# CookiePPP/cookietts

Measured on AMD Instinct MI355X. Metric: audio samples/sec (22.05kHz) WaveGlow infer, 80×900 mel, 1/2/4/8 GPU; real-time factor, higher is better.
Workload: dtype f32; 1 GPU; WaveGlow full (12 flows, 512 WN ch, 8 groups, 8 layers) fp32 infer, batch 8 x (80x900) mel per GPU, sigma 0.6, random-init weights; batch_per_gpu=8, frames=900, parallelism=utterance-batch shard x1

## Files before the change

cookietts_amd/_lib.py:

```python
from __future__ import annotations

import ctypes as C
import os
import threading

import torch

from . import build as _build

_LOCK = threading.Lock()
_LIB = None


class WaveGlowConfig(C.Structure):
    _fields_ = [(n, C.c_int32) for n in (
        "n_mel_channels", "n_group", "n_flows", "n_early_every", "n_early_size",
        "win_length", "hop_length", "n_layers", "n_channels", "kernel_size", "cond_hidden", "speaker_embed_dim",
        "f32_gemm_mode")]


class StftConfig(C.Structure):
    _fields_ = [("filter_length", C.c_int32), ("hop_length", C.c_int32), ("win_length", C.c_int32),
                ("n_mel_channels", C.c_int32), ("clamp_val", C.c_float)]

# ... 205 lines not shown
    "ctts_torchmoji_lengths": (C.c_int, [_FP, _FP, C.c_int32, C.c_int32, _FP]),
    "ctts_torchmoji_features_f32": (C.c_int, [C.POINTER(TorchMojiConfig), _FP, _FP, _FP, _FP, _FP, C.c_int32, C.c_int32, _FP,
                                              C.c_size_t, _FP]),
    "ctts_attention_pool_f32": (C.c_int, [_FP, _FP, _FP, _FP, _FP, C.c_int32, C.c_int32, C.c_int32, _FP]),
    "ctts_taco_embed_f32": (C.c_int, [_FP, _FP, _FP, _FP, _FP, C.c_int32, C.c_int32, C.c_int32, C.c_int32, C.c_int32,
                                      C.c_int32, _FP]),
    "ctts_taco_memory_f32": (C.c_int, [C.POINTER(TacoMemoryWeights), _FP, _FP, _FP, _FP, _FP, C.c_int32, C.c_int32,
                                       C.c_int32, C.c_int32, C.c_int32, C.c_int32, C.c_int32, _FP]),
    "ctts_taco_memory_sylps_f32": (C.c_int, [C.POINTER(TacoMemoryWeights), _FP, _FP, _FP, _FP, _FP, _FP, C.c_int32, C.c_int32,
                                             C.c_int32, C.c_int32, C.c_int32, C.c_int32, C.c_int32, _FP]),
    "ctts_pad_rows_f32": (C.c_int, [_FP, C.c_int64, C.c_int32, _FP, C.c_int32, C.c_int32, C.c_int32, C.c_int32,
                                    C.c_int32, _FP]),
    "ctts_unpad_rows_f32": (C.c_int, [_FP, _FP, C.c_int64, C.c_int32, C.c_int32, C.c_int32, C.c_int32, C.c_int32,
                                      C.c_int32, _FP]),
    "ctts_stft_packed_bytes": (C.c_size_t, [C.POINTER(StftConfig)]),
    "ctts_stft_pack": (C.c_int, [C.POINTER(StftConfig), _FP, _FP, _FP, _FP]),
    "ctts_stft_workspace_bytes": (C.c_size_t, [C.POINTER(StftConfig), C.c_int32, C.c_int32]),
    "ctts_stft_mel_f32": (C.c_int, [C.POINTER(StftConfig), _FP, _FP, _FP, _FP, C.c_int32, C.c_int32, _FP,
                                    C.c_size_t, _FP]),
    "ctts_stft_pack_inverse": (C.c_int, [C.POINTER(StftConfig), _FP, _FP, _FP, _FP]),
    "ctts_stft_transform_f32": (C.c_int, [C.POINTER(StftConfig), _FP, _FP, _FP, _FP, C.c_int32, C.c_int32, _FP,
                                          C.c_size_t, _FP]),
    "ctts_stft_inverse_f32": (C.c_int, [C.POINTER(StftConfig), _FP, _FP, _FP, _FP, C.c_float, _FP, C.c_int32,
                                        C.c_int32, _FP, C.c_size_t, _FP]),
    "ctts_stft_inverse_bias_f32": (C.c_int, [C.POINTER(StftConfig), _FP, _FP, _FP, _FP, C.c_int32, C.c_float, _FP,
                                             C.c_int32, C.c_int32, _FP, C.c_size_t, _FP]),
    "ctts_waveflow_inverse_cond_f32": (C.c_int, [C.POINTER(WaveFlowConfig), _FP, _FP, _FP, C.c_int32, C.c_int32, _FP,
                                                 C.c_int32, C.c_int32, C.c_int32, _FP, C.c_size_t, _FP]),
    "ctts_waveflow_abort_status": (C.c_int, [C.POINTER(WaveFlowConfig), C.c_int32, C.c_int32, _FP, C.c_size_t, _FP]),
    "ctts_wgax_packed_bytes": (C.c_size_t, [C.POINTER(WgaxConfig)]),
    "ctts_wgax_pack_flow": (C.c_int, [C.POINTER(WgaxConfig), C.c_int32, C.POINTER(WgaxFlowWeights), _FP, _FP]),
    "ctts_wgax_workspace_bytes": (C.c_size_t, [C.POINTER(WgaxConfig), C.c_int32, C.c_int64]),
    "ctts_wgax_inverse_f32": (C.c_int, [C.POINTER(WgaxConfig), _FP, _FP, _FP, C.c_int32, C.c_int32, C.c_int32, _FP,
                                        C.c_int32, C.c_int64, _FP, C.c_size_t, _FP]),
    "ctts_wgax_packed_f16_bytes": (C.c_size_t, [C.POINTER(WgaxConfig)]),
    "ctts_wgax_pack_flow_f16": (C.c_int, [C.POINTER(WgaxConfig), C.c_int32, C.POINTER(WgaxFlowWeights), _FP, _FP]),
    "ctts_wgax_workspace_f16_bytes": (C.c_size_t, [C.POINTER(WgaxConfig), C.c_int32, C.c_int64]),
    "ctts_wgax_inverse_f16": (C.c_int, [C.POINTER(WgaxConfig), _FP, _FP, _FP, C.c_int32, C.c_int32, C.c_int32, _FP,
                                        C.c_int32, C.c_int64, _FP, C.c_size_t, _FP]),
    "ctts_wgax_sep_packed_bytes": (C.c_size_t, [C.POINTER(WgaxConfig)]),
    "ctts_wgax_sep_pack_flow": (C.c_int, [C.POINTER(WgaxConfig), C.c_int32, C.POINTER(WgaxFlowWeights), C.POINTER(_FP),
                                          C.POINTER(_FP), _FP, _FP]),
    "ctts_wgax_sep_workspace_bytes": (C.c_size_t, [C.POINTER(WgaxConfig), C.c_int32, C.c_int64]),
    "ctts_wgax_sep_inverse_f32": (C.c_int, [C.POINTER(WgaxConfig), _FP, _FP, _FP, C.c_int32, C.c_int32, C.c_int32, _FP,
                                            C.c_int32, C.c_int64, _FP, C.c_size_t, _FP]),
    "ctts_depthwise_conv1d_f32": (C.c_int, [_FP, _FP, _FP, _FP] + [C.c_int32] * 7 + [_FP]),
    "ctts_hifigan_weight_floats": (C.c_size_t, [C.POINTER(HifiganConfig)]),
    "ctts_hifigan_packed_bytes": (C.c_size_t, [C.POINTER(HifiganConfig)]),
    "ctts_hifigan_pack_f32": (C.c_int, [C.POINTER(HifiganConfig), _FP, C.c_size_t, _FP, _FP]),
    "ctts_hifigan_workspace_bytes": (C.c_size_t, [C.POINTER(HifiganConfig), C.c_int32, C.c_int32]),
    "ctts_hifigan_forward_f32": (C.c_int, [C.POINTER(HifiganConfig), _FP, _FP, C.c_int32, _FP, C.c_int32, C.c_int32, _FP,
                                           C.c_size_t, _FP]),
    "ctts_hifigan_packed_f16_bytes": (C.c_size_t, [C.POINTER(HifiganConfig)]),
    "ctts_hifigan_pack_f16": (C.c_int, [C.POINTER(HifiganConfig), _FP, C.c_size_t, _FP, _FP]),
    "ctts_hifigan_workspace_f16_bytes": (C.c_size_t, [C.POINTER(HifiganConfig), C.c_int32, C.c_int32]),
    "ctts_hifigan_forward_f16": (C.c_int, [C.POINTER(HifiganConfig), _FP, _FP, C.c_int32, _FP, C.c_int32, C.c_int32, _FP,
                                           C.c_size_t, _FP]),
    "ctts_hifigan_packed_bf16x3_bytes": (C.c_size_t, [C.POINTER(HifiganConfig)]),
    "ctts_hifigan_pack_bf16x3": (C.c_int, [C.POINTER(HifiganConfig), _FP, C.c_size_t, _FP, _FP]),
    "ctts_hifigan_workspace_bf16x3_bytes": (C.c_size_t, [C.POINTER(HifiganConfig), C.c_int32, C.c_int32]),
    "ctts_hifigan_forward_bf16x3": (C.c_int, [C.POINTER(HifiganConfig), _FP, _FP, C.c_int32, _FP, C.c_int32, C.c_int32, _FP,
                                              C.c_size_t, _FP]),
    "ctts_replicate_halo_f32":(C.c_int, [_FP, C.c_int32, C.c_int32, C.c_int32, C.c_int32, C.c_int32, C.c_int32, _FP]),
    "ctts_embed_rows_f32": (C.c_int, [_FP, _FP, _FP, C.c_int32, C.c_int32, C.c_int32, C.c_int32, C.c_int32, C.c_int32,
                                      C.c_int32, _FP]),
    "ctts_scale_add_rows_f32": (C.c_int, [_FP, _FP, _FP, _FP, C.c_int32, C.c_int32, C.c_int32, C.c_int32, C.c_int32,
                                          _FP]),
    "ctts_deemphasis_f32": (C.c_int, [_FP, _FP, C.c_int32, C.c_int32, C.c_double, _FP]),
    "ctts_alignment_workspace_bytes": (C.c_size_t, [C.c_int32, C.c_int32, C.c_int32]),
    "ctts_alignment_metric_f32": (C.c_int, [_FP, _FP, _FP, C.c_int32, C.c_int32, C.c_int32, C.c_float, _FP, _FP,
                                            C.c_size_t, _FP]),
    "ctts_first_over_thresh_f32": (C.c_int, [_FP, C.c_int32, C.c_int32, C.c_float, _FP, _FP]),
    "ctts_taco_stop_state_bytes": (C.c_size_t, [C.c_int32]),
    "ctts_taco_stop_reset": (C.c_int, [_FP, C.c_int32, C.c_int32, _FP]),
    "ctts_taco_stop_rule_f32": (C.c_int, [_FP, C.c_int32, C.c_int32, C.c_int32, C.c_int32, C.c_float, C.c_int32, _FP, _FP]),
    "ctts_retry_state_bytes": (C.c_size_t, [C.POINTER(RetryConfig)]),
    "ctts_retry_state_layout": (C.c_int, [C.POINTER(RetryConfig), C.POINTER(C.c_size_t)]),
    "ctts_retry_reset": (C.c_int, [C.POINTER(RetryConfig), _FP, _FP]),
    "ctts_retry_update_f32": (C.c_int, [C.POINTER(RetryConfig), _FP, _FP, _FP, _FP, _FP, _FP, C.c_int32, C.c_int32, _FP, _FP,
                                        _FP]),
    "ctts_retry_vocoder_batch_f32": (C.c_int, [C.POINTER(RetryConfig), _FP, _FP, C.c_int32, C.c_float, _FP]),
    "ctts_pcm16_concat": (C.c_int, [_FP, C.c_int32, _FP, C.c_int32, C.c_int64, C.c_int32, C.c_int32, _FP, C.c_int64, _FP,
                                    _FP]),
    "ctts_affine_rows_f32": (C.c_int, [_FP, C.c_int32, C.c_int32, C.c_int32, C.c_int32, C.c_int32, C.c_int32, C.c_float,
                                       C.c_float, _FP]),
    "ctts_vol_unscale_f32": (C.c_int, [_FP, C.c_int64, _FP]),
    "ctts_resample_rows_f32": (C.c_int, [_FP, _FP] + [C.c_int32] * 9 + [C.c_float, _FP]),
    "ctts_interleave_phases_f32": (C.c_int, [_FP, _FP] + [C.c_int32] * 10 + [_FP]),
    "ctts_last_gemm_loop": (C.c_int, []),
    "ctts_tuning_reload": (C.c_int, []),
    "ctts_tuning_flags": (C.c_int, []),
    "ctts_profile_create": (C.c_int, [C.POINTER(C.c_void_p)]),
    "ctts_profile_bind": (C.c_int, [C.c_void_p]),
    "ctts_profile_collect": (C.c_int, [C.c_void_p, C.c_int32, C.POINTER(C.c_int64), C.POINTER(C.c_double)]),
    "ctts_profile_destroy": (C.c_int, [C.c_void_p]),
}

MODEL_GEMM_MODES = {None: 0, "default": 0, "f32": 1, "bf16x3": 2, "bf16x6": 3}
GEMM_MODES = {"f32": 1, "bf16x3": 2, "bf16x6": 3}


def model_gemm_mode(mode):
    try:
        return MODEL_GEMM_MODES[mode]
    except KeyError:
        raise ValueError(f"f32 GEMM mode {mode!r}: expected one of 'default', 'f32', 'bf16x3', 'bf16x6'") from None


def set_f32_gemm_mode(mode):
    if mode in (None, "default", "f32"):
        return "f32"
    raise RuntimeError(f"cookietts_amd.set_f32_gemm_mode({mode!r}): the process-wide default was removed; "
                       f"call model.set_f32_gemm_mode({mode!r}) on each model instead")


class Profile:

    def __init__(self):
        h = C.c_void_p()
        check(lib().ctts_profile_create(C.byref(h)), "ctts_profile_create")
        self._h = h

    def __enter__(self):
        check(lib().ctts_profile_bind(self._h), "ctts_profile_bind")
        return self

    def __exit__(self, *exc):
        check(lib().ctts_profile_bind(None), "ctts_profile_bind")
        return False

    bind = __enter__

    def unbind(self):
        self.__exit__()

    def collect(self, which):
        n, ms = C.c_int64(), C.c_double()
        check(lib().ctts_profile_collect(self._h, which, C.byref(n), C.byref(ms)), "ctts_profile_collect")
        return int(n.value), float(ms.value)

    def close(self):
        if self._h is not None and _LIB is not None:
            _LIB.ctts_profile_destroy(self._h)
        self._h = None

    def __del__(self):
        try:
            self.close()
        except Exception:
            pass


TUNING_BITS = {"CTTS_F32_NO_GLDS": 0, "CTTS_GEMM_NO_XCD_PAIR": 1, "CTTS_F32_WINOGRAD_FUSED_MIN": 2, "CTTS_BF16_NO_WIDE": 3, "CTTS_BF16_NO_PP": 4,
               "CTTS_F32_WINOGRAD_NO_FUSED": 5, "CTTS_WF_NO_FUSE": 7,
               "CTTS_TACO_NO_FUSE": 8, "CTTS_F32_NO_SMALL": 9, "CTTS_F32_FORCE_SMALL": 10, "CTTS_F32_NO_SPLITK": 11, "CTTS_WF_NO_VEC_INTERP": 12,
               "CTTS_F32_NO_DEFER_SKIP": 13, "CTTS_WF_NO_REGION_SPLIT": 14, "CTTS_WF_NO_ROW_QUEUE": 15, "CTTS_WF_ROW_QUEUE_MIN": 16,
               "CTTS_WF_INJECT_ABORT": 17, "CTTS_WF_QUEUE_DEBUG": 18, "CTTS_F32_NO_ROUND_SPLIT": 19, "CTTS_BF16_PS": 20, "CTTS_BF16_NO_PS": 21,
               "CTTS_TACO_POLL_DELAY": 23, "CTTS_TACO_VALU": 24, "CTTS_UP_NO_MFMA": 25, "CTTS_F32_NO_WN_FOLD": 26, "CTTS_TACO_BG_NO_PIPE": 27,
               "CTTS_F32_NO_WINOGRAD": 28, "CTTS_F32_WINOGRAD_MIN": 29, "CTTS_F32_WINOGRAD_PLAIN": 30}


def tuning_reload():
    check(lib().ctts_tuning_reload(), "ctts_tuning_reload")


def tuning_active(name):
    return bool(lib().ctts_tuning_flags() >> TUNING_BITS[name] & 1)


PROF_WN_IN = 0
PROF_WN_RS = 1
PROF_WN_SKIP = 2
PROF_WN_IN0F = 3
PROF_WN_SKEND = 4
PROF_WN_RES_F = 5


class HipLibraryError(RuntimeError):
    pass


def lib_path():
    return _build.LIB_PATH


def lib():
    global _LIB
    if _LIB is not None:
        return _LIB
    with _LOCK:
        if _LIB is not None:
            return _LIB
        path = lib_path()
        if not os.path.exists(path):
            raise HipLibraryError(
                f"{path} is missing: build it with `python -m cookietts_amd.build` "
                "(or __graft_entry__.build()); there is no CPU fallback for the hot path")
        try:
            handle = C.CDLL(path)
        except OSError as e:
            raise HipLibraryError(f"cannot load {path}: {e}") from e
        for name, (res, args) in SIGNATURES.items():
            try:
                fn = getattr(handle, name)
            except AttributeError as e:
                raise HipLibraryError(f"{path} does not export {name}") from e
            fn.restype = res
            fn.argtypes = args
        if handle.ctts_abi_version() != 7:
            raise HipLibraryError(f"ABI version mismatch: library reports {handle.ctts_abi_version()}")
        _LIB = handle
    return _LIB


def last_error():
    msg = lib().ctts_last_error()
    return msg.decode(errors='replace') if msg else ''


def check(rc, what):
    if rc != 0:
        raise HipLibraryError(f"{what} failed (rc={rc}): {last_error()}")


def nbytes(fn, *args, what):
    n = fn(*args)
    if n == 0:
        raise HipLibraryError(f"{what}: {last_error()}")
    return n


def ptr(t):
    if t is None:
        return None
    return C.c_void_p(t.data_ptr())


def stream(device):
    return C.c_void_p(torch.cuda.current_stream(device).cuda_stream)
```

cookietts_amd/csrc/gemm_f32.hip:

```cpp
#include <atomic>
#include <cstdlib>
#include <mutex>

#include "gemm_f32.h"
#include "tuning.h"
#include "gemm_bf16.h"

namespace ctts {

typedef float f32x16 __attribute__((ext_vector_type(16)));

namespace {

constexpr int STAGE = GEMM_KC * (256 + 128);
constexpr int GEMM_GLDS_MAX_CHUNKS = 384;

__device__ __forceinline__ float fast_sigmoid(float u) {
    return __builtin_amdgcn_rcpf(1.0f + __builtin_amdgcn_exp2f(u * -1.4426950408889634f));
}
__device__ __forceinline__ float fast_tanh(float u) {
    return 1.0f - 2.0f * __builtin_amdgcn_rcpf(1.0f + __builtin_amdgcn_exp2f(u * 2.8853900817779268f));
}

typedef const __attribute__((address_space(1))) float* gfloat_ptr;
// ... 564 lines not shown
                            if (c < a.pairC && ns_ok) dst[(size_t)c * a.dst_ld + a.dst_pad + ns] = v;
                        }
                    }
                }
            }
        }
    } else if constexpr (EPI == GEMM_EPI_GATE_RS) {
        static_assert(EPI != GEMM_EPI_GATE_RS || WM == 1, "fused res/skip needs the 128-row block shape");
        float actv[2][2][16];
#pragma unroll
        for (int mt = 0; mt < 2; ++mt)
#pragma unroll
            for (int nt = 0; nt < 2; ++nt)
#pragma unroll
                for (int r = 0; r < 16; ++r) {
                    const int row = (r & 3) + 8 * (r >> 2) + 4 * lhi;
                    const bool ok = mt * 32 + row < a.pairC;
                    float u0 = acc[mt][nt][r] + bias[mt * 32 + row];
                    float u1 = acc[mt + 2][nt][r] + bias[64 + mt * 32 + row];
                    if (a.addend) {
                        const float* ad = a.addend + (size_t)b * a.addend_bstride + a.addend_pad + n0 + wn * 64 + nt * 32 + l31;
                        const int c = min(mt * 32 + row, a.pairC - 1);
                        u0 += ad[(size_t)c * a.addend_ld];
                        u1 += ad[(size_t)(a.pairC + c) * a.addend_ld];
                    }
                    actv[mt][nt][r] = ok ? fast_tanh(u0) * fast_sigmoid(u1) : 0.0f;
                }
        __syncthreads();
        for (int i = t * 4; i < 64 * 128; i += 1024)
            *reinterpret_cast<float4*>(lds + i) = *reinterpret_cast<const float4*>(a.rs_wT + i);
        if (t < 128) lds[64 * 128 + t] = a.rs_bias[t];
        __syncthreads();
#pragma unroll
        for (int i = 0; i < 4; ++i)
#pragma unroll
            for (int j = 0; j < 2; ++j)
#pragma unroll
                for (int r = 0; r < 16; ++r) acc[i][j][r] = 0.0f;
#pragma unroll
        for (int s = 0; s < 32; ++s) {
            const int r = s & 15;
            const int ch = (s >> 4) * 32 + (r & 3) + 8 * (r >> 2) + 4 * lhi;
            float a2[4];
#pragma unroll
            for (int mt = 0; mt < 4; ++mt) a2[mt] = lds[ch * 128 + mt * 32 + l31];
#pragma unroll
            for (int mt = 0; mt < 4; ++mt)
#pragma unroll
                for (int nt = 0; nt < 2; ++nt)
                    acc[mt][nt] = __builtin_amdgcn_mfma_f32_32x32x2f32(a2[mt], actv[s >> 4][nt][r], acc[mt][nt], 0, 0, 0);
        }
        split_epilogue<GEMM_EPI_SPLIT>(a, acc, lds + 64 * 128, a.rs_rows, 0, b, n0 + wn * 64, l31, lhi);
    } else {
        split_epilogue<EPI>(a, acc, bias, a.M, mb * BM + wm * 128, b, n0 + wn * 64, l31, lhi, EXT ? (long long)part * a.part_dst0 : 0);
    }
#undef CTTS_MAP_PAR
#undef CTTS_A_PTR
}

inline int gemm_f32_mode() { return CTTS_GEMM_F32; }

template <int EPI, int XS>
void launch_shape_xs(int bm, dim3 grid, hipStream_t stream, const GemmArgs& a) {
    const bool few = a.nseg <= 4;
    if (bm == 128) {
        if (few) hipLaunchKernelGGL((conv_gemm_f32_kernel<EPI, 1, 4, true, XS>), grid, dim3(256), 0, stream, a);
        else hipLaunchKernelGGL((conv_gemm_f32_kernel<EPI, 1, GEMM_MAX_SEG, true, XS>), grid, dim3(256), 0, stream, a);
    } else {
        if (few) hipLaunchKernelGGL((conv_gemm_f32_kernel<EPI, 2, 4, true, XS>), grid, dim3(256), 0, stream, a);
        else hipLaunchKernelGGL((conv_gemm_f32_kernel<EPI, 2, GEMM_MAX_SEG, true, XS>), grid, dim3(256), 0, stream, a);
    }
}

template <int EPI, bool GLDS>
void launch_shape_g(int bm, dim3 grid, hipStream_t stream, const GemmArgs& a) {
    const bool few = a.nseg <= 4;
    if (bm == 128) {
        if (few) hipLaunchKernelGGL((conv_gemm_f32_kernel<EPI, 1, 4, GLDS>), grid, dim3(256), 0, stream, a);
        else hipLaunchKernelGGL((conv_gemm_f32_kernel<EPI, 1, GEMM_MAX_SEG, GLDS>), grid, dim3(256), 0, stream, a);
    } else {
        if (few) hipLaunchKernelGGL((conv_gemm_f32_kernel<EPI, 2, 4, GLDS>), grid, dim3(256), 0, stream, a);
        else hipLaunchKernelGGL((conv_gemm_f32_kernel<EPI, 2, GEMM_MAX_SEG, GLDS>), grid, dim3(256), 0, stream, a);
    }
}

template <int EPI>
void launch_shape(int bm, dim3 grid, hipStream_t stream, const GemmArgs& a) {
    if (tuning().f32_no_glds || a.nch_total > GEMM_GLDS_MAX_CHUNKS) launch_shape_g<EPI, false>(bm, grid, stream, a);
    else if (gemm_split_level(a.gemm_mode) == 6) launch_shape_xs<EPI, 6>(bm, grid, stream, a);
    else if (gemm_split_level(a.gemm_mode) == 3) launch_shape_xs<EPI, 3>(bm, grid, stream, a);
    else launch_shape_g<EPI, true>(bm, grid, stream, a);
}

}

int get_gemm_f32_mode() { return gemm_f32_mode(); }
namespace { thread_local int t_last_loop = 0; }
void note_gemm_loop(int code) { t_last_loop = code; }
int last_gemm_loop() { return t_last_loop; }
int gemm_split_level(int m) {
    if (m == CTTS_GEMM_DEFAULT) m = gemm_f32_mode();
    if (m == CTTS_GEMM_BF16X3) return 3;
    if (m == CTTS_GEMM_BF16X6) return 6;
    return 0;
}
bool gemm_mode_is_split(int m) { return gemm_split_level(m) != 0; }

namespace {
std::mutex g_tune_mu;
Tuning g_tune{};
bool g_tune_loaded = false;
void load_tuning_locked() {
    auto on = [](const char* n) { return getenv(n) != nullptr; };
    auto num = [](const char* n, int d) { const char* v = getenv(n); return v ? atoi(v) : d; };
    g_tune.f32_no_glds = on("CTTS_F32_NO_GLDS");
    g_tune.f32_no_small = on("CTTS_F32_NO_SMALL");
    g_tune.f32_force_small = on("CTTS_F32_FORCE_SMALL");
    g_tune.f32_no_splitk = on("CTTS_F32_NO_SPLITK");
    g_tune.f32_no_round_split = on("CTTS_F32_NO_ROUND_SPLIT");
    g_tune.no_xcd_pair = on("CTTS_GEMM_NO_XCD_PAIR");
    g_tune.bf16_no_wide = on("CTTS_BF16_NO_WIDE");
    g_tune.bf16_no_pp = on("CTTS_BF16_NO_PP");
    g_tune.bf16_wide_min = num("CTTS_BF16_WIDE_MIN", 192);
    g_tune.bf16_ps = on("CTTS_BF16_PS");
    g_tune.bf16_no_ps = on("CTTS_BF16_NO_PS");
    g_tune.wf_no_fuse = on("CTTS_WF_NO_FUSE");
    g_tune.taco_no_fuse = on("CTTS_TACO_NO_FUSE");
    g_tune.taco_valu = on("CTTS_TACO_VALU");
    g_tune.up_no_mfma = on("CTTS_UP_NO_MFMA");
    g_tune.taco_bg_no_pipe = on("CTTS_TACO_BG_NO_PIPE");
    {
        static const int dflt[6] = {0x10000 | 36, 0x10000 | 96, 0x10000 | 12, 0x10000 | 20, 0x10000 | 8, 0x10000 | 8};
        int v[6];
        for (int i = 0; i < 6; ++i) v[i] = dflt[i];
        const char* e = getenv("CTTS_TACO_POLL_DELAY");
        if (e && sscanf(e, "%d,%d,%d,%d,%d,%d", v, v + 1, v + 2, v + 3, v + 4, v + 5) != 6)
            for (int i = 0; i < 6; ++i) v[i] = dflt[i];
        for (int i = 0; i < 6; ++i) g_tune.taco_poll_delay[i] = v[i] < 0 ? 0 : v[i];
        g_tune.taco_poll_delay_set = e != nullptr;
    }
    g_tune.wf_no_vec_interp = on("CTTS_WF_NO_VEC_INTERP");
    g_tune.wf_no_region_split = on("CTTS_WF_NO_REGION_SPLIT");
    g_tune.wf_no_row_queue = on("CTTS_WF_NO_ROW_QUEUE");
    g_tune.wf_row_queue_min = num("CTTS_WF_ROW_QUEUE_MIN", -1);
    g_tune.wf_inject_abort = num("CTTS_WF_INJECT_ABORT", 0);
    g_tune.wf_queue_debug = num("CTTS_WF_QUEUE_DEBUG", 0);
    g_tune.f32_no_defer_skip = on("CTTS_F32_NO_DEFER_SKIP");
    g_tune.f32_no_wn_fold = on("CTTS_F32_NO_WN_FOLD");
    g_tune.f32_no_winograd = on("CTTS_F32_NO_WINOGRAD");
    g_tune.f32_winograd_min = num("CTTS_F32_WINOGRAD_MIN", -1);
    g_tune.f32_winograd_plain = on("CTTS_F32_WINOGRAD_PLAIN");
    g_tune.f32_winograd_fused_min = num("CTTS_F32_WINOGRAD_FUSED_MIN", -1);
    g_tune.f32_winograd_no_fused = on("CTTS_F32_WINOGRAD_NO_FUSED");
    g_tune_loaded = true;
}
}

Tuning tuning() {
    std::lock_guard<std::mutex> lk(g_tune_mu);
    if (!g_tune_loaded) load_tuning_locked();
    return g_tune;
}
void reload_tuning() {
    std::lock_guard<std::mutex> lk(g_tune_mu);
    load_tuning_locked();
}

int gemm_check_args(int epi, const GemmArgs& a) {
    CTTS_CHECK_ARG(a.bm == 256 || a.bm == 128, "gemm: bm=%d", a.bm);
    CTTS_CHECK_ARG(gemm_mode_valid(a.gemm_mode), "gemm: f32_gemm_mode %d (0 default, 1 fp32 MFMA, 2 split bf16)", a.gemm_mode);
    const int bn = gemm_bn(a.bm);
    CTTS_CHECK_ARG(a.nseg >= 1 && a.nseg <= GEMM_MAX_SEG, "gemm: nseg=%d", a.nseg);
    int nch = 0;
    for (int s = 0; s < a.nseg; ++s) {
        CTTS_CHECK_ARG(a.seg[s].nch > 0 && a.seg[s].base, "gemm: empty segment %d", s);
        CTTS_CHECK_ARG(a.seg[s].shift >= -a.pad && a.seg[s].shift <= a.pad,
                       "gemm: shift %d exceeds halo %d", a.seg[s].shift, a.pad);
        nch += a.seg[s].nch;
    }
    CTTS_CHECK_ARG(nch == a.nch_total, "gemm: chunk count mismatch %d vs %d", nch, a.nch_total);
    if (a.interleave > 1) {
        CTTS_CHECK_ARG(a.interleave <= a.nseg, "gemm: interleave %d > nseg %d", a.interleave, a.nseg);
        for (int s = 1; s < a.interleave; ++s)
            CTTS_CHECK_ARG(a.seg[s].nch == a.seg[0].nch, "gemm: interleaved segments must have equal length");
    }
    CTTS_CHECK_ARG(a.a_nch_alloc == 0 || a.a_ch_off + a.nch_total <= a.a_nch_alloc, "gemm: A chunk window");
    CTTS_CHECK_ARG(a.ld % 4 == 0 && a.ntiles * bn + 2 * a.pad <= a.ld && a.L <= a.ntiles * bn,
                   "gemm: bad geometry ld=%d pad=%d L=%d ntiles=%d bn=%d", a.ld, a.pad, a.L, a.ntiles, bn);
    CTTS_CHECK_ARG(gemm_epi_is_pair(epi) || a.split % 32 == 0, "gemm: split %d not a multiple of 32", a.split);
    const int cpb = a.bm / 2;
    CTTS_CHECK_ARG(gemm_epi_is_pair(epi) ? (a.pairC > (a.MB - 1) * cpb && a.pairC <= a.MB * cpb)
                                         : (a.M > (a.MB - 1) * a.bm && a.M <= a.MB * a.bm),
                   "gemm: M=%d pairC=%d MB=%d bm=%d", a.M, a.pairC, a.MB, a.bm);
    CTTS_CHECK_ARG(a.dst_ld > 0 && a.dst0, "gemm: destination not set");
    CTTS_CHECK_ARG(a.addend_frames == 0 || ((epi == GEMM_EPI_GATE || epi == GEMM_EPI_GATEX) && a.addend && a.addend_frames <= a.addend_ld - a.addend_pad),
                   "gemm: interpolated addend needs the GATE epilogue (frames=%d)", a.addend_frames);
    CTTS_CHECK_ARG(a.gate >= 0 && a.gate < GATE_KINDS && (a.gate == 0 || epi == GEMM_EPI_GATE), "gemm: gate=%d with epilogue %d",
                   a.gate, epi);
    CTTS_CHECK_ARG((a.addend2 == nullptr && a.map_d == 0) ||
                       (epi == GEMM_EPI_GATE && a.gate == GATE_GTU && a.addend_frames == 0 && a.map_d >= 0 &&
                        (a.addend2 == nullptr || (a.addend && (a.addend2_sign == 1.0f || a.addend2_sign == -1.0f))) &&
                        (a.map_d == 0 || ((a.map_par == 0 || a.map_par == 1) && a.map_L > 0 && a.map_col0 >= 0))),
                   "gemm: second addend / mapped store need the GATE epilogue (epilogue %d, map_d=%d)", epi, a.map_d);
    CTTS_CHECK_ARG(epi != GEMM_EPI_GATE_RS ||
                       (a.bm == 128 && a.pairC <= 64 && a.MB == 1 && a.rs_wT && a.rs_bias && (a.rs_rows == 64 || a.rs_rows == 128)),
                   "gemm: fused res/skip needs bm=128, <= 64 channels, rs_wT / rs_bias and 64 or 128 res/skip rows");
    const int parts = a.parts > 1 ? a.parts : 1;
    CTTS_CHECK_ARG(a.parts >= 0 && a.parts <= 2 && (a.mseg == 0 || a.mseg == 2), "gemm: parts=%d mseg=%d", a.parts, a.mseg);
    if (parts > 1 || a.mseg) {
        CTTS_CHECK_ARG((epi == GEMM_EPI_SPLIT || (epi == GEMM_EPI_GATE && a.gate == GATE_GTU)) && a.bm == 256 && a.nseg <= 4 &&
                           a.interleave <= 1 && gemm_split_level(a.gemm_mode) == 0 && a.shape_blocks == 0 && a.addend_frames == 0,
                       "gemm: parts / mapped segment need the fp32 SPLIT or GATE launch of the 256-row shape (epilogue %d, nseg=%d)", epi, a.nseg);
        CTTS_CHECK_ARG(parts == 1 || epi != GEMM_EPI_SPLIT || (a.acc0 == 0 && a.src0 == nullptr && a.split >= a.M),
                       "gemm: a two-part SPLIT launch stores every row to dst0");
        CTTS_CHECK_ARG(parts == 1 || (long long)parts * a.ntiles * a.batch < (1ll << 31) / a.MB, "gemm: merged grid");
    }
    if (a.mseg) {
        const GemmSeg& g = a.seg[1];
        CTTS_CHECK_ARG(epi == GEMM_EPI_GATE && a.nseg == 2 && a.map_d > 0 && a.map_d % 4 == 0 && a.map_col0 % 4 == 0 && a.mseg_pad >= 0 &&
                           a.mseg_pad % 4 == 0 && a.mseg_ld % 4 == 0 && a.mseg_ld - a.mseg_pad >= 4 && g.bstride % 4 == 0 &&
                           (parts == 1 || a.part_seg[1] % 4 == 0) && reinterpret_cast<uintptr_t>(g.base) % 16 == 0 && g.shift == 0 &&
                           g.mb_rows == 0,
                       "gemm: mapped segment d=%d col0=%d ld=%d pad=%d", a.map_d, a.map_col0, a.mseg_ld, a.mseg_pad);
    }
    return CTTS_OK;
}

bool gemm_f32_dma_staged(int nch_total) { return !tuning().f32_no_glds && nch_total <= GEMM_GLDS_MAX_CHUNKS; }

namespace {
GemmArgs gemm_part_args(const GemmArgs& a, int p) {
    GemmArgs r = a;
    r.parts = 0;
    if (p == 0) return r;
    r.A += a.part_A;
    for (int j = 0; j < r.nseg && j < 4; ++j) r.seg[j].base += a.part_seg[j];
    r.dst0 += a.part_dst0;
    r.map_par = p;
    r.addend2_sign = -a.addend2_sign;
    return r;
}
}

int launch_gemm_f32(int epi, const GemmArgs& a_in, hipStream_t stream) {
    GemmArgs a = a_in;
    gemm_apply_defaults(a);
    if (int rc = gemm_check_args(epi, a)) return rc;
    if (epi == GEMM_EPI_GATE && a.gate != GATE_GTU) epi = GEMM_EPI_GATEX;
    const int parts = a.parts > 1 ? a.parts : 1;
    const bool ext = parts > 1 || a.mseg;
    a.mseg_ch0 = a.mseg_ch1 = 0;
    if (a.mseg) { a.mseg_ch0 = a.seg[0].nch; a.mseg_ch1 = a.seg[0].nch + a.seg[1].nch; }
    CTTS_CHECK_ARG(!a.mseg || gemm_f32_dma_staged(a.nch_total), "gemm: the mapped segment needs the DMA-staged kernels");
    if (parts > 1 && (gemm_f32_small_applies(epi, a) || !gemm_f32_dma_staged(a.nch_total))) {
        for (int p = 0; p < parts; ++p)
            if (int rc = launch_gemm_f32(epi, gemm_part_args(a, p), stream)) return rc;
        return CTTS_OK;
    }
    if (gemm_f32_small_applies(epi, a)) return launch_gemm_f32_small(epi, a, stream);
    long long tiles = (long long)parts * a.ntiles * a.batch;
    if (a.bm == 256 && epi != GEMM_EPI_GATE_RS && a.addend_frames == 0 && a.shape_blocks == 0 && !tuning().f32_no_round_split &&
        !tuning().f32_no_glds && !tuning().f32_no_small && a.nch_total <= GEMM_GLDS_MAX_CHUNKS) {
        const long long slots = 2ll * wf_row_cus();
        const long long rounds = a.MB * tiles / slots;
        const long long rem_tiles = (a.MB * tiles - rounds * slots + a.MB - 1) / a.MB;
        if (rounds >= 2 && rem_tiles > 0 && rem_tiles * a.MB <= slots * 3 / 10 && rem_tiles < a.ntiles &&
            (long long)(a.ntiles - rem_tiles) * gemm_bn(a.bm) < a.L) {
            GemmArgs r = gemm_part_args(a, parts - 1);
            const int bn = gemm_bn(a.bm);
            const long long co = (long long)(a.ntiles - rem_tiles) * bn;
            const long long bo = a.batch - 1;
            for (int j = 0; j < r.nseg; ++j) r.seg[j].base += bo * r.seg[j].bstride + (r.mseg && j == 1 ? 0 : co);
            if (r.dst0) r.dst0 += bo * r.dst0_bstride + (r.map_d > 0 ? 0 : co);
            if (r.map_d > 0) r.map_col0 += (int)co;
            if (r.dst1) r.dst1 += bo * r.dst1_bstride + co;
            if (r.src0) r.src0 += bo * r.src0_bstride + co;
            if (r.addend) r.addend += bo * r.addend_bstride + co;
            if (r.addend2) r.addend2 += bo * r.addend_bstride + co;
            r.L = a.L - (int)co;
            r.ntiles = (int)rem_tiles;
            r.batch = 1;
            if (int rc = launch_gemm_f32_small(epi, r, stream)) return rc;
            tiles -= rem_tiles;
        }
    }
    a.gt_limit = (int)tiles;
    long long blocks = (long long)a.MB * tiles;
    a.map_mode = 0;
    if (a.MB == 4 && epi != GEMM_EPI_GATE_RS && !tuning().no_xcd_pair) {
        a.map_mode = 1;
        blocks = 16ll * ((tiles + 3) / 4);
    }
    CTTS_CHECK_ARG(blocks > 0 && blocks < (1ll << 31), "gemm: grid %lld", blocks);
    dim3 grid((unsigned)blocks);
    note_gemm_loop((tuning().f32_no_glds || a.nch_total > GEMM_GLDS_MAX_CHUNKS) ? 0 : gemm_split_level(a.gemm_mode));
    if (ext) {
        if (epi == GEMM_EPI_GATE) hipLaunchKernelGGL((conv_gemm_f32_kernel<GEMM_EPI_GATE, 2, 4, true, 0, true>), grid, dim3(256), 0, stream, a);
        else hipLaunchKernelGGL((conv_gemm_f32_kernel<GEMM_EPI_SPLIT, 2, 4, true, 0, true>), grid, dim3(256), 0, stream, a);
        CTTS_CHECK_LAUNCH("conv_gemm_f32");
        return CTTS_OK;
    }
    switch (epi) {
        case GEMM_EPI_GATEX: launch_shape<GEMM_EPI_GATEX>(a.bm, grid, stream, a); break;
        case GEMM_EPI_GATE: launch_shape<GEMM_EPI_GATE>(a.bm, grid, stream, a); break;
        case GEMM_EPI_GATE_RS:
            if (tuning().f32_no_glds || a.nch_total > GEMM_GLDS_MAX_CHUNKS) {
// ... 26 lines not shown
```

cookietts_amd/csrc/tuning.h:

```cpp
#pragma once

namespace ctts {

struct Tuning {
    bool f32_no_glds;
    bool f32_no_small;
    bool f32_force_small;
    bool f32_no_splitk;
    bool f32_no_round_split;
    bool no_xcd_pair;
    bool bf16_no_wide;
    int bf16_wide_min;
    bool bf16_no_pp;
    bool bf16_ps;
    bool bf16_no_ps;
    bool wf_no_fuse;
    bool taco_poll_delay_set;
    int taco_poll_delay[6];
    bool taco_no_fuse;
    bool taco_bg_no_pipe;
    bool up_no_mfma;
    bool taco_valu;
    bool f32_no_defer_skip;
    bool f32_no_wn_fold;
    bool f32_no_winograd;
    int f32_winograd_min;
    bool f32_winograd_plain;
    int f32_winograd_fused_min;
    bool f32_winograd_no_fused;
    bool wf_no_region_split;
    bool wf_no_row_queue;
    int wf_row_queue_min;
    int wf_queue_debug;
    int wf_inject_abort;
    bool wf_no_vec_interp;
};

Tuning tuning();
void reload_tuning();

}
```

cookietts_amd/csrc/waveglow_api.hip:

```cpp
#include <mutex>
#include <vector>

#include "gemm_bf16.h"
#include "gemm_f32.h"
#include "tuning.h"
#include "waveglow_kernels.h"
#include "wn_winograd_layer.h"

namespace ctts {

static thread_local char g_err[512] = "";

void set_error(const char* fmt, ...) {
    va_list ap;
    va_start(ap, fmt);
    vsnprintf(g_err, sizeof(g_err), fmt, ap);
    va_end(ap);
}

namespace {

constexpr size_t ALIGN_F = 64;
inline size_t align_up(size_t v) { return (v + ALIGN_F - 1) / ALIGN_F * ALIGN_F; }
constexpr int A_TILE = GEMM_KC * GEMM_BM;

struct FlowDims { int n_rem, n_half, ch_off; };

struct Plan {
    ctts_waveglow_config c;
    int C, H, K0, n_in;
    int S;
    int nch0, nch1h, nch_in, nch_rs;
    int mb_in;
    int nch_in0f;
    std::vector<FlowDims> fd;
    size_t up_w, up_wp, up_b, cond0_A, cond0_b, cond1_A, cond1_b;
    size_t zero_b;
    bool up_mfma;
    struct Flow {
        size_t start_w, start_b, end_w, end_b, winv, spk_tab;
        std::vector<size_t> in_A, in_b, rs_A, rs_b;
        std::vector<size_t> res_A, res_b, skip_A, skip_b;
        size_t in0f_w, in0f_A, skend_W, skend_b;
        std::vector<size_t> wg_T2_A, wg_T3_A, wg_e_A, wg_o_A;
        size_t wg_dense;
    };
    std::vector<Flow> fl;
    size_t total;

    static constexpr int F32_SKIP_GROUP = 4;
    int mb_c() const { return (C + GEMM_BM - 1) / GEMM_BM; }
    int n_groups() const { return (c.n_layers + F32_SKIP_GROUP - 1) / F32_SKIP_GROUP; }
    int group_layers(int g) const { return g + 1 < n_groups() ? F32_SKIP_GROUP : c.n_layers - g * F32_SKIP_GROUP; }
    int rs_rows(int layer) const { return layer < c.n_layers - 1 ? 2 * C : C; }
    int rs_mb(int layer) const { return (rs_rows(layer) + GEMM_BM - 1) / GEMM_BM; }
};

int make_plan(const ctts_waveglow_config* cfg, Plan& p) {
    CTTS_CHECK_ARG(cfg != nullptr, "config is NULL");
    p.c = *cfg;
    const auto& c = p.c;
    CTTS_CHECK_ARG(c.n_flows >= 1 && c.n_layers >= 1 && c.n_layers <= 12, "n_flows=%d n_layers=%d", c.n_flows, c.n_layers);
    CTTS_CHECK_ARG(gemm_mode_valid(c.f32_gemm_mode), "f32_gemm_mode=%d (CTTS_GEMM_DEFAULT / _F32 / _BF16X3 / _BF16X6)", c.f32_gemm_mode);
    CTTS_CHECK_ARG(c.n_group >= 4 && c.n_group % 4 == 0 && c.n_group <= 16, "n_group=%d (4, 8, 12 or 16)", c.n_group);
    CTTS_CHECK_ARG(c.kernel_size == 3, "kernel_size=%d (only 3 built)", c.kernel_size);
    CTTS_CHECK_ARG(c.n_channels >= 128 && c.n_channels % 128 == 0, "n_channels=%d (multiple of 128)", c.n_channels);
    CTTS_CHECK_ARG(c.cond_hidden == GEMM_BM, "cond_hidden=%d (reference hard-codes 256)", c.cond_hidden);
    CTTS_CHECK_ARG(c.hop_length > 0 && c.win_length % c.hop_length == 0 && c.hop_length % c.n_group == 0,
                   "win=%d hop=%d n_group=%d", c.win_length, c.hop_length, c.n_group);
    CTTS_CHECK_ARG((c.n_mel_channels * c.n_group) % GEMM_KC == 0, "n_mel*n_group=%d not a multiple of 16",
                   c.n_mel_channels * c.n_group);
    CTTS_CHECK_ARG(c.n_early_every >= 1 && c.n_early_size >= 0 && c.n_early_size % 2 == 0, "early outputs");
    CTTS_CHECK_ARG(c.speaker_embed_dim >= 0 && c.speaker_embed_dim <= 1024, "speaker_embed_dim=%d", c.speaker_embed_dim);
    p.C = c.n_channels;
    p.H = c.cond_hidden;
    p.K0 = c.n_mel_channels * c.n_group;
    p.S = round_up(c.speaker_embed_dim, 32);
    CTTS_CHECK_ARG(p.S == 0 || p.K0 % 32 == 0, "multispeaker needs n_mel*n_group %% 32 == 0");
    p.nch0 = (p.K0 + p.S) / GEMM_KC;
    p.nch1h = p.H / GEMM_KC;
    p.nch_in = (c.kernel_size * p.C + p.H) / GEMM_KC;
    p.nch_rs = p.C / GEMM_KC;
    p.mb_in = 2 * p.C / GEMM_BM;
    p.nch_in0f = c.kernel_size + p.nch1h;
    int n_half = c.n_group / 2, n_rem = c.n_group;
    p.fd.resize(c.n_flows);
    for (int k = 0; k < c.n_flows; ++k) {
        if (k % c.n_early_every == 0 && k > 0) { n_half -= c.n_early_size / 2; n_rem -= c.n_early_size; }
        CTTS_CHECK_ARG(n_half >= 1 && n_rem == 2 * n_half, "flow %d: n_half=%d n_remaining=%d", k, n_half, n_rem);
        p.fd[k] = {n_rem, n_half, c.n_group - n_rem};
    }
    size_t o = 0;
    auto take = [&](size_t n) { size_t r = o; o = align_up(o + n); return r; };
    p.up_w = take((size_t)c.n_mel_channels * c.n_mel_channels * c.win_length);
    p.up_mfma = upsample_mfma_shape(c.n_mel_channels, c.win_length, c.hop_length, c.n_group);
    p.up_wp = p.up_mfma ? take((size_t)c.n_mel_channels * c.n_mel_channels * c.win_length) : 0;
    p.up_b = take(c.n_mel_channels);
    p.cond0_A = take((size_t)c.n_flows * p.nch0 * A_TILE);
    p.cond0_b = take((size_t)c.n_flows * GEMM_BM);
    p.cond1_A = take((size_t)c.n_flows * p.nch1h * A_TILE);
    p.cond1_b = take((size_t)c.n_flows * GEMM_BM);
    p.zero_b = take((size_t)p.mb_in * GEMM_BM);
    p.fl.resize(c.n_flows);
    for (int k = 0; k < c.n_flows; ++k) {
        auto& f = p.fl[k];
        f.start_w = take((size_t)p.C * p.fd[k].n_half);
        f.start_b = take(p.C);
        f.end_w = take((size_t)2 * p.fd[k].n_half * p.C);
        f.end_b = take(2 * p.fd[k].n_half);
        f.winv = take((size_t)p.fd[k].n_rem * p.fd[k].n_rem);
        f.spk_tab = take((size_t)CTTS_N_SPEAKERS * c.speaker_embed_dim);
        for (int i = 0; i < c.n_layers; ++i) {
            f.in_A.push_back(take((size_t)p.mb_in * p.nch_in * A_TILE));
            f.in_b.push_back(take((size_t)p.mb_in * GEMM_BM));
            f.rs_A.push_back(take((size_t)p.rs_mb(i) * p.nch_rs * A_TILE));
            f.rs_b.push_back(take((size_t)p.rs_mb(i) * GEMM_BM));
            f.res_A.push_back(i + 1 < c.n_layers ? take((size_t)p.mb_c() * p.nch_rs * A_TILE) : 0);
            f.res_b.push_back(i + 1 < c.n_layers ? take((size_t)p.mb_c() * GEMM_BM) : 0);
        }
        for (int gi = 0; gi < p.n_groups(); ++gi) {
            f.skip_A.push_back(take((size_t)p.mb_c() * p.group_layers(gi) * p.nch_rs * A_TILE));
            f.skip_b.push_back(take((size_t)p.mb_c() * GEMM_BM));
        }
        f.in0f_w = take((size_t)2 * p.C * FOLD_ROWS * c.kernel_size);
        f.in0f_A = take((size_t)p.mb_in * p.nch_in0f * A_TILE);
        f.skend_W = take((size_t)c.n_layers * p.C * 2 * p.fd[k].n_half);
        f.skend_b = take(2 * p.fd[k].n_half);
        for (int i = 0; i < c.n_layers; ++i) {
            f.wg_T2_A.push_back(take((size_t)p.mb_in * p.nch_rs * A_TILE));
            f.wg_T3_A.push_back(take((size_t)p.mb_in * p.nch_rs * A_TILE));
            f.wg_e_A.push_back(take((size_t)p.mb_in * (p.nch_rs + p.nch1h) * A_TILE));
            f.wg_o_A.push_back(take((size_t)p.mb_in * (p.nch_rs + p.nch1h) * A_TILE));
        }
        f.wg_dense = take((size_t)3 * 2 * p.C * p.C);
    }
    p.total = o;
    return CTTS_OK;
}

struct Geom { int L, ld, pad, ntiles; };

int make_geom(const Plan& p, int frames, Geom& g) {
    CTTS_CHECK_ARG(frames >= 1, "frames=%d", frames);
    const long long T = (long long)frames * p.c.hop_length;
    g.L = (int)(T / p.c.n_group);
    int maxd = 1 << (p.c.n_layers - 1);
    g.pad = round_up(maxd > 128 ? maxd : 128, 32);
    g.ntiles = (g.L + GEMM_BN - 1) / GEMM_BN;
    g.ld = round_up(g.L, 256) + 2 * g.pad;
    return CTTS_OK;
}

struct PairGeom { int d, Lp, ntiles; };
PairGeom pair_geom(const Geom& g, int layer) {
    const int d = 1 << layer;
    const int Lp = (g.L + 2 * d - 1) / (2 * d) * d;
    return {d, Lp, (Lp + GEMM_BN - 1) / GEMM_BN};
}
int pair_ld(const Plan& p, const Geom& g) {
    int nt = 0;
    for (int i = 0; i < p.c.n_layers; ++i) nt = std::max(nt, pair_geom(g, i).ntiles);
    return nt * GEMM_BN;
}
constexpr long long WINOGRAD_MIN_COLS = 28800;
bool winograd_engages(const Plan& p, const Geom& g) {
    const Tuning t = tuning();
    if (t.f32_no_winograd || gemm_split_level(p.c.f32_gemm_mode) != 0) return false;
    const long long min_cols = t.f32_winograd_min >= 0 ? t.f32_winograd_min : WINOGRAD_MIN_COLS;
    return (long long)g.L >= min_cols;
}

constexpr long long WINOGRAD_FUSED_MIN_COLS = 28800;
bool winograd_fused_engages(const Plan& p, const Geom& g) {
    const Tuning t = tuning();
    if (t.f32_winograd_no_fused || t.f32_winograd_plain || t.f32_no_glds || !wn_winograd_layer_supported(p.C, p.H)) return false;
    const long long min_cols = t.f32_winograd_fused_min >= 0 ? t.f32_winograd_fused_min : WINOGRAD_FUSED_MIN_COLS;
    return winograd_engages(p, g) && (long long)g.L >= min_cols;
}

struct Workspace {
    float *audio, *spect, *spk, *h_tmp, *h_all, *x, *act, *out;
    float* act_all;
    float* a16;
    float* skend;
    float *wgV, *wgT, *wgH;
    int ldp;
    size_t total;
};

void carve(const Plan& p, const Geom& g, int batch, float* base, Workspace& w) {
    size_t o = 0;
    auto take = [&](size_t n) { size_t r = o; o = align_up(o + n); return base ? base + r : nullptr; };
    const size_t B = batch;
    w.audio = take(B * p.c.n_group * g.L);
    w.spect = take(B * p.K0 * g.ld);
    w.spk = take(B * p.c.n_flows * p.S * g.ld);
    w.h_tmp = take(B * p.c.n_flows * p.H * g.ld);
    w.h_all = take(B * p.c.n_flows * p.H * g.ld);
    w.x = take(B * p.C * g.ld);
    w.act = take(B * p.C * g.ld);
    w.out = take(B * p.C * g.ld);
    w.act_all = take((size_t)std::min(p.c.n_layers, (int)Plan::F32_SKIP_GROUP) * B * p.C * g.ld);
    w.a16 = take(B * FOLD_ROWS * g.ld);
    w.skend = take(B * p.c.n_group * g.ld);
    w.wgV = w.wgT = w.wgH = nullptr;
    w.ldp = 0;
    if (winograd_engages(p, g)) {
        w.ldp = pair_ld(p, g);
        w.wgV = take((size_t)4 * B * p.C * w.ldp);
        w.wgT = take((size_t)2 * B * 2 * p.C * w.ldp);
        w.wgH = take((size_t)2 * B * p.H * w.ldp);
    }
    w.total = o;
}

struct Prof {
    std::mutex mu;
    std::vector<std::pair<hipEvent_t, hipEvent_t>> ev[CTTS_PROF_N];
    std::vector<std::pair<hipEvent_t, hipEvent_t>> pool;
};
thread_local Prof* t_prof = nullptr;

struct ProfScope {
    int which; hipStream_t s; hipEvent_t stop = nullptr; bool active = false;
    ProfScope(int which_, hipStream_t s_) : which(which_), s(s_) {
        Prof* pr = t_prof;
        if (!pr) return;
        std::lock_guard<std::mutex> lk(pr->mu);
        std::pair<hipEvent_t, hipEvent_t> e;
        if (!pr->pool.empty()) { e = pr->pool.back(); pr->pool.pop_back(); }
        else { if (hipEventCreate(&e.first) != hipSuccess || hipEventCreate(&e.second) != hipSuccess) return; }
        (void)hipEventRecord(e.first, s);
        stop = e.second;
        pr->ev[which].push_back(e);
        active = true;
    }
    ~ProfScope() { if (active) (void)hipEventRecord(stop, s); }
};

GemmArgs base_args(const Plan& p, const Geom& g, int batch) {
    GemmArgs a{};
    a.gemm_mode = p.c.f32_gemm_mode;
    a.ld = g.ld; a.pad = g.pad; a.L = g.L; a.ntiles = g.ntiles; a.batch = batch;
    a.dst_ld = g.ld; a.dst_pad = g.pad;
    return a;
}

__global__ __launch_bounds__(256) void speaker_rows_kernel(const float* __restrict__ table, const int64_t* __restrict__ ids,
                                                           float* __restrict__ spk, int k, int n_flows, int S, int sdim,
                                                           int L, int ld, int pad) {
    const int n = blockIdx.x * 256 + threadIdx.x;
    const int e = blockIdx.y, b = blockIdx.z;
    if (n >= ld) return;
    float v = 0.f;
    if (e < sdim && n >= pad && n < pad + L) {
        const long long id = ids[b];
        v = (id >= 0 && id < CTTS_N_SPEAKERS) ? table[(size_t)id * sdim + e] : __builtin_nanf("");
    }
    spk[((size_t)b * n_flows * S + (size_t)k * S + e) * ld + n] = v;
}

int fill_speaker_rows(const Plan& p, const Geom& g, const float* blob, const int64_t* ids, float* spk, int batch,
                      hipStream_t s) {
    if (p.S == 0) return CTTS_OK;
    CTTS_CHECK_ARG(ids != nullptr, "multispeaker model (speaker_embed_dim=%d) needs speaker ids (glow.py:193)",
                   p.c.speaker_embed_dim);
    for (int k = 0; k < p.c.n_flows; ++k)
        hipLaunchKernelGGL(speaker_rows_kernel, dim3((g.ld + 255) / 256, p.S, batch), dim3(256), 0, s,
                           blob + p.fl[k].spk_tab, ids, spk, k, p.c.n_flows, p.S, p.c.speaker_embed_dim, g.L, g.ld, g.pad);
    CTTS_CHECK_LAUNCH("speaker_rows");
    return CTTS_OK;
}

int run_cond(const Plan& p, const Geom& g, const float* blob, const float* spect, const float* spk, float* h_tmp,
             float* h_all, int batch, hipStream_t s) {
    const long long hstride = (long long)p.c.n_flows * p.H * g.ld;
    GemmArgs a = base_args(p, g, batch);
    a.A = blob + p.cond0_A; a.bias = blob + p.cond0_b;
    a.nseg = 1; a.nch_total = p.nch0; a.MB = p.c.n_flows;
    a.seg[0] = {spect, (long long)p.K0 * g.ld, p.K0 / GEMM_KC, 0, 0, 0};
    if (p.S) {
        CTTS_CHECK_ARG(spk != nullptr, "wn_cond: multispeaker model needs the speaker rows");
        a.nseg = 2;
        a.seg[1] = {spk, (long long)p.c.n_flows * p.S * g.ld, p.S / GEMM_KC, 0, p.S, 0};
    }
    a.dst0 = h_tmp; a.dst0_bstride = hstride; a.acc0 = 0;
    a.dst1 = h_tmp; a.dst1_bstride = hstride; a.acc1 = 0;
    a.split = p.c.n_flows * GEMM_BM;
    a.M = p.c.n_flows * GEMM_BM;
    int rc = launch_gemm_f32(GEMM_EPI_SPLIT, a, s);
    if (rc) return rc;
    a.A = blob + p.cond1_A; a.bias = blob + p.cond1_b;
    a.nseg = 1; a.nch_total = p.nch1h;
    a.seg[0] = {h_tmp, hstride, p.nch1h, 0, GEMM_BM, 0};
    a.dst0 = h_all; a.dst1 = h_all;
    return launch_gemm_f32(GEMM_EPI_SPLIT, a, s);
}

struct WnFold { float* a16; float* skend; float* audio; float* wave; };
struct WnWinograd { float* V; float* T; float* Hc; int ldp; };

int run_in_layer_winograd(const Plan& p, const Geom& g, const float* blob, int k, int i, const float* x, const float* h_all,
                          float* act, const WnWinograd& wg, int batch, hipStream_t s) {
    const auto& f = p.fl[k];
    const PairGeom pg = pair_geom(g, i);
    const int C = p.C, H = p.H, ldp = wg.ldp;
    const long long hstride = (long long)p.c.n_flows * H * g.ld;
    const size_t vplane = (size_t)batch * C * ldp, tplane = (size_t)batch * 2 * C * ldp, hplane = (size_t)batch * H * ldp;
    const bool lean = !tuning().f32_winograd_plain && gemm_f32_dma_staged(p.nch_rs + p.nch1h);
    const bool in_place = lean && pg.d % 4 == 0;
    const bool fused = lean && winograd_fused_engages(p, g);
    const float* h2 = h_all + (size_t)k * H * g.ld;
    int rc = launch_winograd_transform(x, (long long)C * g.ld, h2, hstride, wg.V, wg.Hc, batch, C, H, pg.d, g.L, pg.Lp, g.ld, g.pad,
                                       ldp, pg.ntiles * GEMM_BN, !in_place, lean, s);
    if (rc) return rc;
    if (fused) {
        WnWinogradLayerArgs w{};
        w.A_T2 = blob + f.wg_T2_A[i]; w.A_T3 = blob + f.wg_T3_A[i]; w.A_e = blob + f.wg_e_A[i]; w.A_o = blob + f.wg_o_A[i];
        w.bias = blob + f.in_b[i];
        w.V = wg.V; w.vplane = (long long)vplane;
        w.Hc = wg.Hc; w.hplane = (long long)hplane;
        w.h2 = h2; w.h_bstride = hstride;
        w.act = act; w.act_bstride = (long long)C * g.ld;
        w.C = C; w.H = H; w.batch = batch;
        w.ldp = ldp; w.Lp = pg.Lp; w.ntiles = pg.ntiles;
        w.d = pg.d; w.L = g.L; w.ld = g.ld; w.pad = g.pad;
        w.in_place = in_place;
        return launch_wn_winograd_layer(w, s);
    }
    GemmArgs a{};
    a.gemm_mode = p.c.f32_gemm_mode;
    a.ld = ldp; a.pad = 0; a.L = pg.Lp; a.ntiles = pg.ntiles; a.batch = batch; a.MB = p.mb_in;
    a.bias = blob + p.zero_b;
    a.nseg = 1; a.nch_total = p.nch_rs;
    a.dst_ld = ldp; a.dst_pad = 0; a.dst0_bstride = (long long)2 * C * ldp;
    a.M = 2 * C; a.split = 2 * C;
    const int np = lean ? 1 : 2;
    if (lean) {
        a.parts = 2;
        a.part_A = (long long)f.wg_T3_A[i] - (long long)f.wg_T2_A[i];
        a.part_seg[0] = (long long)vplane;
        a.part_dst0 = (long long)tplane;
    }
    for (int j = 0; j < np; ++j) {
        a.A = blob + (j == 0 ? f.wg_T2_A[i] : f.wg_T3_A[i]);
        a.seg[0] = {wg.V + (1 + j) * vplane, (long long)C * ldp, p.nch_rs, 0, 0, 0};
        a.dst0 = wg.T + j * tplane;
        if ((rc = launch_gemm_f32(GEMM_EPI_SPLIT, a, s))) return rc;
    }
    a.bias = blob + f.in_b[i];
    a.nseg = 2; a.nch_total = p.nch_rs + p.nch1h;
    a.split = 0; a.pairC = C;
    a.dst0 = act; a.dst0_bstride = (long long)C * g.ld; a.dst_ld = g.ld; a.dst_pad = g.pad;
    a.addend = wg.T; a.addend2 = wg.T + tplane; a.addend_bstride = (long long)2 * C * ldp;
    a.map_d = pg.d; a.map_L = g.L;
    if (lean) {
        a.part_A = (long long)f.wg_o_A[i] - (long long)f.wg_e_A[i];
        a.part_seg[0] = (long long)(3 * vplane);
        a.part_seg[1] = in_place ? 0 : (long long)hplane;
        a.part_dst0 = 0;
    }
    if (in_place) { a.mseg = 2; a.mseg_ld = g.ld; a.mseg_pad = g.pad; }
    for (int j = 0; j < np; ++j) {
        a.A = blob + (j == 0 ? f.wg_e_A[i] : f.wg_o_A[i]);
        a.seg[0] = {wg.V + (j == 0 ? 0 : 3) * vplane, (long long)C * ldp, p.nch_rs, 0, 0, 0};
        if (in_place) a.seg[1] = {h2, hstride, p.nch1h, 0, 0, 0};
        else a.seg[1] = {wg.Hc + j * hplane, (long long)H * ldp, p.nch1h, 0, 0, 0};
        a.addend2_sign = j == 0 ? 1.0f : -1.0f;
        a.map_par = j;
        if ((rc = launch_gemm_f32(GEMM_EPI_GATE, a, s))) return rc;
    }
    return CTTS_OK;
}

int run_wn_stack(const Plan& p, const Geom& g, const float* blob, int k, const float* audio, const float* h_all,
                 float* x, float* act, float* out, int batch, hipStream_t s, float* act_all = nullptr,
                 const WnFold* fold = nullptr, const WnWinograd* wg = nullptr, const CouplingForward* fwd = nullptr) {
    const auto& f = p.fl[k];
    const auto& d = p.fd[k];
    const long long cstride = (long long)p.C * g.ld;
    const long long hstride = (long long)p.c.n_flows * p.H * g.ld;
    int rc = launch_wn_start(audio, blob + f.start_w, blob + f.start_b, x, batch, p.C, p.c.n_group, d.ch_off,
                             d.n_half, g.L, g.ld, g.pad, s);
    if (rc) return rc;
    CTTS_CHECK_ARG(fold == nullptr || act_all != nullptr, "wn_stack: the folded form needs the kept activations");
    if (fold && (rc = launch_wn_start_ones(audio, fold->a16, batch, p.c.n_group, d.ch_off, d.n_half, g.L, g.ld, g.pad, s)))
        return rc;
    const int ncx = p.C / GEMM_KC;
    const bool defer = act_all != nullptr && (fold != nullptr || !tuning().f32_no_defer_skip);
    const size_t act_stride = (size_t)batch * p.C * g.ld;
    for (int i = 0; i < p.c.n_layers; ++i) {
        const int dil = 1 << i;
        if (defer) act = act_all + (size_t)(i % Plan::F32_SKIP_GROUP) * act_stride;
        if (fold && i == 0) {
            GemmArgs a = base_args(p, g, batch);
            a.A = blob + f.in0f_A; a.bias = blob + f.in_b[0];
            a.nseg = 4; a.interleave = 3; a.nch_total = p.nch_in0f; a.MB = p.mb_in;
            const long long astride = (long long)FOLD_ROWS * g.ld;
            a.seg[0] = {fold->a16, astride, 1, -dil, 0, 0};
            a.seg[1] = {fold->a16, astride, 1, 0, 0, 0};
            a.seg[2] = {fold->a16, astride, 1, dil, 0, 0};
            a.seg[3] = {h_all + (size_t)k * p.H * g.ld, hstride, p.nch1h, 0, 0, 0};
            a.dst0 = act; a.dst0_bstride = cstride;
            a.M = 2 * p.C; a.pairC = p.C;
            ProfScope ps(CTTS_PROF_WN_IN, s), ps0(CTTS_PROF_WN_IN0F, s);
            rc = launch_gemm_f32(GEMM_EPI_GATE, a, s);
            if (rc) return rc;
        } else if (wg) {
            ProfScope ps(CTTS_PROF_WN_IN, s);
            rc = run_in_layer_winograd(p, g, blob, k, i, x, h_all, act, *wg, batch, s);
            if (rc) return rc;
        } else {
            GemmArgs a = base_args(p, g, batch);
            a.A = blob + f.in_A[i]; a.bias = blob + f.in_b[i];
            a.nseg = 4; a.interleave = 3; a.nch_total = p.nch_in; a.MB = p.mb_in;
            a.seg[0] = {x, cstride, ncx, -dil, 0, 0};
            a.seg[1] = {x, cstride, ncx, 0, 0, 0};
            a.seg[2] = {x, cstride, ncx, dil, 0, 0};
            a.seg[3] = {h_all + (size_t)k * p.H * g.ld, hstride, p.nch1h, 0, 0, 0};
            a.dst0 = act; a.dst0_bstride = cstride;
            a.M = 2 * p.C; a.pairC = p.C;
            ProfScope ps(CTTS_PROF_WN_IN, s);
            rc = launch_gemm_f32(GEMM_EPI_GATE, a, s);
            if (rc) return rc;
        }
        if (defer) {
            const bool last = i == p.c.n_layers - 1;
            if (!last) {
                GemmArgs a = base_args(p, g, batch);
                a.A = blob + f.res_A[i]; a.bias = blob + f.res_b[i];
                a.nseg = 1; a.nch_total = p.nch_rs; a.MB = p.mb_c();
                a.seg[0] = {act, cstride, p.nch_rs, 0, 0, 0};
                a.M = p.C; a.split = p.C;
                a.dst0 = x; a.dst0_bstride = cstride; a.acc0 = 1;
                a.dst1 = out; a.dst1_bstride = cstride; a.acc1 = 0;
                ProfScope ps(fold ? CTTS_PROF_WN_RES_F : CTTS_PROF_WN_RS, s);
                rc = launch_gemm_f32(GEMM_EPI_SPLIT, a, s);
                if (rc) return rc;
            }
            const int gi = i / Plan::F32_SKIP_GROUP;
            if (fold && (last || (i + 1) % Plan::F32_SKIP_GROUP == 0)) {
                const int E = 2 * d.n_half;
                ProfScope ps(CTTS_PROF_WN_SKEND, s);
                rc = launch_skip_end(act_all, (long long)act_stride, p.group_layers(gi),
                                     blob + f.skend_W + (size_t)gi * Plan::F32_SKIP_GROUP * p.C * E, fold->skend, gi == 0, last,
                                     blob + f.skend_b, blob + f.winv, fold->audio, fold->wave, batch, p.C, p.c.n_group, d.ch_off,
                                     d.n_half, g.L, g.ld, g.pad, s, last ? fwd : nullptr);
                if (rc) return rc;
            } else if (last || (i + 1) % Plan::F32_SKIP_GROUP == 0) {
                const int nl = p.group_layers(gi);
                GemmArgs a = base_args(p, g, batch);
                a.A = blob + f.skip_A[gi]; a.bias = blob + f.skip_b[gi];
                a.nseg = nl; a.nch_total = nl * p.nch_rs; a.MB = p.mb_c();
                for (int j = 0; j < nl; ++j)
                    a.seg[j] = {act_all + (size_t)j * act_stride, cstride, p.nch_rs, 0, 0, 0};
                a.M = p.C; a.split = 0;
                a.dst0 = x; a.dst0_bstride = cstride; a.acc0 = 1;
                a.dst1 = out; a.dst1_bstride = cstride; a.acc1 = gi > 0 ? 1 : 0;
                ProfScope ps(CTTS_PROF_WN_SKIP, s);
                rc = launch_gemm_f32(GEMM_EPI_SPLIT, a, s);
                if (rc) return rc;
            }
        } else {
            const bool last = i == p.c.n_layers - 1;
            GemmArgs a = base_args(p, g, batch);
            a.A = blob + f.rs_A[i]; a.bias = blob + f.rs_b[i];
            a.nseg = 1; a.nch_total = p.nch_rs; a.MB = p.rs_mb(i);
            a.seg[0] = {act, cstride, p.nch_rs, 0, 0, 0};
            a.M = p.rs_rows(i);
            a.dst0 = x; a.dst0_bstride = cstride; a.acc0 = 1;
            a.dst1 = out; a.dst1_bstride = cstride; a.acc1 = i > 0 ? 1 : 0;
            a.split = last ? 0 : p.C;
            ProfScope ps(CTTS_PROF_WN_RS, s);
            rc = launch_gemm_f32(GEMM_EPI_SPLIT, a, s);
            if (rc) return rc;
        }
    }
    return CTTS_OK;
}

int run_flow_tail(const Plan& p, const Geom& g, const float* blob, int k, const float* out, float* audio,
                  float* wave, int batch, hipStream_t s, const CouplingForward* fwd = nullptr) {
    const auto& f = p.fl[k];
    const auto& d = p.fd[k];
    return launch_flow_tail(out, audio, wave, blob + f.end_w, blob + f.end_b, blob + f.winv, batch, p.C,
                            p.c.n_group, d.ch_off, d.n_half, g.L, g.ld, g.pad, s, fwd);
}

int run_flow(const Plan& p, const Geom& g, const float* blob, int k, const Workspace& w, float* audio, const float* h_all,
             float* wave, int batch, hipStream_t s, const CouplingForward* fwd = nullptr) {
    const Tuning t = tuning();
    const bool folded = !t.f32_no_wn_fold && !t.f32_no_defer_skip;
    const WnWinograd wg{w.wgV, w.wgT, w.wgH, w.ldp};
    const WnFold fw{w.a16, w.skend, audio, wave};
    int rc = run_wn_stack(p, g, blob, k, audio, h_all, w.x, w.act, w.out, batch, s, w.act_all, folded ? &fw : nullptr,
                          w.wgV ? &wg : nullptr, fwd);
    if (rc || folded) return rc;
    return run_flow_tail(p, g, blob, k, w.out, audio, wave, batch, s, fwd);
}

size_t fwd_mix_off(const Plan& p, int k) {
    size_t o = 0;
    for (int j = 0; j < k; ++j) o += align_up((size_t)p.fd[j].n_rem * p.fd[j].n_rem);
    return o;
}
int fwd_log_s_rows(const Plan& p, int k) {
    int r = 0;
    for (int j = 0; j < k; ++j) r += p.fd[j].n_half;
    return r;
}

struct FwdWorkspace { Workspace w; double *ls_part, *z_part; int nblk_ls, nblk_z; size_t total; };

void carve_fwd(const Plan& p, const Geom& g, int batch, float* base, FwdWorkspace& fw) {
    carve(p, g, batch, base, fw.w);
    fw.nblk_ls = (g.L + 255) / 256;
    fw.nblk_z = (int)(((long long)p.c.n_group * g.L + FWD_SUMSQ_CHUNK - 1) / FWD_SUMSQ_CHUNK);
    size_t o = fw.w.total;
    auto take = [&](size_t doubles) { size_t r = o; o = align_up(o + 2 * doubles); return base ? reinterpret_cast<double*>(base + r) : nullptr; };
    fw.ls_part = take((size_t)batch * p.c.n_flows * fw.nblk_ls);
    fw.z_part = take((size_t)batch * fw.nblk_z);
    fw.total = o;
}

int run_flow_forward(const Plan& p, const Geom& g, const float* blob, const float* fwd_blob, int k, const FwdWorkspace& fw,
                     float* z, const float* wave, const float* h_all, float* log_s_flow, long long ls_bstride, int batch,
                     hipStream_t s) {
    const auto& d = p.fd[k];
    int rc = launch_flow_head_forward(fwd_blob + fwd_mix_off(p, k), wave, z, batch, p.c.n_group, d.ch_off, d.n_rem, g.L, s);
    if (rc) return rc;
    const CouplingForward cf{log_s_flow, ls_bstride, fw.ls_part + (size_t)k * fw.nblk_ls, (long long)p.c.n_flows * fw.nblk_ls};
    return run_flow(p, g, blob, k, fw.w, z, h_all, nullptr, batch, s, &cf);
}

constexpr int BF_SKIP_GROUP = 4;
struct BfPlan {
    std::vector<std::vector<size_t>> in_A, rs_A;
    std::vector<std::vector<size_t>> skip_A;
    std::vector<size_t> skip_b;
    size_t cond0_A, cond1_A;
    size_t total;
    int nch_in, nch_rs, nch_c0, nch_c1;
    int mb_c, n_groups;
    int P;
    int f16;
    int group_layers(int g, int n_layers) const { return std::min(BF_SKIP_GROUP, n_layers - g * BF_SKIP_GROUP); }
};

void make_bf_plan(const Plan& p, BfPlan& q, int P, int f16 = 0) {
    size_t o = 0;
    auto take = [&](size_t n) { size_t r = o; o = (o + n + 127) / 128 * 128; return r; };
    q.P = P;
    q.f16 = f16;
    q.nch_in = P * (p.c.kernel_size * p.C + p.H) / BGEMM_KC;
    q.nch_rs = P * p.C / BGEMM_KC;
    q.nch_c0 = P * (p.K0 + p.S) / BGEMM_KC;
    q.nch_c1 = P * p.H / BGEMM_KC;
    q.cond0_A = take((size_t)p.c.n_flows * q.nch_c0 * BGEMM_KC * BGEMM_BM);
    q.cond1_A = take((size_t)p.c.n_flows * q.nch_c1 * BGEMM_KC * BGEMM_BM);
    q.mb_c = (p.C + BGEMM_BM - 1) / BGEMM_BM;
    q.n_groups = (p.c.n_layers + BF_SKIP_GROUP - 1) / BF_SKIP_GROUP;
    q.in_A.assign(p.c.n_flows, {});
    q.rs_A.assign(p.c.n_flows, {});
    q.skip_A.assign(p.c.n_flows, {});
    for (int k = 0; k < p.c.n_flows; ++k) {
        for (int i = 0; i < p.c.n_layers; ++i) {
            q.in_A[k].push_back(take((size_t)p.mb_in * q.nch_in * BGEMM_KC * BGEMM_BM));
            q.rs_A[k].push_back(i < p.c.n_layers - 1 ? take((size_t)q.mb_c * q.nch_rs * BGEMM_KC * BGEMM_BM) : 0);
        }
        for (int gi = 0; gi < q.n_groups; ++gi)
            q.skip_A[k].push_back(take((size_t)q.mb_c * q.group_layers(gi, p.c.n_layers) * q.nch_rs * BGEMM_KC * BGEMM_BM));
        q.skip_b.push_back(take((size_t)2 * 2 * q.mb_c * BGEMM_BM));
    }
    q.total = o;
}

struct BfWs {
    float *audio, *spect, *spk;
    bf16_t *spect_bf, *spk_bf, *h_tmp_bf, *h_bf, *x, *act, *out;
    long long spect_lo, spk_lo, h_lo, x_lo, act_lo;
    size_t total_bytes;
};

void carve_bf(const Plan& p, const Geom& g, int batch, char* base, BfWs& w, int P) {
    size_t o = 0;
    auto take = [&](size_t bytes) { size_t r = o; o = (o + bytes + 255) / 256 * 256; return base ? base + r : nullptr; };
    const size_t B = batch;
    const size_t planes = P == 3 ? 2 : 1;
    w.audio = (float*)take(B * p.c.n_group * g.L * 4);
    w.spect = (float*)take(B * p.K0 * g.ld * 4);
    w.spect_bf = (bf16_t*)take(planes * B * p.K0 * g.ld * 2);
    w.spk = (float*)take(B * p.c.n_flows * p.S * g.ld * 4);
    w.spk_bf = (bf16_t*)take(planes * B * p.c.n_flows * p.S * g.ld * 2);
    w.h_tmp_bf = (bf16_t*)take(planes * B * p.c.n_flows * p.H * g.ld * 2);
    w.h_bf = (bf16_t*)take(planes * B * p.c.n_flows * p.H * g.ld * 2);
    w.x = (bf16_t*)take(planes * B * p.C * g.ld * 2);
    w.act = (bf16_t*)take(planes * B * p.C * g.ld * 2 * std::min(p.c.n_layers, BF_SKIP_GROUP));
    w.out = (bf16_t*)take(planes * B * p.C * g.ld * 2);
    const long long on = P == 3 ? 1 : 0;
    w.spect_lo = on * (long long)(B * p.K0 * g.ld);
    w.spk_lo = on * (long long)(B * p.c.n_flows * p.S * g.ld);
    w.h_lo = on * (long long)(B * p.c.n_flows * p.H * g.ld);
    w.x_lo = on * (long long)(B * p.C * g.ld);
    w.act_lo = on * (long long)(B * p.C * g.ld) * std::min(p.c.n_layers, BF_SKIP_GROUP);
    w.total_bytes = o;
}

int push_segs(BGemmArgs& a, int idx, int P, const bf16_t* base, long long lo_off, long long bstride, int nch, int shift,
              int mb_rows) {
    for (int pi = 0; pi < P; ++pi) a.seg[idx++] = {pi == 1 ? base + lo_off : base, bstride, nch, shift, mb_rows};
    return idx;
}

__device__ __forceinline__ unsigned int pack_bf16x2_residual(float v0, float v1, unsigned int hi) {
    return pack_bf16x2(v0 - __builtin_bit_cast(float, hi << 16), v1 - __builtin_bit_cast(float, hi & 0xffff0000u));
}

__global__ __launch_bounds__(256) void cvt_f32_to_k8_kernel(const float* __restrict__ src, bf16_t* __restrict__ dst,
                                                            int rows, int ld, long long lo_off, int f16) {
    const int n = blockIdx.x * 256 + threadIdx.x;
    const int grp = blockIdx.y, b = blockIdx.z;
    if (n >= ld) return;
    const float* s = src + ((size_t)b * rows + (size_t)grp * 8) * ld + n;
    unsigned int pk[4], pl[4];
#pragma unroll
    for (int j = 0; j < 4; ++j) {
        const float v0 = s[(size_t)(2 * j) * ld], v1 = s[(size_t)(2 * j + 1) * ld];
        pk[j] = f16 ? pack_f16x2(v0, v1) : pack_bf16x2(v0, v1);
        pl[j] = pack_bf16x2_residual(v0, v1, pk[j]);
    }
    bf16_t* d = dst + (((size_t)b * (rows / 8) + grp) * ld + n) * 8;
    *reinterpret_cast<uint4*>(d) = make_uint4(pk[0], pk[1], pk[2], pk[3]);
    if (lo_off) *reinterpret_cast<uint4*>(d + lo_off) = make_uint4(pl[0], pl[1], pl[2], pl[3]);
}

template <int H>
__global__ __launch_bounds__(256) void wn_start_bf16_kernel(const float* __restrict__ audio, const float* __restrict__ Ws,
                                                            const float* __restrict__ bs, bf16_t* __restrict__ x, int C,
                                                            int G, int ch_off, int L, int ld, int pad, long long lo_off, int f16) {
    const int n = blockIdx.x * 256 + threadIdx.x;
    const int grp = blockIdx.y, b = blockIdx.z;
    if (n >= L) return;
    float a[H];
#pragma unroll
    for (int j = 0; j < H; ++j) a[j] = audio[((size_t)b * G + ch_off + j) * L + n];
    unsigned int pk[4], pl[4];
// ... 157 lines not shown
            int ns = 0;
            for (int t = 0; t < ks; ++t) ns = push_segs(a, ns, P, w.x, w.x_lo, cstride, ncx, (t - ks / 2) * dil, 0);
            a.interleave = ns;
            ns = push_segs(a, ns, P, w.h_bf + (size_t)k * p.H * g.ld, w.h_lo, hstride, p.H / BGEMM_KC, 0, 0);
            a.nseg = ns; a.nch_total = q.nch_in; a.MB = p.mb_in;
            a.M = 2 * p.C; a.pairC = p.C;
            a.dst0 = act; a.dst0_bstride = cstride; a.lo_off = w.act_lo;
            ProfScope ps(CTTS_PROF_WN_IN, s);
            if ((rc = launch_gemm_bf16(BGEMM_EPI_GATE, a, s))) return rc;
        }
        if (i < p.c.n_layers - 1) {
            BGemmArgs a{};
            a.f16 = q.f16;
            a.ld = g.ld; a.pad = g.pad; a.L = g.L; a.ntiles = g.ntiles; a.batch = batch;
            a.A = bblob + q.rs_A[k][i]; a.bias = blob + f.rs_b[i];
            a.nseg = push_segs(a, 0, P, act, w.act_lo, cstride, ncx, 0, 0); a.nch_total = q.nch_rs; a.MB = q.mb_c;
            a.M = p.C; a.split = p.C;
            a.dst0 = w.x; a.dst0_bstride = cstride; a.acc0 = 1;
            a.dst1 = w.x; a.dst1_bstride = cstride; a.acc1 = 1;
            a.lo_off = w.x_lo;
            ProfScope ps(CTTS_PROF_WN_RS, s);
            if ((rc = launch_gemm_bf16(BGEMM_EPI_SPLIT, a, s))) return rc;
        }
        if (i == p.c.n_layers - 1 || (i + 1) % BF_SKIP_GROUP == 0) {
            if ((rc = skip_group(i / BF_SKIP_GROUP))) return rc;
        }
    }
    return CTTS_OK;
}

}
}

using namespace ctts;

extern "C" {

int ctts_abi_version(void) { return CTTS_ABI_VERSION; }
const char* ctts_last_error(void) { return g_err; }

int ctts_waveglow_geometry_for(const ctts_waveglow_config* cfg, int32_t frames, ctts_waveglow_geometry* out) {
    Plan p; Geom g;
    int rc = make_plan(cfg, p); if (rc) return rc;
    rc = make_geom(p, frames, g); if (rc) return rc;
    CTTS_CHECK_ARG(out != nullptr, "geometry out is NULL");
    out->steps = g.L; out->ld = g.ld; out->pad = g.pad; out->n_remaining = p.fd.back().n_rem;
    return CTTS_OK;
}

int ctts_fold_weightnorm_f32(const float* v, const float* g, float* w, int32_t out_ch, int32_t fan, void* stream) {
    CTTS_CHECK_ARG(v && g && w, "fold_weightnorm: NULL pointer");
    return launch_fold_weightnorm(v, g, w, out_ch, fan, as_stream(stream));
}

size_t ctts_waveglow_packed_bytes(const ctts_waveglow_config* cfg) {
    Plan p;
    if (make_plan(cfg, p)) return 0;
    return p.total * sizeof(float);
}

int ctts_waveglow_pack_upsample(const ctts_waveglow_config* cfg, const float* up_w, const float* up_b, void* packed,
                                void* stream) {
    Plan p;
    int rc = make_plan(cfg, p); if (rc) return rc;
    CTTS_CHECK_ARG(up_w && up_b && packed, "pack_upsample: NULL pointer");
    float* blob = static_cast<float*>(packed);
    const size_t nw = (size_t)p.c.n_mel_channels * p.c.n_mel_channels * p.c.win_length;
    CTTS_CHECK_HIP(hipMemcpyAsync(blob + p.up_w, up_w, nw * sizeof(float), hipMemcpyDeviceToDevice, as_stream(stream)));
    CTTS_CHECK_HIP(hipMemcpyAsync(blob + p.up_b, up_b, p.c.n_mel_channels * sizeof(float), hipMemcpyDeviceToDevice,
                                  as_stream(stream)));
    if (p.up_mfma) return launch_upsample_pack_mfma(up_w, blob + p.up_wp, as_stream(stream));
    return CTTS_OK;
}

int ctts_waveglow_pack_flow(const ctts_waveglow_config* cfg, int32_t k, const ctts_waveglow_flow_weights* w,
                            void* packed, void* stream) {
    Plan p;
    int rc = make_plan(cfg, p); if (rc) return rc;
    CTTS_CHECK_ARG(k >= 0 && k < p.c.n_flows, "pack_flow: flow %d", k);
    CTTS_CHECK_ARG(w && packed, "pack_flow: NULL pointer");
    hipStream_t s = as_stream(stream);
    float* blob = static_cast<float*>(packed);
    const auto& f = p.fl[k];
    const auto& d = p.fd[k];
    const int C = p.C, H = p.H, ks = p.c.kernel_size;
    auto d2d = [&](size_t off, const float* src, size_t n) -> int {
        CTTS_CHECK_ARG(src != nullptr, "pack_flow: NULL weight pointer");
        CTTS_CHECK_HIP(hipMemcpyAsync(blob + off, src, n * sizeof(float), hipMemcpyDeviceToDevice, s));
        return CTTS_OK;
    };
    if ((rc = d2d(f.start_w, w->start_w, (size_t)C * d.n_half))) return rc;
    if ((rc = d2d(f.start_b, w->start_b, C))) return rc;
    if ((rc = d2d(f.end_w, w->end_w, (size_t)2 * d.n_half * C))) return rc;
    if ((rc = d2d(f.end_b, w->end_b, 2 * d.n_half))) return rc;
    if ((rc = d2d(f.winv, w->w_inverse, (size_t)d.n_rem * d.n_rem))) return rc;
    CTTS_CHECK_ARG(w->cond_w[0] && w->cond_w[1] && w->cond_w[2] && w->cond_b[0] && w->cond_b[1] && w->cond_b[2],
                   "pack_flow: NULL cond weights");
    const int sdim = p.c.speaker_embed_dim;
    if ((rc = launch_pack_a(blob + p.cond0_A + (size_t)k * p.nch0 * A_TILE, w->cond_w[0], GEMM_BM, 1, p.nch0, 0, p.K0,
                            GEMM_EPI_SPLIT, C, H, 0, p.K0 + sdim, 1, s))) return rc;
    if (sdim) {
        if ((rc = launch_pack_a(blob + p.cond0_A + (size_t)k * p.nch0 * A_TILE, w->cond_w[0] + p.K0, GEMM_BM, 1, p.nch0,
                                p.K0, sdim, GEMM_EPI_SPLIT, C, H, 0, p.K0 + sdim, 1, s))) return rc;
        if ((rc = d2d(f.spk_tab, w->speaker_embed, (size_t)CTTS_N_SPEAKERS * sdim))) return rc;
    }
    if ((rc = launch_pack_bias(blob + p.cond0_b + (size_t)k * GEMM_BM, GEMM_BM, 1, w->cond_b[0], 0, nullptr, 0,
                               GEMM_EPI_SPLIT, C, H, s))) return rc;
    if ((rc = launch_pack_a(blob + p.cond1_A + (size_t)k * p.nch1h * A_TILE, w->cond_w[1], GEMM_BM, 1, p.nch1h, 0, H,
                            GEMM_EPI_SPLIT, C, H, 0, H, 1, s))) return rc;
    if ((rc = launch_pack_bias(blob + p.cond1_b + (size_t)k * GEMM_BM, GEMM_BM, 1, w->cond_b[1], 0, nullptr, 0,
                               GEMM_EPI_SPLIT, C, H, s))) return rc;
    for (int i = 0; i < p.c.n_layers; ++i) {
        CTTS_CHECK_ARG(w->in_w[i] && w->in_b[i] && w->rs_w[i] && w->rs_b[i], "pack_flow: NULL layer %d weights", i);
        for (int t = 0; t < ks; ++t)
            if ((rc = launch_pack_a(blob + f.in_A[i], w->in_w[i] + t, GEMM_BM, p.mb_in, p.nch_in, 0, C, GEMM_EPI_GATE, C,
                                    2 * C, 0, (long long)C * ks, ks, s, ks, t))) return rc;
        if ((rc = launch_pack_a(blob + f.in_A[i], w->cond_w[2], GEMM_BM, p.mb_in, p.nch_in, ks * C, H, GEMM_EPI_GATE, C,
                                2 * C, (long long)2 * C * i, H, 1, s))) return rc;
        if ((rc = launch_pack_bias(blob + f.in_b[i], GEMM_BM, p.mb_in, w->in_b[i], 0, w->cond_b[2], (long long)2 * C * i,
                                   GEMM_EPI_GATE, C, 2 * C, s))) return rc;
        const int rows = p.rs_rows(i);
        if ((rc = launch_pack_a(blob + f.rs_A[i], w->rs_w[i], GEMM_BM, p.rs_mb(i), p.nch_rs, 0, C, GEMM_EPI_SPLIT, C, rows,
                                0, C, 1, s))) return rc;
        if ((rc = launch_pack_bias(blob + f.rs_b[i], GEMM_BM, p.rs_mb(i), w->rs_b[i], 0, nullptr, 0, GEMM_EPI_SPLIT, C, rows,
                                   s))) return rc;
        const bool last = i == p.c.n_layers - 1;
        const int gi = i / Plan::F32_SKIP_GROUP, gj = i % Plan::F32_SKIP_GROUP;
        if (!last) {
            if ((rc = launch_pack_a(blob + f.res_A[i], w->rs_w[i], GEMM_BM, p.mb_c(), p.nch_rs, 0, C, GEMM_EPI_SPLIT, C, C,
                                    0, C, 1, s))) return rc;
            if ((rc = launch_pack_bias(blob + f.res_b[i], GEMM_BM, p.mb_c(), w->rs_b[i], 0, nullptr, 0, GEMM_EPI_SPLIT, C, C,
                                       s))) return rc;
        }
        if ((rc = launch_pack_a(blob + f.skip_A[gi], w->rs_w[i], GEMM_BM, p.mb_c(), p.group_layers(gi) * p.nch_rs, gj * C, C,
                                GEMM_EPI_SPLIT, C, C, last ? 0 : C, C, 1, s))) return rc;
        hipLaunchKernelGGL(skip_bias_kernel, dim3((p.mb_c() * GEMM_BM + 255) / 256), dim3(256), 0, s, blob + f.skip_b[gi],
                           w->rs_b[i] + (last ? 0 : C), C, p.mb_c() * GEMM_BM, gj == 0 ? 1 : 0);
        CTTS_CHECK_LAUNCH("skip_bias_f32");
    }
    for (int i = 0; i < p.c.n_layers; ++i) {
        float* dense = blob + f.wg_dense;
        const size_t dn = (size_t)2 * C * C;
        if ((rc = launch_winograd_g(w->in_w[i], dense, 2 * C, C, s))) return rc;
        if ((rc = launch_pack_a(blob + f.wg_T2_A[i], dense, GEMM_BM, p.mb_in, p.nch_rs, 0, C, GEMM_EPI_SPLIT, C, 2 * C, 0, C, 1, s))) return rc;
        if ((rc = launch_pack_a(blob + f.wg_T3_A[i], dense + dn, GEMM_BM, p.mb_in, p.nch_rs, 0, C, GEMM_EPI_SPLIT, C, 2 * C, 0, C, 1, s))) return rc;
        if ((rc = launch_pack_a(blob + f.wg_e_A[i], w->in_w[i], GEMM_BM, p.mb_in, p.nch_rs + p.nch1h, 0, C, GEMM_EPI_GATE, C, 2 * C, 0,
                                (long long)C * ks, ks, s))) return rc;
        if ((rc = launch_pack_a(blob + f.wg_o_A[i], dense + 2 * dn, GEMM_BM, p.mb_in, p.nch_rs + p.nch1h, 0, C, GEMM_EPI_GATE, C, 2 * C, 0,
                                C, 1, s))) return rc;
        for (float* A : {blob + f.wg_e_A[i], blob + f.wg_o_A[i]})
            if ((rc = launch_pack_a(A, w->cond_w[2], GEMM_BM, p.mb_in, p.nch_rs + p.nch1h, C, H, GEMM_EPI_GATE, C, 2 * C,
                                    (long long)2 * C * i, H, 1, s))) return rc;
    }
    if ((rc = launch_fold_in0(w->in_w[0], w->start_w, w->start_b, blob + f.in0f_w, C, d.n_half, ks, s))) return rc;
    for (int t = 0; t < ks; ++t)
        if ((rc = launch_pack_a(blob + f.in0f_A, blob + f.in0f_w + t, GEMM_BM, p.mb_in, p.nch_in0f, 0, FOLD_ROWS, GEMM_EPI_GATE, C,
                                2 * C, 0, (long long)FOLD_ROWS * ks, ks, s, ks, t))) return rc;
    if ((rc = launch_pack_a(blob + f.in0f_A, w->cond_w[2], GEMM_BM, p.mb_in, p.nch_in0f, ks * FOLD_ROWS, H, GEMM_EPI_GATE, C,
                            2 * C, 0, H, 1, s))) return rc;
    return launch_fold_skend(w->rs_w, w->rs_b, w->end_w, w->end_b, blob + f.skend_W, blob + f.skend_b, C, p.c.n_layers, d.n_half, s);
}

size_t ctts_waveglow_workspace_bytes(const ctts_waveglow_config* cfg, int32_t batch, int32_t frames) {
    Plan p; Geom g; Workspace w;
    if (make_plan(cfg, p) || make_geom(p, frames, g) || batch < 1) return 0;
    carve(p, g, batch, nullptr, w);
    return w.total * sizeof(float);
}

int ctts_upsample_squeeze_f32(const ctts_waveglow_config* cfg, const void* packed, const float* mel, float* spect,
                              int32_t batch, int32_t frames, void* stream) {
    Plan p; Geom g;
    int rc = make_plan(cfg, p); if (rc) return rc;
    rc = make_geom(p, frames, g); if (rc) return rc;
    CTTS_CHECK_ARG(packed && mel && spect && batch >= 1, "upsample_squeeze: bad argument");
    const float* blob = static_cast<const float*>(packed);
    return launch_upsample_squeeze(mel, blob + p.up_w, p.up_mfma ? blob + p.up_wp : nullptr, blob + p.up_b, spect, batch, p.c.n_mel_channels, frames,
                                   p.c.win_length, p.c.hop_length, p.c.n_group, g.ld, g.pad, as_stream(stream));
}

int ctts_wn_cond_f32(const ctts_waveglow_config* cfg, const void* packed, const float* spect, const float* spk_rows,
                     float* h_tmp, float* h_all, int32_t batch, int32_t frames, void* stream) {
    Plan p; Geom g;
    int rc = make_plan(cfg, p); if (rc) return rc;
    rc = make_geom(p, frames, g); if (rc) return rc;
    CTTS_CHECK_ARG(packed && spect && h_tmp && h_all && batch >= 1, "wn_cond: bad argument");
    return run_cond(p, g, static_cast<const float*>(packed), spect, spk_rows, h_tmp, h_all, batch, as_stream(stream));
}

int ctts_wn_stack_f32(const ctts_waveglow_config* cfg, const void* packed, int32_t flow, const float* audio,
                      const float* h_all, float* x, float* act, float* out, int32_t batch, int32_t frames,
                      void* stream) {
    Plan p; Geom g;
    int rc = make_plan(cfg, p); if (rc) return rc;
    rc = make_geom(p, frames, g); if (rc) return rc;
    CTTS_CHECK_ARG(flow >= 0 && flow < p.c.n_flows, "wn_stack: flow %d", flow);
    CTTS_CHECK_ARG(packed && audio && h_all && x && act && out && batch >= 1, "wn_stack: bad argument");
    return run_wn_stack(p, g, static_cast<const float*>(packed), flow, audio, h_all, x, act, out, batch,
                        as_stream(stream));
}

int ctts_flow_tail_f32(const ctts_waveglow_config* cfg, const void* packed, int32_t flow, const float* out,
                       float* audio, float* wave, int32_t batch, int32_t frames, void* stream) {
    Plan p; Geom g;
    int rc = make_plan(cfg, p); if (rc) return rc;
    rc = make_geom(p, frames, g); if (rc) return rc;
    CTTS_CHECK_ARG(flow >= 0 && flow < p.c.n_flows, "flow_tail: flow %d", flow);
    CTTS_CHECK_ARG(packed && out && audio && batch >= 1, "flow_tail: bad argument");
    return run_flow_tail(p, g, static_cast<const float*>(packed), flow, out, audio, wave, batch, as_stream(stream));
}

int ctts_waveglow_flow_f32(const ctts_waveglow_config* cfg, const void* packed, int32_t flow, float* audio,
                           const float* h_all, float* wave, int32_t batch, int32_t frames, void* workspace,
                           size_t workspace_bytes, void* stream) {
    Plan p; Geom g; Workspace w;
    int rc = make_plan(cfg, p); if (rc) return rc;
    rc = make_geom(p, frames, g); if (rc) return rc;
    CTTS_CHECK_ARG(flow >= 0 && flow < p.c.n_flows, "waveglow_flow: flow %d", flow);
    CTTS_CHECK_ARG(packed && audio && h_all && workspace && batch >= 1, "waveglow_flow: bad argument");
    carve(p, g, batch, static_cast<float*>(workspace), w);
    if (w.total * sizeof(float) > workspace_bytes) {
        set_error("waveglow_flow: workspace %zu bytes < required %zu", workspace_bytes, w.total * sizeof(float));
        return CTTS_E_WORKSPACE;
    }
    return run_flow(p, g, static_cast<const float*>(packed), flow, w, audio, h_all, wave, batch, as_stream(stream));
}

size_t ctts_waveglow_forward_packed_bytes(const ctts_waveglow_config* cfg) {
    Plan p;
    if (make_plan(cfg, p)) return 0;
    return fwd_mix_off(p, p.c.n_flows) * sizeof(float);
}

int ctts_waveglow_pack_forward_mix(const ctts_waveglow_config* cfg, int32_t flow, const float* w, void* packed_fwd,
                                   void* stream) {
    Plan p;
    int rc = make_plan(cfg, p); if (rc) return rc;
    CTTS_CHECK_ARG(flow >= 0 && flow < p.c.n_flows, "pack_forward_mix: flow %d", flow);
    CTTS_CHECK_ARG(w && packed_fwd, "pack_forward_mix: NULL pointer");
    const size_t n = (size_t)p.fd[flow].n_rem * p.fd[flow].n_rem;
    CTTS_CHECK_HIP(hipMemcpyAsync(static_cast<float*>(packed_fwd) + fwd_mix_off(p, flow), w, n * sizeof(float),
                                  hipMemcpyDeviceToDevice, as_stream(stream)));
    return CTTS_OK;
}

size_t ctts_waveglow_forward_workspace_bytes(const ctts_waveglow_config* cfg, int32_t batch, int32_t frames) {
    Plan p; Geom g; FwdWorkspace fw;
    if (make_plan(cfg, p) || make_geom(p, frames, g)) return 0;
    if (batch < 1) { set_error("forward_workspace_bytes: batch=%d", batch); return 0; }
    carve_fwd(p, g, batch, nullptr, fw);
    return fw.total * sizeof(float);
}

int ctts_waveglow_flow_forward_f32(const ctts_waveglow_config* cfg, const void* packed, const void* packed_fwd, int32_t flow,
                                   float* z, const float* wave, const float* h_all, float* log_s, double* sum_log_s,
                                   int32_t batch, int32_t frames, void* workspace, size_t workspace_bytes, void* stream) {
    Plan p; Geom g; FwdWorkspace fw;
    int rc = make_plan(cfg, p); if (rc) return rc;
    rc = make_geom(p, frames, g); if (rc) return rc;
    CTTS_CHECK_ARG(flow >= 0 && flow < p.c.n_flows, "waveglow_flow_forward: flow %d", flow);
    CTTS_CHECK_ARG(packed && packed_fwd && z && h_all && workspace && batch >= 1, "waveglow_flow_forward: bad argument");
    CTTS_CHECK_ARG(wave == nullptr || flow == 0, "waveglow_flow_forward: only flow 0 reads the waveform (flow %d)", flow);
    carve_fwd(p, g, batch, static_cast<float*>(workspace), fw);
    if (fw.total * sizeof(float) > workspace_bytes) {
        set_error("waveglow_flow_forward: workspace %zu bytes < required %zu", workspace_bytes, fw.total * sizeof(float));
        return CTTS_E_WORKSPACE;
    }
    hipStream_t s = as_stream(stream);
    rc = run_flow_forward(p, g, static_cast<const float*>(packed), static_cast<const float*>(packed_fwd), flow, fw, z, wave, h_all,
                          log_s, (long long)p.fd[flow].n_half * g.L, batch, s);
    if (rc || !sum_log_s) return rc;
    return launch_sum_partials(fw.ls_part + (size_t)flow * fw.nblk_ls, (long long)p.c.n_flows * fw.nblk_ls, 0, fw.nblk_ls, sum_log_s,
                               1, 1, batch, s);
}

int ctts_waveglow_forward_spk_f32(const ctts_waveglow_config* cfg, const void* packed, const void* packed_fwd, const float* mel,
                                  const float* audio, const int64_t* speaker_ids, float* z, float* log_s, double* sums,
                                  int32_t batch, int32_t frames, void* workspace, size_t workspace_bytes, void* stream) {
    Plan p; Geom g; FwdWorkspace fw;
    int rc = make_plan(cfg, p); if (rc) return rc;
    rc = make_geom(p, frames, g); if (rc) return rc;
    CTTS_CHECK_ARG(packed && packed_fwd && mel && audio && z && workspace && batch >= 1, "forward: bad argument");
    CTTS_CHECK_ARG(p.S == 0 || speaker_ids != nullptr, "multispeaker model (speaker_embed_dim=%d) needs speaker ids (glow.py:193)",
                   p.c.speaker_embed_dim);
    carve_fwd(p, g, batch, static_cast<float*>(workspace), fw);
    if (fw.total * sizeof(float) > workspace_bytes) {
        set_error("forward: workspace %zu bytes < required %zu", workspace_bytes, fw.total * sizeof(float));
        return CTTS_E_WORKSPACE;
    }
    hipStream_t s = as_stream(stream);
    const float* blob = static_cast<const float*>(packed);
    const Workspace& w = fw.w;
    rc = launch_upsample_squeeze(mel, blob + p.up_w, p.up_mfma ? blob + p.up_wp : nullptr, blob + p.up_b, w.spect, batch, p.c.n_mel_channels, frames,
                                 p.c.win_length, p.c.hop_length, p.c.n_group, g.ld, g.pad, s);
    if (rc) return rc;
    rc = fill_speaker_rows(p, g, blob, speaker_ids, w.spk, batch, s);
    if (rc) return rc;
    rc = run_cond(p, g, blob, w.spect, w.spk, w.h_tmp, w.h_all, batch, s);
    if (rc) return rc;
    const int S = fwd_log_s_rows(p, p.c.n_flows);
    for (int k = 0; k < p.c.n_flows; ++k) {
        float* ls = log_s ? log_s + (size_t)fwd_log_s_rows(p, k) * g.L : nullptr;
        rc = run_flow_forward(p, g, blob, static_cast<const float*>(packed_fwd), k, fw, z, k == 0 ? audio : nullptr, w.h_all, ls,
                              (long long)S * g.L, batch, s);
        if (rc) return rc;
    }
    if (!sums) return CTTS_OK;
    rc = launch_sum_partials(fw.ls_part, (long long)p.c.n_flows * fw.nblk_ls, fw.nblk_ls, fw.nblk_ls, sums, p.c.n_flows + 1,
                             p.c.n_flows, batch, s);
    if (rc) return rc;
    rc = launch_sumsq_partials(z, fw.z_part, batch, (long long)p.c.n_group * g.L, fw.nblk_z, s);
    if (rc) return rc;
    return launch_sum_partials(fw.z_part, fw.nblk_z, 0, fw.nblk_z, sums + p.c.n_flows, p.c.n_flows + 1, 1, batch, s);
}

int ctts_waveglow_infer_f32(const ctts_waveglow_config* cfg, const void* packed, const float* mel,
                            const float* z_scaled, float* wave, int32_t batch, int32_t frames, void* workspace,
                            size_t workspace_bytes, void* stream) {
    return ctts_waveglow_infer_spk_f32(cfg, packed, mel, z_scaled, nullptr, wave, batch, frames, workspace,
                                       workspace_bytes, stream);
}

int ctts_waveglow_infer_spk_f32(const ctts_waveglow_config* cfg, const void* packed, const float* mel,
                                const float* z_scaled, const int64_t* speaker_ids, float* wave, int32_t batch,
                                int32_t frames, void* workspace, size_t workspace_bytes, void* stream) {
    Plan p; Geom g; Workspace w;
    int rc = make_plan(cfg, p); if (rc) return rc;
    rc = make_geom(p, frames, g); if (rc) return rc;
    CTTS_CHECK_ARG(packed && mel && z_scaled && wave && workspace && batch >= 1, "infer: bad argument");
    carve(p, g, batch, static_cast<float*>(workspace), w);
    if (w.total * sizeof(float) > workspace_bytes) {
        set_error("infer: workspace %zu bytes < required %zu", workspace_bytes, w.total * sizeof(float));
        return CTTS_E_WORKSPACE;
    }
    hipStream_t s = as_stream(stream);
    const float* blob = static_cast<const float*>(packed);
    CTTS_CHECK_HIP(hipMemcpyAsync(w.audio, z_scaled, (size_t)batch * p.c.n_group * g.L * sizeof(float),
                                  hipMemcpyDeviceToDevice, s));
    rc = launch_upsample_squeeze(mel, blob + p.up_w, p.up_mfma ? blob + p.up_wp : nullptr, blob + p.up_b, w.spect, batch, p.c.n_mel_channels, frames,
                                 p.c.win_length, p.c.hop_length, p.c.n_group, g.ld, g.pad, s);
    if (rc) return rc;
    rc = fill_speaker_rows(p, g, blob, speaker_ids, w.spk, batch, s);
    if (rc) return rc;
    rc = run_cond(p, g, blob, w.spect, w.spk, w.h_tmp, w.h_all, batch, s);
    if (rc) return rc;
    for (int k = p.c.n_flows - 1; k >= 0; --k) {
        rc = run_flow(p, g, blob, k, w, w.audio, w.h_all, k == 0 ? wave : nullptr, batch, s);
        if (rc) return rc;
    }
    return CTTS_OK;
}

int ctts_last_gemm_loop(void) { return last_gemm_loop(); }
int ctts_tuning_reload(void) { reload_tuning(); return CTTS_OK; }
int ctts_tuning_flags(void) {
    const Tuning t = tuning();
    return (t.f32_no_glds ? 1 : 0) | (t.no_xcd_pair ? 2 : 0) | (t.bf16_no_wide ? 8 : 0) | (t.bf16_no_pp ? 16 : 0) |
           (t.wf_no_fuse ? 128 : 0) | (t.taco_no_fuse ? 256 : 0) | (t.f32_no_small ? 512 : 0) | (t.f32_force_small ? 1024 : 0) |
           (t.f32_no_splitk ? 2048 : 0) | (t.wf_no_vec_interp ? 4096 : 0) | (t.f32_no_defer_skip ? 8192 : 0) |
           (t.wf_no_region_split ? 16384 : 0) | (t.wf_no_row_queue ? 32768 : 0) | (t.wf_row_queue_min >= 0 ? 65536 : 0) |
           (t.wf_inject_abort ? 131072 : 0) | (t.wf_queue_debug ? 262144 : 0) | (t.f32_no_round_split ? 524288 : 0) |
           (t.bf16_ps ? (1 << 20) : 0) | (t.bf16_no_ps ? (1 << 21) : 0) | (t.taco_poll_delay_set ? (1 << 23) : 0) |
           (t.taco_valu ? (1 << 24) : 0) | (t.up_no_mfma ? (1 << 25) : 0) | (t.f32_no_wn_fold ? (1 << 26) : 0) |
           (t.taco_bg_no_pipe ? (1 << 27) : 0) | (t.f32_no_winograd ? (1 << 28) : 0) | (t.f32_winograd_min >= 0 ? (1 << 29) : 0) |
           (t.f32_winograd_plain ? (1 << 30) : 0) | (t.f32_winograd_fused_min >= 0 ? 4 : 0) | (t.f32_winograd_no_fused ? 32 : 0);
}

int ctts_profile_create(void** handle) {
    CTTS_CHECK_ARG(handle, "profile_create: NULL");
    *handle = new Prof();
    return CTTS_OK;
}

int ctts_profile_bind(void* handle) {
    t_prof = static_cast<Prof*>(handle);
    return CTTS_OK;
}

int ctts_profile_collect(void* handle, int32_t which, int64_t* launches, double* total_ms) {
    Prof* pr = static_cast<Prof*>(handle);
    CTTS_CHECK_ARG(pr && which >= 0 && which < CTTS_PROF_N && launches && total_ms, "profile_collect: bad argument");
    std::lock_guard<std::mutex> lk(pr->mu);
    double tot = 0.0;
    int64_t n = 0;
    for (auto& e : pr->ev[which]) {
        float ms = 0.f;
        CTTS_CHECK_HIP(hipEventSynchronize(e.second));
        CTTS_CHECK_HIP(hipEventElapsedTime(&ms, e.first, e.second));
        tot += ms; ++n;
        pr->pool.push_back(e);
    }
    pr->ev[which].clear();
    *launches = n; *total_ms = tot;
    return CTTS_OK;
}

int ctts_profile_destroy(void* handle) {
    Prof* pr = static_cast<Prof*>(handle);
    if (!pr) return CTTS_OK;
    if (t_prof == pr) t_prof = nullptr;
    {
        std::lock_guard<std::mutex> lk(pr->mu);
        for (int w = 0; w < CTTS_PROF_N; ++w)
            for (auto& e : pr->ev[w]) { (void)hipEventDestroy(e.first); (void)hipEventDestroy(e.second); }
        for (auto& e : pr->pool) { (void)hipEventDestroy(e.first); (void)hipEventDestroy(e.second); }
    }
    delete pr;
    return CTTS_OK;
}

static size_t packed_bf16_bytes_impl(const ctts_waveglow_config* cfg, int P) {
    Plan p; BfPlan q;
    if (make_plan(cfg, p)) return 0;
    if (p.C % BGEMM_KC != 0 || p.H % BGEMM_KC != 0) { set_error("bf16: channels must be multiples of 32"); return 0; }
    make_bf_plan(p, q, P);
    return q.total * sizeof(bf16_t);
}

static int pack_flow_bf16_impl(const ctts_waveglow_config* cfg, int32_t k, const ctts_waveglow_flow_weights* w,
                               void* packed_bf16, void* stream, int P, int f16 = 0) {
    Plan p; BfPlan q;
    int rc = make_plan(cfg, p); if (rc) return rc;
    CTTS_CHECK_ARG(k >= 0 && k < p.c.n_flows && w && packed_bf16, "pack_flow_bf16: bad argument");
    CTTS_CHECK_ARG(p.C % BGEMM_KC == 0 && p.H % BGEMM_KC == 0, "pack_flow_bf16: channels must be multiples of 32");
    CTTS_CHECK_ARG(!f16 || P == 1, "pack_flow: the split form exists for bf16 only");
    make_bf_plan(p, q, P, f16);
    CTTS_CHECK_ARG(q.nch_in <= BGEMM_MAX_CHUNKS && BF_SKIP_GROUP * q.nch_rs <= BGEMM_MAX_CHUNKS,
                   "pack_flow_bf16: K of %d chunks exceeds the chunk table", q.nch_in);
    hipStream_t s = as_stream(stream);
    bf16_t* bb = static_cast<bf16_t*>(packed_bf16);
    const int C = p.C, H = p.H, ks = p.c.kernel_size;
    CTTS_CHECK_ARG(w->cond_w[0] && w->cond_w[1] && p.K0 % BGEMM_KC == 0, "pack_flow_bf16: cond weights / n_mel*n_group %% 32");
    const int sdim = p.c.speaker_embed_dim;
    bf16_t* c0 = bb + q.cond0_A + (size_t)k * q.nch_c0 * BGEMM_KC * BGEMM_BM;
    bf16_t* c1 = bb + q.cond1_A + (size_t)k * q.nch_c1 * BGEMM_KC * BGEMM_BM;
    for (int pi = 0; pi < P; ++pi) {
        const int part = pi == 2;
        if ((rc = launch_pack_a_bf16(c0, w->cond_w[0], 1, q.nch_c0, pi * p.K0, p.K0, BGEMM_EPI_SPLIT, C, H, 0, p.K0 + sdim, 1,
                                     s, 1, 0, part, q.f16))) return rc;
        if (sdim && (rc = launch_pack_a_bf16(c0, w->cond_w[0] + p.K0, 1, q.nch_c0, P * p.K0 + pi * p.S, sdim, BGEMM_EPI_SPLIT,
                                             C, H, 0, p.K0 + sdim, 1, s, 1, 0, part, q.f16))) return rc;
        if ((rc = launch_pack_a_bf16(c1, w->cond_w[1], 1, q.nch_c1, pi * H, H, BGEMM_EPI_SPLIT, C, H, 0, H, 1, s, 1, 0,
                                     part, q.f16))) return rc;
    }
    for (int i = 0; i < p.c.n_layers; ++i) {
        CTTS_CHECK_ARG(w->in_w[i] && w->rs_w[i] && w->cond_w[2] && w->rs_b[i], "pack_flow_bf16: NULL layer %d weights", i);
        const bool last = i == p.c.n_layers - 1;
        const int gi = i / BF_SKIP_GROUP, j = i % BF_SKIP_GROUP;
        for (int pi = 0; pi < P; ++pi) {
            const int part = pi == 2;
            for (int t = 0; t < ks; ++t)
                if ((rc = launch_pack_a_bf16(bb + q.in_A[k][i], w->in_w[i] + t, p.mb_in, q.nch_in, 0, C, BGEMM_EPI_GATE, C,
                                             2 * C, 0, (long long)C * ks, ks, s, ks * P, t * P + pi, part, q.f16))) return rc;
            if ((rc = launch_pack_a_bf16(bb + q.in_A[k][i], w->cond_w[2], p.mb_in, q.nch_in, ks * P * C + pi * H, H,
                                         BGEMM_EPI_GATE, C, 2 * C, (long long)2 * C * i, H, 1, s, 1, 0, part, q.f16))) return rc;
            if (!last && (rc = launch_pack_a_bf16(bb + q.rs_A[k][i], w->rs_w[i], q.mb_c, q.nch_rs, pi * C, C, BGEMM_EPI_SPLIT,
                                                  C, C, 0, C, 1, s, 1, 0, part, q.f16))) return rc;
            if ((rc = launch_pack_a_bf16(bb + q.skip_A[k][gi], w->rs_w[i], q.mb_c, q.group_layers(gi, p.c.n_layers) * q.nch_rs,
                                         (j * P + pi) * C, C, BGEMM_EPI_SPLIT, C, C, last ? 0 : C, C, 1, s, 1, 0,
                                         part, q.f16))) return rc;
        }
        hipLaunchKernelGGL(skip_bias_kernel, dim3((2 * q.mb_c * BGEMM_BM + 255) / 256), dim3(256), 0, s,
                           reinterpret_cast<float*>(bb + q.skip_b[k]), w->rs_b[i] + (last ? 0 : C), C,
                           2 * q.mb_c * BGEMM_BM, i == 0 ? 1 : 0);
        CTTS_CHECK_LAUNCH("skip_bias");
    }
    return CTTS_OK;
}

static size_t workspace_bf16_bytes_impl(const ctts_waveglow_config* cfg, int32_t batch, int32_t frames, int P) {
    Plan p; Geom g; BfWs w;
    if (make_plan(cfg, p) || make_geom(p, frames, g) || batch < 1) return 0;
    carve_bf(p, g, batch, nullptr, w, P);
    return w.total_bytes;
}

static int infer_bf16_impl(const ctts_waveglow_config* cfg, const void* packed, const void* packed_bf16, const float* mel,
                           const float* z_scaled, const int64_t* speaker_ids, float* wave, int32_t batch, int32_t frames,
                           void* workspace, size_t workspace_bytes, void* stream, int P, int f16 = 0) {
    Plan p; Geom g; BfWs w; BfPlan q;
    int rc = make_plan(cfg, p); if (rc) return rc;
    rc = make_geom(p, frames, g); if (rc) return rc;
    CTTS_CHECK_ARG(packed && packed_bf16 && mel && z_scaled && wave && workspace && batch >= 1, "infer_bf16: bad argument");
    CTTS_CHECK_ARG(p.C % BGEMM_KC == 0 && p.C <= 512, "infer_bf16: n_channels=%d (multiple of 32, <= 512)", p.C);
    CTTS_CHECK_ARG(p.c.n_group <= 8, "infer_bf16: n_group=%d (the reduced-precision flow boundaries hold <= 8 channels; fp32 takes 16)", p.c.n_group);
    make_bf_plan(p, q, P, f16);
    carve_bf(p, g, batch, static_cast<char*>(workspace), w, P);
    if (w.total_bytes > workspace_bytes) {
        set_error("infer_bf16: workspace %zu bytes < required %zu", workspace_bytes, w.total_bytes);
        return CTTS_E_WORKSPACE;
    }
    hipStream_t s = as_stream(stream);
    const float* blob = static_cast<const float*>(packed);
    const bf16_t* bblob = static_cast<const bf16_t*>(packed_bf16);
    CTTS_CHECK_HIP(hipMemcpyAsync(w.audio, z_scaled, (size_t)batch * p.c.n_group * g.L * sizeof(float),
                                  hipMemcpyDeviceToDevice, s));
    rc = launch_upsample_squeeze(mel, blob + p.up_w, p.up_mfma ? blob + p.up_wp : nullptr, blob + p.up_b, w.spect, batch, p.c.n_mel_channels, frames,
                                 p.c.win_length, p.c.hop_length, p.c.n_group, g.ld, g.pad, s);
    if (rc) return rc;
    hipLaunchKernelGGL(cvt_f32_to_k8_kernel, dim3((g.ld + 255) / 256, p.K0 / 8, batch), dim3(256), 0, s, w.spect,
                       w.spect_bf, p.K0, g.ld, w.spect_lo, q.f16);
    CTTS_CHECK_LAUNCH("cvt_f32_to_k8");
    if (p.S) {
        if ((rc = fill_speaker_rows(p, g, blob, speaker_ids, w.spk, batch, s))) return rc;
        hipLaunchKernelGGL(cvt_f32_to_k8_kernel, dim3((g.ld + 255) / 256, p.c.n_flows * p.S / 8, batch), dim3(256), 0, s,
                           w.spk, w.spk_bf, p.c.n_flows * p.S, g.ld, w.spk_lo, q.f16);
        CTTS_CHECK_LAUNCH("cvt_f32_to_k8(speaker rows)");
    }
    {
        const long long hstride = (long long)p.c.n_flows * p.H * g.ld;
        BGemmArgs a{};
        a.f16 = q.f16;
        a.ld = g.ld; a.pad = g.pad; a.L = g.L; a.ntiles = g.ntiles; a.batch = batch;
        a.A = bblob + q.cond0_A; a.bias = blob + p.cond0_b;
        a.nch_total = q.nch_c0; a.MB = p.c.n_flows; a.M = p.c.n_flows * BGEMM_BM;
        int ns = push_segs(a, 0, P, w.spect_bf, w.spect_lo, (long long)p.K0 * g.ld, p.K0 / BGEMM_KC, 0, 0);
        if (p.S) ns = push_segs(a, ns, P, w.spk_bf, w.spk_lo, (long long)p.c.n_flows * p.S * g.ld, p.S / BGEMM_KC, 0, p.S);
        a.nseg = ns;
// ... 84 lines not shown
```

cookietts_amd/csrc/waveglow_kernels.h:

```cpp
#pragma once

#include "common.h"
#include "gemm_f32.h"

namespace ctts {

int launch_fold_weightnorm(const float* v, const float* g, float* w, int out_ch, int fan, hipStream_t s);
int launch_pack_a(float* dst, const float* src, int bm, int MB, int nch_total, int k_off, int ksrc, int epi, int C, int M,
                  long long src_row_off, long long src_row_stride, int src_k_stride, hipStream_t s, int k_group = 1,
                  int k_member = 0);
int launch_pack_bias(float* dst, int bm, int MB, const float* src0, long long off0, const float* src1, long long off1,
                     int epi, int C, int M, hipStream_t s);
bool upsample_mfma_shape(int n_mel, int win, int hop, int G);
int launch_upsample_pack_mfma(const float* W, float* Wp, hipStream_t s);
int launch_upsample_squeeze(const float* mel, const float* W, const float* Wp, const float* bias, float* spect, int batch,
                            int n_mel, int F, int win, int hop, int G, int ld, int pad, hipStream_t s);
int launch_wn_start(const float* audio, const float* Ws, const float* bs, float* x, int batch, int C, int G,
                    int ch_off, int n_half, int L, int ld, int pad, hipStream_t s);
struct CouplingForward {
    float* log_s;
    long long ls_bstride;
    double* part;
    long long part_bstride;
};
constexpr int FWD_SUMSQ_CHUNK = 4096;
int launch_flow_tail(const float* out, float* audio, float* wave, const float* Wend, const float* bend,
                     const float* Winv, int batch, int C, int G, int ch_off, int n_half, int L, int ld, int pad,
                     hipStream_t s, const CouplingForward* fwd = nullptr);
int launch_flow_head_forward(const float* W, const float* wave, float* z, int batch, int G, int ch_off, int n_rem, int L,
                             hipStream_t s);
int launch_sumsq_partials(const float* z, double* part, int batch, long long n_item, int nblk, hipStream_t s);
int launch_sum_partials(const double* part, long long part_bstride, long long part_kstride, int n, double* out, int out_bstride,
                        int nk, int batch, hipStream_t s);

constexpr int FOLD_ROWS = 16;
int launch_fold_in0(const float* in_w, const float* Ws, const float* bs, float* dst, int C, int n_half, int ks, hipStream_t s);
int launch_fold_skend(const float* const* rs_w, const float* const* rs_b, const float* Wend, const float* bend, float* Wf,
                      float* bf, int C, int n_layers, int n_half, hipStream_t s);
int launch_wn_start_ones(const float* audio, float* a16, int batch, int G, int ch_off, int n_half, int L, int ld, int pad,
                         hipStream_t s);
int launch_skip_end(const float* act, long long act_stride, int nl, const float* Wf, float* acc, bool first, bool tail,
                    const float* bf, const float* Winv, float* audio, float* wave, int batch, int C, int G, int ch_off,
                    int n_half, int L, int ld, int pad, hipStream_t s, const CouplingForward* fwd = nullptr);

int launch_winograd_g(const float* in_w, float* dense, int rows, int C, hipStream_t s);
int launch_winograd_transform(const float* x, long long x_bstride, const float* h2, long long h_bstride, float* V, float* Hc,
                              int batch, int C, int H, int d, int L, int Lp, int ld, int pad, int ldp, int ncols, bool cond_rows,
                              bool vec_d2, hipStream_t s);

}
```

cookietts_amd/csrc/waveglow_kernels.hip:

```cpp
#include "waveglow_kernels.h"
#include "tuning.h"

namespace ctts {

namespace {

__global__ __launch_bounds__(256) void fold_weightnorm_kernel(const float* __restrict__ v,
                                                              const float* __restrict__ g,
                                                              float* __restrict__ w, int fan) {
    __shared__ float red[4];
    const int o = blockIdx.x;
    const float* vr = v + (size_t)o * fan;
    float s = 0.f;
    for (int i = threadIdx.x; i < fan; i += 256) { const float x = vr[i]; s = fmaf(x, x, s); }
#pragma unroll
    for (int off = 32; off > 0; off >>= 1) s += __shfl_xor(s, off);
    if ((threadIdx.x & 63) == 0) red[threadIdx.x >> 6] = s;
    __syncthreads();
    const float tot = red[0] + red[1] + red[2] + red[3];
    const float scale = g[o] / sqrtf(tot);
    float* wr = w + (size_t)o * fan;
    for (int i = threadIdx.x; i < fan; i += 256) wr[i] = vr[i] * scale;
}

// ... 367 lines not shown
            m.x = fmaf(w, a[j].x, m.x); m.y = fmaf(w, a[j].y, m.y);
            m.z = fmaf(w, a[j].z, m.z); m.w = fmaf(w, a[j].w, m.w);
        }
        *reinterpret_cast<float4*>(zb + (size_t)i * L) = m;
    }
}

__device__ __forceinline__ double block_sum_f64(double s, double* red) {
#pragma unroll
    for (int off = 32; off > 0; off >>= 1) s += __shfl_xor(s, off);
    if ((threadIdx.x & 63) == 0) red[threadIdx.x >> 6] = s;
    __syncthreads();
    return ((red[0] + red[1]) + red[2]) + red[3];
}

__global__ __launch_bounds__(256) void sumsq_partials_kernel(const float* __restrict__ z, double* __restrict__ part,
                                                             long long n_item, int nblk) {
    __shared__ double red[4];
    const int b = blockIdx.y;
    const float* zb = z + (size_t)b * n_item;
    double s = 0.0;
#pragma unroll
    for (int r = 0; r < FWD_SUMSQ_CHUNK / 1024; ++r) {
        const long long i = (long long)blockIdx.x * FWD_SUMSQ_CHUNK + (r * 256 + threadIdx.x) * 4;
        if (i < n_item) {
            const float4 v = *reinterpret_cast<const float4*>(zb + i);
            s += ((double)v.x * (double)v.x + (double)v.y * (double)v.y) + ((double)v.z * (double)v.z + (double)v.w * (double)v.w);
        }
    }
    s = block_sum_f64(s, red);
    if (threadIdx.x == 0) part[(size_t)b * nblk + blockIdx.x] = s;
}

__global__ __launch_bounds__(64) void sum_partials_kernel(const double* __restrict__ part, long long part_bstride,
                                                          long long part_kstride, int n, double* __restrict__ out,
                                                          int out_bstride) {
    const int k = blockIdx.x, b = blockIdx.y;
    const double* p = part + (size_t)b * part_bstride + (size_t)k * part_kstride;
    double s = 0.0;
    for (int i = threadIdx.x; i < n; i += 64) s += p[i];
#pragma unroll
    for (int off = 32; off > 0; off >>= 1) s += __shfl_xor(s, off);
    if (threadIdx.x == 0) out[(size_t)b * out_bstride + k] = s;
}



__global__ __launch_bounds__(256) void fold_in0_kernel(const float* __restrict__ in_w, const float* __restrict__ Ws,
                                                       const float* __restrict__ bs, float* __restrict__ dst, int C, int H,
                                                       int ks, int rows) {
    const int idx = blockIdx.x * 256 + threadIdx.x;
    if (idx >= rows * FOLD_ROWS * ks) return;
    const int t = idx % ks, r = (idx / ks) % FOLD_ROWS, o = idx / (ks * FOLD_ROWS);
    double acc = 0.0;
    if (r <= H) {
        const float* wr = in_w + (size_t)o * C * ks + t;
        for (int c = 0; c < C; ++c) acc += (double)wr[(size_t)c * ks] * (double)(r < H ? Ws[c * H + r] : bs[c]);
    }
    dst[idx] = (float)acc;
}

__global__ __launch_bounds__(256) void fold_skend_w_kernel(const float* __restrict__ Wend, const float* __restrict__ rs_w,
                                                           float* __restrict__ Wf, int C, int E, int row_off) {
    const int idx = blockIdx.x * 256 + threadIdx.x;
    if (idx >= C * E) return;
    const int e = idx % E, c = idx / E;
    double acc = 0.0;
    for (int m = 0; m < C; ++m) acc += (double)Wend[(size_t)e * C + m] * (double)rs_w[(size_t)(row_off + m) * C + c];
    Wf[idx] = (float)acc;
}

struct SkipBiasPtrs { const float* p[12]; int row_off[12]; };

__global__ __launch_bounds__(64) void fold_skend_b_kernel(const float* __restrict__ Wend, const float* __restrict__ bend,
                                                          SkipBiasPtrs sb, int n_layers, float* __restrict__ bf, int C, int E) {
    const int e = threadIdx.x;
    if (e >= E) return;
    double acc = 0.0;
    for (int m = 0; m < C; ++m) {
        double bm = 0.0;
        for (int i = 0; i < n_layers; ++i) bm += (double)sb.p[i][sb.row_off[i] + m];
        acc += (double)Wend[(size_t)e * C + m] * bm;
    }
    bf[e] = (float)(acc + (double)bend[e]);
}


__global__ __launch_bounds__(256) void winograd_g_kernel(const float* __restrict__ in_w, float* __restrict__ dense, int n) {
    const int idx = blockIdx.x * 256 + threadIdx.x;
    if (idx >= n) return;
    const double w0 = in_w[(size_t)idx * 3], w1 = in_w[(size_t)idx * 3 + 1], w2 = in_w[(size_t)idx * 3 + 2];
    dense[idx] = (float)((w0 + w1 + w2) * 0.5);
    dense[(size_t)n + idx] = (float)((w0 - w1 + w2) * 0.5);
    dense[2 * (size_t)n + idx] = -in_w[(size_t)idx * 3 + 2];
}

template <int MODE>
__global__ __launch_bounds__(256) void winograd_transform_kernel(const float* __restrict__ x, long long x_bstride,
                                                                 const float* __restrict__ h2, long long h_bstride,
                                                                 float* __restrict__ V, float* __restrict__ Hc, int C, int H,
                                                                 int d, int L, int Lp, int ld, int pad, int ldp, int ncols) {
    const int j4 = (blockIdx.x * 256 + threadIdx.x) * 4;
    if (j4 >= ncols) return;
    const int row = blockIdx.y, b = blockIdx.z, B = gridDim.z;
    const bool is_x = row < C;
    const float* src = is_x ? x + (size_t)b * x_bstride + (size_t)row * ld + pad
                            : h2 + (size_t)b * h_bstride + (size_t)(row - C) * ld + pad;
    float4 vm = {0.f, 0.f, 0.f, 0.f}, v0 = vm, v1 = vm, v2 = vm;
    [[maybe_unused]] auto ld4 = [&](int t) { return (t >= 0 && t < L) ? *reinterpret_cast<const float4*>(src + t) : make_float4(0.f, 0.f, 0.f, 0.f); };
    if constexpr (MODE == 1) {
        if (j4 < Lp) {
            const int te = (j4 / d) * 2 * d + j4 % d;
            if (is_x) { vm = ld4(te - d); v2 = ld4(te + 2 * d); }
            v0 = ld4(te); v1 = ld4(te + d);
        }
    } else if constexpr (MODE == 2) {
        if (j4 < Lp) {
            const int t0 = 2 * j4;
            const float4 q = ld4(t0), r = ld4(t0 + 4);
            float4 p = vm, u = vm;
            if (is_x) { p = ld4(t0 - 4); u = ld4(t0 + 8); }
            const bool hi = j4 + 2 < Lp;
            vm = make_float4(p.z, p.w, hi ? q.z : 0.f, hi ? q.w : 0.f);
            v0 = make_float4(q.x, q.y, hi ? r.x : 0.f, hi ? r.y : 0.f);
            v1 = make_float4(q.z, q.w, hi ? r.z : 0.f, hi ? r.w : 0.f);
            v2 = make_float4(r.x, r.y, hi ? u.x : 0.f, hi ? u.y : 0.f);
        }
    } else {
        float am[4], a0[4], a1[4], a2[4];
#pragma unroll
        for (int e = 0; e < 4; ++e) {
            const int j = j4 + e;
            const int te = (j / d) * 2 * d + j % d;
            const bool in = j < Lp;
            auto ld1 = [&](int t) { return (in && t >= 0 && t < L) ? src[t] : 0.f; };
            am[e] = is_x ? ld1(te - d) : 0.f; a2[e] = is_x ? ld1(te + 2 * d) : 0.f;
            a0[e] = ld1(te); a1[e] = ld1(te + d);
        }
        vm = make_float4(am[0], am[1], am[2], am[3]); v0 = make_float4(a0[0], a0[1], a0[2], a0[3]);
        v1 = make_float4(a1[0], a1[1], a1[2], a1[3]); v2 = make_float4(a2[0], a2[1], a2[2], a2[3]);
    }
    if (is_x) {
        const size_t plane = (size_t)B * C * ldp;
        float* o = V + ((size_t)b * C + row) * ldp + j4;
        *reinterpret_cast<float4*>(o) = make_float4(vm.x - v1.x, vm.y - v1.y, vm.z - v1.z, vm.w - v1.w);
        *reinterpret_cast<float4*>(o + plane) = make_float4(v0.x + v1.x, v0.y + v1.y, v0.z + v1.z, v0.w + v1.w);
        *reinterpret_cast<float4*>(o + 2 * plane) = make_float4(v1.x - v0.x, v1.y - v0.y, v1.z - v0.z, v1.w - v0.w);
        *reinterpret_cast<float4*>(o + 3 * plane) = make_float4(v0.x - v2.x, v0.y - v2.y, v0.z - v2.z, v0.w - v2.w);
    } else {
        const size_t plane = (size_t)B * H * ldp;
        float* o = Hc + ((size_t)b * H + (row - C)) * ldp + j4;
        *reinterpret_cast<float4*>(o) = v0;
        *reinterpret_cast<float4*>(o + plane) = v1;
    }
}

template <int H>
__global__ __launch_bounds__(256) void wn_start_ones_kernel(const float* __restrict__ audio, float* __restrict__ a16, int G,
                                                            int ch_off, int L, int ld, int pad) {
    const int col = (blockIdx.x * 256 + threadIdx.x) * 4;
    const int b = blockIdx.z;
    if (col >= ld) return;
    const int n = col - pad;
    const bool in = n >= 0 && n < L;
    float* dst = a16 + (size_t)b * FOLD_ROWS * ld + col;
#pragma unroll
    for (int r = 0; r < FOLD_ROWS; ++r) {
        float4 v = make_float4(0.f, 0.f, 0.f, 0.f);
        if (in && r < H) v = *reinterpret_cast<const float4*>(audio + ((size_t)b * G + ch_off + r) * L + n);
        else if (in && r == H) v = make_float4(1.f, 1.f, 1.f, 1.f);
        *reinterpret_cast<float4*>(dst + (size_t)r * ld) = v;
    }
}

enum { SKEND_ACC = 0, SKEND_TAIL = 1, SKEND_FWD = 2 };
template <int H, int TAIL>
__global__ __launch_bounds__(256) void skip_end_kernel(const float* __restrict__ act, long long act_stride, int nl,
                                                       const float* __restrict__ Wf, float* __restrict__ acc, int first,
                                                       const float* __restrict__ bf, const float* __restrict__ Winv,
                                                       float* __restrict__ audio, float* __restrict__ wave,
                                                       int C, int G, int ch_off, int L, int ld, int pad, CouplingForward fw) {
    constexpr int E = 2 * H;
    constexpr int NG = E <= 4 ? 8 : E <= 8 ? 4 : 2;
    __shared__ __attribute__((aligned(16))) float part[3][E][256];
    __shared__ float sWinv[E * E];
    const int lane = threadIdx.x & 63;
    const int wv = threadIdx.x >> 6;
    const int b = blockIdx.y;
    const int n = blockIdx.x * 256 + lane * 4;
    if (TAIL == SKEND_TAIL && threadIdx.x < E * E) sWinv[threadIdx.x] = Winv[threadIdx.x];
    float4 e[E];
#pragma unroll
    for (int j = 0; j < E; ++j) e[j] = make_float4(0.f, 0.f, 0.f, 0.f);
    const int cq = C / 4;
    const int cbeg = __builtin_amdgcn_readfirstlane(wv * cq);
    for (int l = 0; l < nl; ++l) {
        const float* ob = act + (size_t)l * act_stride + (size_t)b * C * ld + pad + n;
        const float* wl = Wf + (size_t)l * C * E;
        for (int c = cbeg; c < cbeg + cq; c += NG) {
            float4 v[NG];
#pragma unroll
            for (int k = 0; k < NG; ++k) v[k] = *reinterpret_cast<const float4*>(ob + (size_t)(c + k) * ld);
#pragma unroll
            for (int k = 0; k < NG; ++k)
#pragma unroll
                for (int j = 0; j < E; ++j) {
                    const float w = wl[(c + k) * E + j];
                    e[j].x = fmaf(w, v[k].x, e[j].x); e[j].y = fmaf(w, v[k].y, e[j].y);
                    e[j].z = fmaf(w, v[k].z, e[j].z); e[j].w = fmaf(w, v[k].w, e[j].w);
                }
        }
    }
    if (wv > 0) {
#pragma unroll
        for (int j = 0; j < E; ++j) *reinterpret_cast<float4*>(&part[wv - 1][j][lane * 4]) = e[j];
    }
    __syncthreads();
    if (wv != 0 || (TAIL != SKEND_FWD && n >= L)) return;
    float* ab = acc + (size_t)b * E * ld + pad + n;
#pragma unroll
    for (int j = 0; j < E; ++j) {
#pragma unroll
        for (int q = 0; q < 3; ++q) {
            const float4 pv = *reinterpret_cast<const float4*>(&part[q][j][lane * 4]);
            e[j].x += pv.x; e[j].y += pv.y; e[j].z += pv.z; e[j].w += pv.w;
        }
        if (!first) {
            const float4 pv = *reinterpret_cast<const float4*>(ab + (size_t)j * ld);
            e[j].x += pv.x; e[j].y += pv.y; e[j].z += pv.z; e[j].w += pv.w;
        }
    }
    if constexpr (TAIL == SKEND_ACC) {
#pragma unroll
        for (int j = 0; j < E; ++j) *reinterpret_cast<float4*>(ab + (size_t)j * ld) = e[j];
    } else {
#pragma unroll
        for (int j = 0; j < E; ++j) {
            const float bj = bf[j];
            e[j].x += bj; e[j].y += bj; e[j].z += bj; e[j].w += bj;
        }
        if constexpr (TAIL == SKEND_FWD) coupling_forward<H>(e, audio, fw, b, G, ch_off, L, n);
        else coupling_tail<H>(e, sWinv, audio, wave, b, G, ch_off, L, n);
    }
}

}


int launch_fold_weightnorm(const float* v, const float* g, float* w, int out_ch, int fan, hipStream_t s) {
    CTTS_CHECK_ARG(out_ch > 0 && fan > 0, "fold_weightnorm: out_ch=%d fan=%d", out_ch, fan);
    hipLaunchKernelGGL(fold_weightnorm_kernel, dim3(out_ch), dim3(256), 0, s, v, g, w, fan);
    CTTS_CHECK_LAUNCH("fold_weightnorm");
    return CTTS_OK;
}

int launch_pack_a(float* dst, const float* src, int bm, int MB, int nch_total, int k_off, int ksrc, int epi, int C, int M,
                  long long src_row_off, long long src_row_stride, int src_k_stride, hipStream_t s, int k_group,
                  int k_member) {
    CTTS_CHECK_ARG(k_off >= 0 && ksrc > 0 && k_off + ksrc * (k_group > 1 ? k_group : 1) <= nch_total * GEMM_KC,
                   "pack_a: k range");
    CTTS_CHECK_ARG(k_group <= 1 || (ksrc % GEMM_KC == 0 && k_member >= 0 && k_member < k_group), "pack_a: k group");
    hipLaunchKernelGGL(pack_a_kernel, dim3(ksrc, MB), dim3(256), 0, s, dst, src, bm, nch_total, k_off, ksrc, epi, C, M,
                       src_row_off, src_row_stride, src_k_stride, k_group, k_member);
    CTTS_CHECK_LAUNCH("pack_a");
    return CTTS_OK;
}

int launch_pack_bias(float* dst, int bm, int MB, const float* src0, long long off0, const float* src1, long long off1,
                     int epi, int C, int M, hipStream_t s) {
    hipLaunchKernelGGL(pack_bias_kernel, dim3(MB), dim3(256), 0, s, dst, bm, src0, off0, src1, off1, epi, C, M);
    CTTS_CHECK_LAUNCH("pack_bias");
    return CTTS_OK;
}

bool upsample_mfma_shape(int n_mel, int win, int hop, int G) {
    return n_mel == UM_NMEL && hop == UM_HOP && win == UM_HOP * UM_TAPS && G == UM_G;
}

int launch_upsample_pack_mfma(const float* W, float* Wp, hipStream_t s) {
    const size_t n = (size_t)UM_NMEL * UM_NMEL * UM_HOP * UM_TAPS;
    hipLaunchKernelGGL(upsample_pack_mfma_kernel, dim3((unsigned)((n + 255) / 256)), dim3(256), 0, s, W, Wp);
    CTTS_CHECK_LAUNCH("upsample_pack_mfma");
    return CTTS_OK;
}

int launch_upsample_squeeze(const float* mel, const float* W, const float* Wp, const float* bias, float* spect, int batch,
                            int n_mel, int F, int win, int hop, int G, int ld, int pad, hipStream_t s) {
    CTTS_CHECK_ARG(win % hop == 0 && hop % G == 0, "upsample_squeeze: win %d hop %d n_group %d", win, hop, G);
    if (Wp && upsample_mfma_shape(n_mel, win, hop, G) && ld % 4 == 0 && pad % 4 == 0 && (reinterpret_cast<uintptr_t>(spect) & 15) == 0 &&
        !tuning().up_no_mfma) {
        const int nchunks = (F + UM_CHUNK_MAX - 1) / UM_CHUNK_MAX;
        const int chunk = ((F + nchunks - 1) / nchunks + 15) / 16 * 16;
        const int srow = (chunk + 31) / 32 * 32 + 4;
        const int lds = UM_NMEL * srow * (int)sizeof(float);
        if (lds > 64 * 1024)
            CTTS_CHECK_HIP(hipFuncSetAttribute(reinterpret_cast<const void*>(upsample_squeeze_mfma_kernel),
                                               hipFuncAttributeMaxDynamicSharedMemorySize, UM_NMEL * (UM_CHUNK_MAX + 4) * (int)sizeof(float)));
        hipLaunchKernelGGL(upsample_squeeze_mfma_kernel, dim3(UM_NMEL, (unsigned)(batch * nchunks)), dim3(512), lds, s, mel, Wp, bias,
                           spect, F, chunk, nchunks, srow, ld, pad);
        CTTS_CHECK_LAUNCH("upsample_squeeze_mfma");
        return CTTS_OK;
    }
    if (hop != 256 || G != 8) {
        dim3 ggrid((unsigned)(((long long)F * hop + 255) / 256), n_mel, batch);
        hipLaunchKernelGGL(upsample_squeeze_generic_kernel, ggrid, dim3(256), 0, s, mel, W, bias, spect, n_mel, F, win, hop, G, ld, pad);
        CTTS_CHECK_LAUNCH("upsample_squeeze_generic");
        return CTTS_OK;
    }
    const int taps = win / hop;
    const size_t smem = ((size_t)n_mel * (UP_UQ + taps - 1) + (size_t)(UP_UO / 2) * G * (UP_UQ * (hop / G) + 8)) * sizeof(float);
    CTTS_CHECK_ARG(smem <= 64 * 1024, "upsample_squeeze: LDS %zu", smem);
    dim3 grid((F + UP_UQ - 1) / UP_UQ, (n_mel + UP_UO - 1) / UP_UO, batch);
    hipLaunchKernelGGL((upsample_squeeze_kernel<256, 8>), grid, dim3(256), smem, s, mel, W, bias, spect, n_mel, F,
                       win, ld, pad);
    CTTS_CHECK_LAUNCH("upsample_squeeze");
    return CTTS_OK;
}

int launch_wn_start(const float* audio, const float* Ws, const float* bs, float* x, int batch, int C, int G,
                    int ch_off, int n_half, int L, int ld, int pad, hipStream_t s) {
    CTTS_CHECK_ARG(L % 4 == 0, "wn_start: L=%d not a multiple of 4", L);
    dim3 grid((L / 4 + 255) / 256, (C + 31) / 32, batch);
#define CTTS_START_CASE(H)                                                                                     \
    case H:                                                                                                    \
        hipLaunchKernelGGL(wn_start_kernel<H>, grid, dim3(256), 0, s, audio, Ws, bs, x, C, G, ch_off, L, ld,   \
                           pad);                                                                               \
        break;
    switch (n_half) {
        CTTS_START_CASE(1) CTTS_START_CASE(2) CTTS_START_CASE(3) CTTS_START_CASE(4)
        CTTS_START_CASE(5) CTTS_START_CASE(6) CTTS_START_CASE(7) CTTS_START_CASE(8)
        default:
            set_error("wn_start: n_half=%d unsupported (1..8)", n_half);
            return CTTS_E_ARG;
    }
#undef CTTS_START_CASE
    CTTS_CHECK_LAUNCH("wn_start");
    return CTTS_OK;
}

int launch_flow_tail(const float* out, float* audio, float* wave, const float* Wend, const float* bend,
                     const float* Winv, int batch, int C, int G, int ch_off, int n_half, int L, int ld, int pad,
                     hipStream_t s, const CouplingForward* fwd) {
    CTTS_CHECK_ARG(L % 4 == 0 && C % 4 == 0, "flow_tail: L=%d C=%d", L, C);
    CTTS_CHECK_ARG(fwd == nullptr || (fwd->part != nullptr && wave == nullptr), "flow_tail: forward direction needs the partial sums");
    const CouplingForward fw = fwd ? *fwd : CouplingForward{};
    CTTS_CHECK_ARG(wave == nullptr || (ch_off == 0 && 2 * n_half == G && G % 4 == 0),
                   "flow_tail: un-squeeze needs the full group (ch_off=%d n_half=%d G=%d)", ch_off, n_half, G);
    dim3 grid((L + 255) / 256, batch);
#define CTTS_TAIL_CASE(H)                                                                                       \
    case H:                                                                                                     \
        if (fwd)                                                                                                \
            hipLaunchKernelGGL((flow_tail_kernel<H, true>), grid, dim3(256), 0, s, out, audio, wave, Wend, bend, Winv, C, G, \
                               ch_off, L, ld, pad, fw);                                                         \
        else                                                                                                    \
            hipLaunchKernelGGL((flow_tail_kernel<H, false>), grid, dim3(256), 0, s, out, audio, wave, Wend, bend, Winv, C, G, \
                               ch_off, L, ld, pad, fw);                                                         \
        break;
    switch (n_half) {
        CTTS_TAIL_CASE(1) CTTS_TAIL_CASE(2) CTTS_TAIL_CASE(3) CTTS_TAIL_CASE(4)
        CTTS_TAIL_CASE(5) CTTS_TAIL_CASE(6) CTTS_TAIL_CASE(7) CTTS_TAIL_CASE(8)
        default:
            set_error("flow_tail: n_half=%d unsupported (1..8)", n_half);
            return CTTS_E_ARG;
    }
#undef CTTS_TAIL_CASE
    CTTS_CHECK_LAUNCH("flow_tail");
    return CTTS_OK;
}

int launch_fold_in0(const float* in_w, const float* Ws, const float* bs, float* dst, int C, int n_half, int ks, hipStream_t s) {
    CTTS_CHECK_ARG(n_half >= 1 && n_half < FOLD_ROWS, "fold_in0: n_half=%d", n_half);
    const int n = 2 * C * FOLD_ROWS * ks;
    hipLaunchKernelGGL(fold_in0_kernel, dim3((n + 255) / 256), dim3(256), 0, s, in_w, Ws, bs, dst, C, n_half, ks, 2 * C);
    CTTS_CHECK_LAUNCH("fold_in0");
    return CTTS_OK;
}

int launch_fold_skend(const float* const* rs_w, const float* const* rs_b, const float* Wend, const float* bend, float* Wf,
                      float* bf, int C, int n_layers, int n_half, hipStream_t s) {
    const int E = 2 * n_half;
    CTTS_CHECK_ARG(n_layers >= 1 && n_layers <= 12 && E <= 64, "fold_skend: n_layers=%d n_half=%d", n_layers, n_half);
    SkipBiasPtrs sb{};
    for (int i = 0; i < n_layers; ++i) {
        CTTS_CHECK_ARG(rs_w[i] && rs_b[i], "fold_skend: NULL layer %d weights", i);
        const int row_off = i < n_layers - 1 ? C : 0;
        sb.p[i] = rs_b[i];
        sb.row_off[i] = row_off;
        hipLaunchKernelGGL(fold_skend_w_kernel, dim3((C * E + 255) / 256), dim3(256), 0, s, Wend, rs_w[i], Wf + (size_t)i * C * E,
                           C, E, row_off);
    }
    hipLaunchKernelGGL(fold_skend_b_kernel, dim3(1), dim3(64), 0, s, Wend, bend, sb, n_layers, bf, C, E);
    CTTS_CHECK_LAUNCH("fold_skend");
    return CTTS_OK;
}

int launch_winograd_g(const float* in_w, float* dense, int rows, int C, hipStream_t s) {
    const int n = rows * C;
    hipLaunchKernelGGL(winograd_g_kernel, dim3((n + 255) / 256), dim3(256), 0, s, in_w, dense, n);
    CTTS_CHECK_LAUNCH("winograd_g");
    return CTTS_OK;
}

int launch_winograd_transform(const float* x, long long x_bstride, const float* h2, long long h_bstride, float* V, float* Hc,
                              int batch, int C, int H, int d, int L, int Lp, int ld, int pad, int ldp, int ncols, bool cond_rows,
                              bool vec_d2, hipStream_t s) {
    CTTS_CHECK_ARG(d >= 1 && Lp % d == 0 && (long long)Lp * 2 >= L && Lp <= ncols && ncols <= ldp && ncols % 4 == 0 && ldp % 4 == 0 &&
                       ld % 4 == 0 && pad % 4 == 0 && pad + L <= ld,
                   "winograd_transform: d=%d L=%d Lp=%d ncols=%d ldp=%d ld=%d pad=%d", d, L, Lp, ncols, ldp, ld, pad);
    dim3 grid((ncols / 4 + 255) / 256, cond_rows ? C + H : C, batch);
    if (d % 4 == 0 && L % 4 == 0)
        hipLaunchKernelGGL(winograd_transform_kernel<1>, grid, dim3(256), 0, s, x, x_bstride, h2, h_bstride, V, Hc, C, H, d, L, Lp,
                           ld, pad, ldp, ncols);
    else if (d == 2 && L % 4 == 0 && vec_d2)
        hipLaunchKernelGGL(winograd_transform_kernel<2>, grid, dim3(256), 0, s, x, x_bstride, h2, h_bstride, V, Hc, C, H, d, L, Lp,
                           ld, pad, ldp, ncols);
    else
        hipLaunchKernelGGL(winograd_transform_kernel<0>, grid, dim3(256), 0, s, x, x_bstride, h2, h_bstride, V, Hc, C, H, d, L, Lp,
                           ld, pad, ldp, ncols);
    CTTS_CHECK_LAUNCH("winograd_transform");
    return CTTS_OK;
}

int launch_wn_start_ones(const float* audio, float* a16, int batch, int G, int ch_off, int n_half, int L, int ld, int pad,
                         hipStream_t s) {
    CTTS_CHECK_ARG(L % 4 == 0 && ld % 4 == 0 && pad % 4 == 0, "wn_start_ones: L=%d ld=%d pad=%d", L, ld, pad);
    dim3 grid((ld / 4 + 255) / 256, 1, batch);
#define CTTS_ONES_CASE(H)                                                                                     \
    case H:                                                                                                   \
        hipLaunchKernelGGL(wn_start_ones_kernel<H>, grid, dim3(256), 0, s, audio, a16, G, ch_off, L, ld, pad); \
        break;
    switch (n_half) {
        CTTS_ONES_CASE(1) CTTS_ONES_CASE(2) CTTS_ONES_CASE(3) CTTS_ONES_CASE(4)
        CTTS_ONES_CASE(5) CTTS_ONES_CASE(6) CTTS_ONES_CASE(7) CTTS_ONES_CASE(8)
        default:
            set_error("wn_start_ones: n_half=%d unsupported (1..8)", n_half);
            return CTTS_E_ARG;
    }
#undef CTTS_ONES_CASE
    CTTS_CHECK_LAUNCH("wn_start_ones");
    return CTTS_OK;
}

int launch_skip_end(const float* act, long long act_stride, int nl, const float* Wf, float* acc, bool first, bool tail,
                    const float* bf, const float* Winv, float* audio, float* wave, int batch, int C, int G, int ch_off,
                    int n_half, int L, int ld, int pad, hipStream_t s, const CouplingForward* fwd) {
    CTTS_CHECK_ARG(fwd == nullptr || (tail && fwd->part != nullptr && wave == nullptr), "skip_end: forward direction on the tail pass only");
    const CouplingForward fw = fwd ? *fwd : CouplingForward{};
    CTTS_CHECK_ARG(L % 4 == 0 && C % 32 == 0 && ld % 4 == 0 && pad % 4 == 0 && nl >= 1, "skip_end: L=%d C=%d nl=%d", L, C, nl);
    CTTS_CHECK_ARG(acc != nullptr || (first && tail), "skip_end: a group after the first needs the accumulator");
    CTTS_CHECK_ARG(!tail || wave == nullptr || (ch_off == 0 && 2 * n_half == G && G % 4 == 0),
                   "skip_end: un-squeeze needs the full group (ch_off=%d n_half=%d G=%d)", ch_off, n_half, G);
    dim3 grid((L + 255) / 256, batch);
    const int fi = first ? 1 : 0;
#define CTTS_SKEND_CASE(H)                                                                                                \
    case H:                                                                                                               \
        if (fwd)                                                                                                          \
            hipLaunchKernelGGL((skip_end_kernel<H, SKEND_FWD>), grid, dim3(256), 0, s, act, act_stride, nl, Wf, acc, fi, bf, Winv, \
                               audio, wave, C, G, ch_off, L, ld, pad, fw);                                                \
        else if (tail)                                                                                                    \
            hipLaunchKernelGGL((skip_end_kernel<H, SKEND_TAIL>), grid, dim3(256), 0, s, act, act_stride, nl, Wf, acc, fi, bf, Winv, \
                               audio, wave, C, G, ch_off, L, ld, pad, fw);                                                \
        else                                                                                                              \
            hipLaunchKernelGGL((skip_end_kernel<H, SKEND_ACC>), grid, dim3(256), 0, s, act, act_stride, nl, Wf, acc, fi, bf, Winv, \
                               audio, wave, C, G, ch_off, L, ld, pad, fw);                                                \
        break;
    switch (n_half) {
        CTTS_SKEND_CASE(1) CTTS_SKEND_CASE(2) CTTS_SKEND_CASE(3) CTTS_SKEND_CASE(4)
        CTTS_SKEND_CASE(5) CTTS_SKEND_CASE(6) CTTS_SKEND_CASE(7) CTTS_SKEND_CASE(8)
        default:
            set_error("skip_end: n_half=%d unsupported (1..8)", n_half);
            return CTTS_E_ARG;
    }
#undef CTTS_SKEND_CASE
    CTTS_CHECK_LAUNCH("skip_end");
    return CTTS_OK;
}

int launch_flow_head_forward(const float* W, const float* wave, float* z, int batch, int G, int ch_off, int n_rem, int L,
                             hipStream_t s) {
    CTTS_CHECK_ARG(L % 4 == 0 && n_rem >= 2 && n_rem % 2 == 0 && ch_off >= 0 && ch_off + n_rem == G,
                   "flow_head_forward: L=%d n_rem=%d ch_off=%d G=%d", L, n_rem, ch_off, G);
    CTTS_CHECK_ARG(wave == nullptr || (ch_off == 0 && G % 4 == 0), "flow_head_forward: the squeeze needs the full group (ch_off=%d G=%d)",
                   ch_off, G);
    dim3 grid((L / 4 + 255) / 256, batch);
#define CTTS_HEAD_LAUNCH(EE, SQ) \
    hipLaunchKernelGGL((flow_head_forward_kernel<EE, SQ>), grid, dim3(256), 0, s, W, wave, z, G, ch_off, L)
#define CTTS_HEAD_CASE(EE)             \
    case EE:                           \
        CTTS_HEAD_LAUNCH(EE, false);   \
        break;
#define CTTS_HEAD_CASE_SQ(EE)                                                       \
    case EE:                                                                        \
        if (wave) CTTS_HEAD_LAUNCH(EE, true); else CTTS_HEAD_LAUNCH(EE, false);     \
        break;
    switch (n_rem) {
        CTTS_HEAD_CASE(2) CTTS_HEAD_CASE_SQ(4) CTTS_HEAD_CASE(6) CTTS_HEAD_CASE_SQ(8)
        CTTS_HEAD_CASE(10) CTTS_HEAD_CASE_SQ(12) CTTS_HEAD_CASE(14) CTTS_HEAD_CASE_SQ(16)
        default:
            set_error("flow_head_forward: n_rem=%d unsupported (2..16, even)", n_rem);
            return CTTS_E_ARG;
    }
#undef CTTS_HEAD_CASE_SQ
#undef CTTS_HEAD_CASE
#undef CTTS_HEAD_LAUNCH
    CTTS_CHECK_LAUNCH("flow_head_forward");
    return CTTS_OK;
}

int launch_sumsq_partials(const float* z, double* part, int batch, long long n_item, int nblk, hipStream_t s) {
    CTTS_CHECK_ARG(n_item > 0 && n_item % 4 == 0 && (long long)nblk * FWD_SUMSQ_CHUNK >= n_item, "sumsq_partials: n=%lld nblk=%d",
                   n_item, nblk);
    hipLaunchKernelGGL(sumsq_partials_kernel, dim3(nblk, batch), dim3(256), 0, s, z, part, n_item, nblk);
    CTTS_CHECK_LAUNCH("sumsq_partials");
    return CTTS_OK;
}

int launch_sum_partials(const double* part, long long part_bstride, long long part_kstride, int n, double* out, int out_bstride,
                        int nk, int batch, hipStream_t s) {
    CTTS_CHECK_ARG(n >= 1 && nk >= 1, "sum_partials: n=%d nk=%d", n, nk);
    hipLaunchKernelGGL(sum_partials_kernel, dim3(nk, batch), dim3(64), 0, s, part, part_bstride, part_kstride, n, out, out_bstride);
    CTTS_CHECK_LAUNCH("sum_partials");
    return CTTS_OK;
}

}
```

cookietts_amd/csrc/wn_winograd_layer.h:

```cpp
#pragma once

#include "common.h"
#include "gemm_f32.h"

namespace ctts {

constexpr int WNWG_MAX_CHUNKS = 320;

struct WnWinogradLayerArgs {
    const float *A_T2, *A_T3, *A_e, *A_o, *bias;
    const float* V; long long vplane;
    const float* Hc; long long hplane;
    const float* h2; long long h_bstride;
    float* act; long long act_bstride;
    int C, H, batch;
    int ldp, Lp, ntiles;
    int d, L, ld, pad;
    int in_place;
    int kt, kt_total, b0, col0;
};

bool wn_winograd_layer_supported(int C, int H);
int launch_wn_winograd_layer(const WnWinogradLayerArgs& a, hipStream_t stream);

}
```

cookietts_amd/csrc/wn_winograd_layer.hip:

```cpp
#include "wn_winograd_layer.h"
#include "tuning.h"

namespace ctts {

typedef float wg_f32x16 __attribute__((ext_vector_type(16)));

namespace {

__device__ __forceinline__ float wg_sigmoid(float u) {
    return __builtin_amdgcn_rcpf(1.0f + __builtin_amdgcn_exp2f(u * -1.4426950408889634f));
}
__device__ __forceinline__ float wg_tanh(float u) {
    return 1.0f - 2.0f * __builtin_amdgcn_rcpf(1.0f + __builtin_amdgcn_exp2f(u * 2.8853900817779268f));
}

}

template <int NT>
__global__ __launch_bounds__(256, 2) void wn_winograd_layer_f32_kernel(const WnWinogradLayerArgs a) {
    constexpr int BN = 64 * NT;
    constexpr int A_ST = GEMM_KC * 128;
    constexpr int STG = A_ST + GEMM_KC * BN;
    constexpr int TAB = 3 * STG;
    constexpr int BIAS = TAB + 4 * WNWG_MAX_CHUNKS;
    constexpr int UPR = BN / 4;
    constexpr int RPP = 64 / UPR;
    __shared__ __attribute__((aligned(16))) float lds[BIAS + 128];

    const int t = threadIdx.x;
    const int lane = t & 63;
    const int wave = __builtin_amdgcn_readfirstlane(t >> 6);
    const int wm = wave >> 1, wn = wave & 1;
    const int l31 = lane & 31, lhi = lane >> 5;

    const int ncb = a.C >> 6;
    const int jx = blockIdx.x >> 3;
    const int cb = jx % ncb;
    const int gt = (jx / ncb) * 8 + (blockIdx.x & 7);
    if (gt >= a.kt_total) return;
    const int b = a.b0 + gt / a.kt;
    const int n0 = a.col0 + (gt % a.kt) * BN;

    const int n1 = a.C / GEMM_KC, n2 = (a.C + a.H) / GEMM_KC;
    const int c_e = 2 * n1, c_o = 2 * n1 + n2, nch = 2 * n1 + 2 * n2;

    const int mb_t = (64 * cb) >> 8, loc_t = (64 * cb) & 255;
    const int mb_s = (a.C + 64 * cb) >> 8, loc_s = (a.C + 64 * cb) & 255;
    {
        uint4* tab = reinterpret_cast<uint4*>(lds + TAB);
        for (int c = t; c < nch; c += 256) {
            const float *ap, *bp;
            if (c < c_e) {
                const int ph = c >= n1, loc = c - ph * n1;
                ap = (ph ? a.A_T3 : a.A_T2) + ((size_t)mb_t * n1 + loc) * (GEMM_KC * 256) + loc_t;
                bp = a.V + (1 + ph) * a.vplane + ((size_t)b * a.C + (size_t)loc * GEMM_KC) * a.ldp + n0;
            } else {
                const int ph = c >= c_o, loc = c - c_e - ph * n2;
                ap = (ph ? a.A_o : a.A_e) + ((size_t)(cb >> 1) * n2 + loc) * (GEMM_KC * 256) + (cb & 1) * 128;
                if (loc < n1) bp = a.V + (ph ? 3 : 0) * a.vplane + ((size_t)b * a.C + (size_t)loc * GEMM_KC) * a.ldp + n0;
                else if (a.in_place) bp = a.h2 + (size_t)b * a.h_bstride + (size_t)(loc - n1) * GEMM_KC * a.ld;
                else bp = a.Hc + ph * a.hplane + ((size_t)b * a.H + (size_t)(loc - n1) * GEMM_KC) * a.ldp + n0;
            }
            const unsigned long long ua = reinterpret_cast<unsigned long long>(ap), ub = reinterpret_cast<unsigned long long>(bp);
            tab[c] = make_uint4((unsigned)ua, (unsigned)(ua >> 32), (unsigned)ub, (unsigned)(ub >> 32));
        }
        if (t < 128) lds[BIAS + t] = a.bias[cb * 128 + t];
    }

    unsigned offa_g[2], offa_s[2], offb[NT], offb_e[NT], offb_o[NT];
    {
        const int col = (lane & 31) * 4;
        const long long delta = ((long long)(mb_s - mb_t) * n1) * (GEMM_KC * 256) + (loc_s - loc_t);
#pragma unroll
        for (int j = 0; j < 2; ++j) {
            const int krow = 2 * (wave + 4 * j) + (lane >> 5);
            offa_g[j] = (unsigned)((krow * 256 + col) * 4);
            offa_s[j] = (unsigned)((krow * 256 + (col < 64 ? (long long)col : col - 64 + delta)) * 4);
        }
        const int bcol = (lane % UPR) * 4;
#pragma unroll
        for (int j = 0; j < NT; ++j) {
            const int krow = (wave + 4 * j) * RPP + lane / UPR;
            offb[j] = (unsigned)(((size_t)krow * a.ldp + bcol) * 4);
            offb_e[j] = offb_o[j] = 0;
            if (a.in_place) {
                const int q = n0 + bcol;
                const int te = (q / a.d) * (2 * a.d) + q % a.d;
                const int lim = (a.ld - a.pad - 4) & ~3;
                offb_e[j] = (unsigned)(((size_t)krow * a.ld + a.pad + min(te, lim)) * 4);
                offb_o[j] = (unsigned)(((size_t)krow * a.ld + a.pad + min(te + a.d, lim)) * 4);
            }
        }
    }
    const int m_e0 = a.in_place ? c_e + n1 : 0x7fffffff, m_e1 = c_o;
    const int m_o0 = a.in_place ? c_o + n1 : 0x7fffffff;

    wg_f32x16 S[2][NT], D[2][NT];
#pragma unroll
    for (int i = 0; i < 2; ++i)
#pragma unroll
        for (int j = 0; j < NT; ++j)
#pragma unroll
            for (int r = 0; r < 16; ++r) { S[i][j][r] = 0.0f; D[i][j][r] = 0.0f; }
    __syncthreads();

    typedef __attribute__((address_space(3))) float* lds_fptr;
    typedef const __attribute__((address_space(1))) float* gfloat_ptr;
    typedef const __attribute__((address_space(1))) char* gbyte_ptr;
    const uint4* ctab = reinterpret_cast<const uint4*>(lds + TAB);
#define WNWG_ADDR(buf, c)                                                                                   \
    lds_fptr la_ = (lds_fptr)(lds + (buf) * STG + wave * 256);                                              \
    const uint4 e_ = ctab[c];                                                                               \
    const bool as_ = (c) < c_e;                                       \
    const bool me_ = (c) >= m_e0 && (c) < m_e1, mo_ = (c) >= m_o0;
#define WNWG_BASES()                                                                                        \
    const gbyte_ptr ac_ = reinterpret_cast<gbyte_ptr>(                                                      \
        ((unsigned long long)(unsigned)__builtin_amdgcn_readfirstlane((int)e_.y) << 32) |                   \
        (unsigned)__builtin_amdgcn_readfirstlane((int)e_.x));                                               \
    const gbyte_ptr bp_ = reinterpret_cast<gbyte_ptr>(                                                      \
        ((unsigned long long)(unsigned)__builtin_amdgcn_readfirstlane((int)e_.w) << 32) |                   \
        (unsigned)__builtin_amdgcn_readfirstlane((int)e_.z));
#define WNWG_PIECE(p)                                                                                       \
    do {                                                                                                    \
        if constexpr ((p) < 2) {                                                                            \
            unsigned o_ = as_ ? offa_s[(p)] : offa_g[(p)];                                                  \
            asm volatile("" : "+v"(o_));                                                                    \
            __builtin_amdgcn_global_load_lds((gfloat_ptr)(ac_ + o_), la_ + 1024 * (p), 16, 0, 0);           \
        } else if constexpr ((p) < 2 + NT) {                                                                \
            unsigned o_ = me_ ? offb_e[(p) - 2] : mo_ ? offb_o[(p) - 2] : offb[(p) - 2];                     \
            asm volatile("" : "+v"(o_));                                                                    \
            __builtin_amdgcn_global_load_lds((gfloat_ptr)(bp_ + o_), la_ + A_ST + 1024 * ((p) - 2), 16, 0, 0); \
        }                                                                                                   \
    } while (0)
#define WNWG_WAIT()                                                                                         \
    do {                                                                                                    \
        if constexpr (NT == 2) asm volatile("s_waitcnt vmcnt(4)" ::: "memory");                             \
        else asm volatile("s_waitcnt vmcnt(3)" ::: "memory");                                               \
    } while (0)

    {
        { WNWG_ADDR(0, 0) WNWG_BASES() WNWG_PIECE(0); WNWG_PIECE(1); WNWG_PIECE(2); WNWG_PIECE(3); }
        { WNWG_ADDR(1, 1) WNWG_BASES() WNWG_PIECE(0); WNWG_PIECE(1); WNWG_PIECE(2); WNWG_PIECE(3); }
        WNWG_WAIT();
        __builtin_amdgcn_s_barrier();
        __builtin_amdgcn_sched_barrier(0);
    }

    int cur = 0;
#define WNWG_READ_FRAGS(ks)                                                                                 \
    _Pragma("unroll") for (int mt = 0; mt < 2; ++mt) av[ks][mt] = As[(2 * (ks) + lhi) * 128 + mt * 64];     \
    _Pragma("unroll") for (int nt = 0; nt < NT; ++nt) bv[ks][nt] = Bs[(2 * (ks) + lhi) * BN + nt * 32];
#define WNWG_MFMA(X, ks)                                                                                    \
    _Pragma("unroll") for (int mt = 0; mt < 2; ++mt)                                                        \
        _Pragma("unroll") for (int nt = 0; nt < NT; ++nt)                                                   \
            X[mt][nt] = __builtin_amdgcn_mfma_f32_32x32x2f32(av[ks][mt], bv[ks][nt], X[mt][nt], 0, 0, 0);
#define WNWG_REGION(X, ks, p)                                                                               \
    __builtin_amdgcn_sched_barrier(0);                                                                      \
    if constexpr ((ks) + 1 < GEMM_KC / 2) { WNWG_READ_FRAGS((ks) + 1) }                                     \
    WNWG_MFMA(X, ks)                                                                                        \
    WNWG_PIECE(p);
#define WNWG_CHUNK(X)                                                                                       \
    {                                                                                                       \
        const float* As = lds + cur * STG + wm * 32 + l31;                                                  \
        const float* Bs = lds + cur * STG + A_ST + wn * (32 * NT) + l31;                                    \
        float av[GEMM_KC / 2][2], bv[GEMM_KC / 2][NT];                                                      \
        const int nb = cur >= 1 ? cur - 1 : 2;                \
        const int cn = ch + 2 < nch ? ch + 2 : nch - 1;                                                     \
        WNWG_ADDR(nb, cn)                                                                                   \
        WNWG_READ_FRAGS(0)                                                                                  \
        __builtin_amdgcn_sched_barrier(0);                                                                  \
        WNWG_BASES()                                                                                        \
        WNWG_REGION(X, 0, 0) WNWG_REGION(X, 1, 1) WNWG_REGION(X, 2, 2) WNWG_REGION(X, 3, 3)                 \
        WNWG_REGION(X, 4, 4) WNWG_REGION(X, 5, 4) WNWG_REGION(X, 6, 4) WNWG_REGION(X, 7, 4)                 \
        __builtin_amdgcn_sched_barrier(0);                                                                  \
        WNWG_WAIT();                                         \
        __builtin_amdgcn_s_barrier();                                                                       \
        __builtin_amdgcn_sched_barrier(0);                                                                  \
        cur = cur == 2 ? 0 : cur + 1;                                                                       \
    }

    float* dst = a.act + (size_t)b * a.act_bstride + (size_t)(cb * 64 + wm * 32) * a.ld + a.pad;
    const float* bias = lds + BIAS + wm * 32;
#define WNWG_GATE(X, par)                                                                                   \
    _Pragma("unroll") for (int nt = 0; nt < NT; ++nt) {                                                     \
        const int n = n0 + wn * (32 * NT) + nt * 32 + l31;                                                  \
        const int ns = (n / a.d) * (2 * a.d) + n % a.d + (par) * a.d;                                       \
        if (n < a.Lp && ns < a.L) {                                                                         \
            _Pragma("unroll") for (int r = 0; r < 16; ++r) {                                                \
                const int row = (r & 3) + 8 * (r >> 2) + 4 * lhi;                                           \
                const float u0 = X[0][nt][r] + bias[row];                                                   \
                const float u1 = X[1][nt][r] + bias[64 + row];                                              \
                dst[(size_t)row * a.ld + ns] = wg_tanh(u0) * wg_sigmoid(u1);                                \
            }                                                                                               \
        }                                                                                                   \
    }

    int ch = 0;
    for (; ch < n1; ++ch) WNWG_CHUNK(S)
    for (; ch < c_e; ++ch) WNWG_CHUNK(D)
#pragma unroll
    for (int i = 0; i < 2; ++i)
#pragma unroll
        for (int j = 0; j < NT; ++j)
#pragma unroll
            for (int r = 0; r < 16; ++r) {
                const float s = S[i][j][r], dd = D[i][j][r];
                S[i][j][r] = s + dd;
                D[i][j][r] = s - dd;
            }
    for (; ch < c_o; ++ch) WNWG_CHUNK(S)
    WNWG_GATE(S, 0)
    for (; ch < nch; ++ch) WNWG_CHUNK(D)
    asm volatile("s_waitcnt vmcnt(0)" ::: "memory");
    __builtin_amdgcn_s_barrier();
    WNWG_GATE(D, 1)
#undef WNWG_GATE
#undef WNWG_CHUNK
#undef WNWG_REGION
#undef WNWG_MFMA
#undef WNWG_READ_FRAGS
#undef WNWG_WAIT
#undef WNWG_PIECE
#undef WNWG_BASES
#undef WNWG_ADDR
}

bool wn_winograd_layer_supported(int C, int H) {
    return C >= 128 && C % 128 == 0 && H > 0 && H % GEMM_KC == 0 && 2 * (C / GEMM_KC) + 2 * ((C + H) / GEMM_KC) <= WNWG_MAX_CHUNKS;
}

namespace {
template <int NT>
int launch_wnwg_shape(WnWinogradLayerArgs a, int kt, long long kt_total, hipStream_t stream) {
    a.kt = kt;
    a.kt_total = (int)kt_total;
    const long long blocks = 8ll * (a.C / 64) * ((kt_total + 7) / 8);
    CTTS_CHECK_ARG(blocks > 0 && blocks < (1ll << 31) && kt_total < (1ll << 31), "wn_winograd_layer: grid %lld", blocks);
    hipLaunchKernelGGL((wn_winograd_layer_f32_kernel<NT>), dim3((unsigned)blocks), dim3(256), 0, stream, a);
    CTTS_CHECK_LAUNCH("wn_winograd_layer");
    return CTTS_OK;
}
}

int launch_wn_winograd_layer(const WnWinogradLayerArgs& a_in, hipStream_t stream) {
    WnWinogradLayerArgs a = a_in;
    CTTS_CHECK_ARG(wn_winograd_layer_supported(a.C, a.H), "wn_winograd_layer: C=%d H=%d", a.C, a.H);
    CTTS_CHECK_ARG(a.A_T2 && a.A_T3 && a.A_e && a.A_o && a.bias && a.V && a.act && a.batch >= 1, "wn_winograd_layer: operand not set");
    CTTS_CHECK_ARG(a.d >= 1 && a.L >= 1 && a.Lp >= 1 && a.ntiles >= 1 && a.Lp <= a.ntiles * 128 && a.ntiles * 128 <= a.ldp && a.ldp % 4 == 0 &&
                       a.ld % 4 == 0 && a.pad >= 0 && a.pad % 4 == 0 && a.L + a.pad <= a.ld,
                   "wn_winograd_layer: geometry d=%d L=%d Lp=%d ntiles=%d ldp=%d ld=%d pad=%d", a.d, a.L, a.Lp, a.ntiles, a.ldp, a.ld, a.pad);
    CTTS_CHECK_ARG(a.in_place ? (a.h2 && a.d % 4 == 0 && a.ld - a.pad >= 4 && a.h_bstride % 4 == 0 && reinterpret_cast<uintptr_t>(a.h2) % 16 == 0)
                              : a.Hc != nullptr,
                   "wn_winograd_layer: cond rows (in_place=%d d=%d)", a.in_place, a.d);
    a.b0 = 0;
    a.col0 = 0;
    const Tuning tn = tuning();
    const int ncb = a.C / 64;
    const long long slots = 2ll * wf_row_cus();
    const int kt_narrow = (a.Lp + 63) / 64;
    long long tiles = (long long)a.ntiles * a.batch;
    if (!tn.f32_no_small && (tn.f32_force_small || ncb * tiles < 2 * slots)) return launch_wnwg_shape<1>(a, kt_narrow, (long long)kt_narrow * a.batch, stream);
    if (!tn.f32_no_round_split && !tn.f32_no_small) {
        const long long rounds = ncb * tiles / slots;
        const long long rem_tiles = (ncb * tiles - rounds * slots + ncb - 1) / ncb;
        if (rounds >= 2 && rem_tiles > 0 && rem_tiles * ncb <= slots * 3 / 10 && rem_tiles < a.ntiles &&
            (long long)(a.ntiles - rem_tiles) * 128 < a.Lp) {
            WnWinogradLayerArgs r = a;
            r.b0 = a.batch - 1;
            r.col0 = (int)(a.ntiles - rem_tiles) * 128;
            const int kt = (a.Lp - r.col0 + 63) / 64;
            if (int rc = launch_wnwg_shape<1>(r, kt, kt, stream)) return rc;
            tiles -= rem_tiles;
        }
    }
    return launch_wnwg_shape<2>(a, a.ntiles, tiles, stream);
}

}
```

Baseline: 3.514 million samples/s.

## Add Winograd F(4,3) path for fused WN in-layer dilated conv

Adds an F(4,3) Winograd form for the WaveNet dilated conv alongside the existing F(2,3) one. It brings a new input transform into six planes, precomputed transformed weights packed for the GEMM, and a fused layer kernel that runs four product accumulators and applies the inverse transform before the gated activation. It engages by default on long sequences when the fused path is active. The aim is fewer multiplies per output than F(2,3), at the cost of more transform traffic, extra registers, larger workspace and weaker fp32 numerical conditioning.

```diff
diff --git a/cookietts_amd/_lib.py b/cookietts_amd/_lib.py
--- a/cookietts_amd/_lib.py
+++ b/cookietts_amd/_lib.py
@@ -381,10 +381,11 @@
 
 
 TUNING_BITS = {"CTTS_F32_NO_GLDS": 0, "CTTS_GEMM_NO_XCD_PAIR": 1, "CTTS_F32_WINOGRAD_FUSED_MIN": 2, "CTTS_BF16_NO_WIDE": 3, "CTTS_BF16_NO_PP": 4,
-               "CTTS_F32_WINOGRAD_NO_FUSED": 5, "CTTS_WF_NO_FUSE": 7,
+               "CTTS_F32_WINOGRAD_NO_FUSED": 5, "CTTS_F32_WINOGRAD_F43_MIN": 6, "CTTS_WF_NO_FUSE": 7,
                "CTTS_TACO_NO_FUSE": 8, "CTTS_F32_NO_SMALL": 9, "CTTS_F32_FORCE_SMALL": 10, "CTTS_F32_NO_SPLITK": 11, "CTTS_WF_NO_VEC_INTERP": 12,
                "CTTS_F32_NO_DEFER_SKIP": 13, "CTTS_WF_NO_REGION_SPLIT": 14, "CTTS_WF_NO_ROW_QUEUE": 15, "CTTS_WF_ROW_QUEUE_MIN": 16,
                "CTTS_WF_INJECT_ABORT": 17, "CTTS_WF_QUEUE_DEBUG": 18, "CTTS_F32_NO_ROUND_SPLIT": 19, "CTTS_BF16_PS": 20, "CTTS_BF16_NO_PS": 21,
+               "CTTS_F32_WINOGRAD_NO_F43": 22,
                "CTTS_TACO_POLL_DELAY": 23, "CTTS_TACO_VALU": 24, "CTTS_UP_NO_MFMA": 25, "CTTS_F32_NO_WN_FOLD": 26, "CTTS_TACO_BG_NO_PIPE": 27,
                "CTTS_F32_NO_WINOGRAD": 28, "CTTS_F32_WINOGRAD_MIN": 29, "CTTS_F32_WINOGRAD_PLAIN": 30}
 
diff --git a/cookietts_amd/csrc/gemm_f32.hip b/cookietts_amd/csrc/gemm_f32.hip
--- a/cookietts_amd/csrc/gemm_f32.hip
+++ b/cookietts_amd/csrc/gemm_f32.hip
@@ -740,6 +740,8 @@
     g_tune.f32_winograd_plain = on("CTTS_F32_WINOGRAD_PLAIN");
     g_tune.f32_winograd_fused_min = num("CTTS_F32_WINOGRAD_FUSED_MIN", -1);
     g_tune.f32_winograd_no_fused = on("CTTS_F32_WINOGRAD_NO_FUSED");
+    g_tune.f32_winograd_f43_min = num("CTTS_F32_WINOGRAD_F43_MIN", -1);
+    g_tune.f32_winograd_no_f43 = on("CTTS_F32_WINOGRAD_NO_F43");
     g_tune_loaded = true;
 }
 }
diff --git a/cookietts_amd/csrc/tuning.h b/cookietts_amd/csrc/tuning.h
--- a/cookietts_amd/csrc/tuning.h
+++ b/cookietts_amd/csrc/tuning.h
@@ -27,6 +27,8 @@
     int f32_winograd_min;
     bool f32_winograd_plain;
     int f32_winograd_fused_min;
+    int f32_winograd_f43_min;
+    bool f32_winograd_no_f43;
     bool f32_winograd_no_fused;
     bool wf_no_region_split;
     bool wf_no_row_queue;
diff --git a/cookietts_amd/csrc/waveglow_api.hip b/cookietts_amd/csrc/waveglow_api.hip
--- a/cookietts_amd/csrc/waveglow_api.hip
+++ b/cookietts_amd/csrc/waveglow_api.hip
@@ -44,6 +44,7 @@
         size_t in0f_w, in0f_A, skend_W, skend_b;
         std::vector<size_t> wg_T2_A, wg_T3_A, wg_e_A, wg_o_A;
         size_t wg_dense;
+        std::vector<size_t> wq_U_A[4], wq_e_A, wq_o_A;
     };
     std::vector<Flow> fl;
     size_t total;
@@ -132,7 +133,13 @@
             f.wg_e_A.push_back(take((size_t)p.mb_in * (p.nch_rs + p.nch1h) * A_TILE));
             f.wg_o_A.push_back(take((size_t)p.mb_in * (p.nch_rs + p.nch1h) * A_TILE));
         }
-        f.wg_dense = take((size_t)3 * 2 * p.C * p.C);
+        const bool f43 = wn_winograd_layer_f43_supported(p.C, p.H);
+        for (int i = 0; f43 && i < c.n_layers; ++i) {
+            for (auto& u : f.wq_U_A) u.push_back(take((size_t)p.mb_in * p.nch_rs * A_TILE));
+            f.wq_e_A.push_back(take((size_t)p.mb_in * (p.nch_rs + p.nch1h) * A_TILE));
+            f.wq_o_A.push_back(take((size_t)p.mb_in * (p.nch_rs + p.nch1h) * A_TILE));
+        }
+        f.wg_dense = take((size_t)(f43 ? 6 : 3) * 2 * p.C * p.C);
     }
     p.total = o;
     return CTTS_OK;
@@ -162,6 +169,16 @@
     for (int i = 0; i < p.c.n_layers; ++i) nt = std::max(nt, pair_geom(g, i).ntiles);
     return nt * GEMM_BN;
 }
+PairGeom quad_geom(const Geom& g, int layer) {
+    const int d = 1 << layer;
+    const int Lq = (g.L + 4 * d - 1) / (4 * d) * d;
+    return {d, Lq, (Lq + 63) / 64};
+}
+int quad_ld(const Plan& p, const Geom& g) {
+    int nt = 0;
+    for (int i = 0; i < p.c.n_layers; ++i) nt = std::max(nt, quad_geom(g, i).ntiles);
+    return nt * 64;
+}
 constexpr long long WINOGRAD_MIN_COLS = 28800;
 bool winograd_engages(const Plan& p, const Geom& g) {
     const Tuning t = tuning();
@@ -178,13 +195,21 @@
     return winograd_engages(p, g) && (long long)g.L >= min_cols;
 }
 
+constexpr long long WINOGRAD_F43_MIN_COLS = 28800;
+bool winograd_f43_engages(const Plan& p, const Geom& g) {
+    const Tuning t = tuning();
+    if (t.f32_winograd_no_f43 || !wn_winograd_layer_f43_supported(p.C, p.H) || !gemm_f32_dma_staged(p.nch_rs + p.nch1h)) return false;
+    const long long min_cols = t.f32_winograd_f43_min >= 0 ? t.f32_winograd_f43_min : WINOGRAD_F43_MIN_COLS;
+    return winograd_fused_engages(p, g) && (long long)g.L >= min_cols;
+}
+
 struct Workspace {
     float *audio, *spect, *spk, *h_tmp, *h_all, *x, *act, *out;
     float* act_all;
     float* a16;
     float* skend;
     float *wgV, *wgT, *wgH;
-    int ldp;
+    int ldp, ldq;
     size_t total;
 };
 
@@ -204,12 +229,13 @@
     w.a16 = take(B * FOLD_ROWS * g.ld);
     w.skend = take(B * p.c.n_group * g.ld);
     w.wgV = w.wgT = w.wgH = nullptr;
-    w.ldp = 0;
+    w.ldp = w.ldq = 0;
     if (winograd_engages(p, g)) {
         w.ldp = pair_ld(p, g);
-        w.wgV = take((size_t)4 * B * p.C * w.ldp);
+        w.ldq = winograd_f43_engages(p, g) ? quad_ld(p, g) : 0;
+        w.wgV = take(std::max((size_t)4 * w.ldp, (size_t)6 * w.ldq) * B * p.C);
         w.wgT = take((size_t)2 * B * 2 * p.C * w.ldp);
-        w.wgH = take((size_t)2 * B * p.H * w.ldp);
+        w.wgH = take(std::max((size_t)2 * w.ldp, (size_t)4 * w.ldq) * B * p.H);
     }
     w.total = o;
 }
@@ -298,7 +324,7 @@
 }
 
 struct WnFold { float* a16; float* skend; float* audio; float* wave; };
-struct WnWinograd { float* V; float* T; float* Hc; int ldp; };
+struct WnWinograd { float* V; float* T; float* Hc; int ldp; int ldq; };
 
 int run_in_layer_winograd(const Plan& p, const Geom& g, const float* blob, int k, int i, const float* x, const float* h_all,
                           float* act, const WnWinograd& wg, int batch, hipStream_t s) {
@@ -311,6 +337,27 @@
     const bool in_place = lean && pg.d % 4 == 0;
     const bool fused = lean && winograd_fused_engages(p, g);
     const float* h2 = h_all + (size_t)k * H * g.ld;
+    if (fused && wg.ldq > 0 && winograd_f43_engages(p, g)) {
+        const PairGeom qg = quad_geom(g, i);
+        const int ldq = wg.ldq;
+        int rc = launch_winograd_transform_quad(x, (long long)C * g.ld, h2, hstride, wg.V, wg.Hc, batch, C, H, qg.d, g.L, qg.Lp, g.ld, g.pad,
+                                                ldq, qg.ntiles * 64, !in_place, s);
+        if (rc) return rc;
+        WnWinogradLayerArgs w{};
+        w.form = WNWG_F43;
+        w.A_T2 = blob + f.wq_U_A[0][i]; w.A_T3 = blob + f.wq_U_A[1][i]; w.A_T4 = blob + f.wq_U_A[2][i]; w.A_T5 = blob + f.wq_U_A[3][i];
+        w.A_e = blob + f.wq_e_A[i]; w.A_o = blob + f.wq_o_A[i];
+        w.bias = blob + f.in_b[i];
+        w.V = wg.V; w.vplane = (long long)batch * C * ldq;
+        w.Hc = wg.Hc; w.hplane = (long long)batch * H * ldq;
+        w.h2 = h2; w.h_bstride = hstride;
+        w.act = act; w.act_bstride = (long long)C * g.ld;
+        w.C = C; w.H = H; w.batch = batch;
+        w.ldp = ldq; w.Lp = qg.Lp; w.ntiles = qg.ntiles;
+        w.d = qg.d; w.L = g.L; w.ld = g.ld; w.pad = g.pad;
+        w.in_place = in_place;
+        return launch_wn_winograd_layer(w, s);
+    }
     int rc = launch_winograd_transform(x, (long long)C * g.ld, h2, hstride, wg.V, wg.Hc, batch, C, H, pg.d, g.L, pg.Lp, g.ld, g.pad,
                                        ldp, pg.ntiles * GEMM_BN, !in_place, lean, s);
     if (rc) return rc;
@@ -491,7 +538,7 @@
              float* wave, int batch, hipStream_t s, const CouplingForward* fwd = nullptr) {
     const Tuning t = tuning();
     const bool folded = !t.f32_no_wn_fold && !t.f32_no_defer_skip;
-    const WnWinograd wg{w.wgV, w.wgT, w.wgH, w.ldp};
+    const WnWinograd wg{w.wgV, w.wgT, w.wgH, w.ldp, w.ldq};
     const WnFold fw{w.a16, w.skend, audio, wave};
     int rc = run_wn_stack(p, g, blob, k, audio, h_all, w.x, w.act, w.out, batch, s, w.act_all, folded ? &fw : nullptr,
                           w.wgV ? &wg : nullptr, fwd);
@@ -955,6 +1002,18 @@
             if ((rc = launch_pack_a(A, w->cond_w[2], GEMM_BM, p.mb_in, p.nch_rs + p.nch1h, C, H, GEMM_EPI_GATE, C, 2 * C,
                                     (long long)2 * C * i, H, 1, s))) return rc;
     }
+    for (int i = 0; i < (f.wq_e_A.empty() ? 0 : p.c.n_layers); ++i) {
+        float* dense = blob + f.wg_dense;
+        const size_t dn = (size_t)2 * C * C;
+        if ((rc = launch_winograd_g43(w->in_w[i], dense, 2 * C, C, s))) return rc;
+        for (int j = 0; j < 4; ++j)
+            if ((rc = launch_pack_a(blob + f.wq_U_A[j][i], dense + (1 + j) * dn, GEMM_BM, p.mb_in, p.nch_rs, 0, C, GEMM_EPI_SPLIT, C, 2 * C, 0, C, 1, s))) return rc;
+        if ((rc = launch_pack_a(blob + f.wq_e_A[i], dense, GEMM_BM, p.mb_in, p.nch_rs + p.nch1h, 0, C, GEMM_EPI_GATE, C, 2 * C, 0, C, 1, s))) return rc;
+        if ((rc = launch_pack_a(blob + f.wq_o_A[i], dense + 5 * dn, GEMM_BM, p.mb_in, p.nch_rs + p.nch1h, 0, C, GEMM_EPI_GATE, C, 2 * C, 0, C, 1, s))) return rc;
+        for (float* A : {blob + f.wq_e_A[i], blob + f.wq_o_A[i]})
+            if ((rc = launch_pack_a(A, w->cond_w[2], GEMM_BM, p.mb_in, p.nch_rs + p.nch1h, C, H, GEMM_EPI_GATE, C, 2 * C,
+                                    (long long)2 * C * i, H, 1, s))) return rc;
+    }
     if ((rc = launch_fold_in0(w->in_w[0], w->start_w, w->start_b, blob + f.in0f_w, C, d.n_half, ks, s))) return rc;
     for (int t = 0; t < ks; ++t)
         if ((rc = launch_pack_a(blob + f.in0f_A, blob + f.in0f_w + t, GEMM_BM, p.mb_in, p.nch_in0f, 0, FOLD_ROWS, GEMM_EPI_GATE, C,
@@ -1166,7 +1225,8 @@
            (t.bf16_ps ? (1 << 20) : 0) | (t.bf16_no_ps ? (1 << 21) : 0) | (t.taco_poll_delay_set ? (1 << 23) : 0) |
            (t.taco_valu ? (1 << 24) : 0) | (t.up_no_mfma ? (1 << 25) : 0) | (t.f32_no_wn_fold ? (1 << 26) : 0) |
            (t.taco_bg_no_pipe ? (1 << 27) : 0) | (t.f32_no_winograd ? (1 << 28) : 0) | (t.f32_winograd_min >= 0 ? (1 << 29) : 0) |
-           (t.f32_winograd_plain ? (1 << 30) : 0) | (t.f32_winograd_fused_min >= 0 ? 4 : 0) | (t.f32_winograd_no_fused ? 32 : 0);
+           (t.f32_winograd_plain ? (1 << 30) : 0) | (t.f32_winograd_fused_min >= 0 ? 4 : 0) | (t.f32_winograd_no_fused ? 32 : 0) |
+           (t.f32_winograd_f43_min >= 0 ? (1 << 6) : 0) | (t.f32_winograd_no_f43 ? (1 << 22) : 0);
 }
 
 int ctts_profile_create(void** handle) {
diff --git a/cookietts_amd/csrc/waveglow_kernels.h b/cookietts_amd/csrc/waveglow_kernels.h
--- a/cookietts_amd/csrc/waveglow_kernels.h
+++ b/cookietts_amd/csrc/waveglow_kernels.h
@@ -48,4 +48,9 @@
                               int batch, int C, int H, int d, int L, int Lp, int ld, int pad, int ldp, int ncols, bool cond_rows,
                               bool vec_d2, hipStream_t s);
 
+int launch_winograd_g43(const float* in_w, float* dense, int rows, int C, hipStream_t s);
+int launch_winograd_transform_quad(const float* x, long long x_bstride, const float* h2, long long h_bstride, float* V, float* Hc,
+                                   int batch, int C, int H, int d, int L, int Lq, int ld, int pad, int ldq, int ncols, bool cond_rows,
+                                   hipStream_t s);
+
 }
diff --git a/cookietts_amd/csrc/waveglow_kernels.hip b/cookietts_amd/csrc/waveglow_kernels.hip
--- a/cookietts_amd/csrc/waveglow_kernels.hip
+++ b/cookietts_amd/csrc/waveglow_kernels.hip
@@ -543,6 +543,98 @@
         float* o = Hc + ((size_t)b * H + (row - C)) * ldp + j4;
         *reinterpret_cast<float4*>(o) = v0;
         *reinterpret_cast<float4*>(o + plane) = v1;
+    }
+}
+
+
+__global__ __launch_bounds__(256) void winograd_g43_kernel(const float* __restrict__ in_w, float* __restrict__ dense, int n) {
+    const int idx = blockIdx.x * 256 + threadIdx.x;
+    if (idx >= n) return;
+    const double w0 = in_w[(size_t)idx * 3], w1 = in_w[(size_t)idx * 3 + 1], w2 = in_w[(size_t)idx * 3 + 2];
+    dense[idx] = (float)(w0 / 4.0);
+    dense[(size_t)n + idx] = (float)(-(w0 + w1 + w2) / 6.0);
+    dense[2 * (size_t)n + idx] = (float)(-(w0 - w1 + w2) / 6.0);
+    dense[3 * (size_t)n + idx] = (float)(w0 / 24.0 + w1 / 12.0 + w2 / 6.0);
+    dense[4 * (size_t)n + idx] = (float)(w0 / 24.0 - w1 / 12.0 + w2 / 6.0);
+    dense[5 * (size_t)n + idx] = in_w[(size_t)idx * 3 + 2];
+}
+
+template <int MODE>
+__global__ __launch_bounds__(256) void winograd_transform_quad_kernel(const float* __restrict__ x, long long x_bstride,
+                                                                      const float* __restrict__ h2, long long h_bstride,
+                                                                      float* __restrict__ V, float* __restrict__ Hc, int C, int H,
+                                                                      int d, int L, int Lq, int ld, int pad, int ldq, int ncols) {
+    const int q4 = (blockIdx.x * 256 + threadIdx.x) * 4;
+    if (q4 >= ncols) return;
+    const int row = blockIdx.y, b = blockIdx.z, B = gridDim.z;
+    const bool is_x = row < C;
+    const float* src = is_x ? x + (size_t)b * x_bstride + (size_t)row * ld + pad
+                            : h2 + (size_t)b * h_bstride + (size_t)(row - C) * ld + pad;
+    float tap[6][4];
+#pragma unroll
+    for (int j = 0; j < 6; ++j)
+#pragma unroll
+        for (int e = 0; e < 4; ++e) tap[j][e] = 0.f;
+    [[maybe_unused]] auto ld4 = [&](int t) { return (t >= 0 && t < L) ? *reinterpret_cast<const float4*>(src + t) : make_float4(0.f, 0.f, 0.f, 0.f); };
+    if constexpr (MODE == 1) {
+        if (q4 < Lq) {
+            const int t0 = (q4 / d) * 4 * d + q4 % d;
+#pragma unroll
+            for (int j = 0; j < 6; ++j) {
+                if (!is_x && (j == 0 || j == 5)) continue;
+                const float4 v = ld4(t0 + (j - 1) * d);
+                tap[j][0] = v.x; tap[j][1] = v.y; tap[j][2] = v.z; tap[j][3] = v.w;
+            }
+        }
+    } else if constexpr (MODE == 2) {
+        if (q4 < Lq) {
+            float a[24];
+#pragma unroll
+            for (int u = 0; u < 6; ++u) {
+                const float4 v = ld4(4 * q4 - 4 + 4 * u);
+                a[4 * u] = v.x; a[4 * u + 1] = v.y; a[4 * u + 2] = v.z; a[4 * u + 3] = v.w;
+            }
+            const bool hi = q4 + 2 < Lq;
+#pragma unroll
+            for (int j = 0; j < 6; ++j) {
+                tap[j][0] = a[4 + (j - 1) * 2]; tap[j][1] = a[5 + (j - 1) * 2];
+                tap[j][2] = hi ? a[12 + (j - 1) * 2] : 0.f; tap[j][3] = hi ? a[13 + (j - 1) * 2] : 0.f;
+            }
+        }
+    } else {
+#pragma unroll
+        for (int e = 0; e < 4; ++e) {
+            const int q = q4 + e;
+            const int t0 = (q / d) * 4 * d + q % d;
+#pragma unroll
+            for (int j = 0; j < 6; ++j) {
+                const int t = t0 + (j - 1) * d;
+                tap[j][e] = (q < Lq && t >= 0 && t < L && (is_x || (j >= 1 && j <= 4))) ? src[t] : 0.f;
+            }
+        }
+    }
+    if (is_x) {
+        const size_t plane = (size_t)B * C * ldq;
+        float* o = V + ((size_t)b * C + row) * ldq + q4;
+        float v[6][4];
+#pragma unroll
+        for (int e = 0; e < 4; ++e) {
+            const float x0 = tap[0][e], x1 = tap[1][e], x2 = tap[2][e], x3 = tap[3][e], x4 = tap[4][e], x5 = tap[5][e];
+            const float s12 = x1 + x2, d12 = x1 - x2, s34 = x3 + x4, d34 = x3 - x4, d13 = x1 - x3, d24 = x2 - x4;
+            v[0][e] = 4.f * x0 - 5.f * x2 + x4;
+            v[1][e] = s34 - 4.f * s12;
+            v[2][e] = 4.f * d12 - d34;
+            v[3][e] = -2.f * d13 - d24;
+            v[4][e] = 2.f * d13 - d24;
+            v[5][e] = 4.f * x1 - 5.f * x3 + x5;
+        }
+#pragma unroll
+        for (int j = 0; j < 6; ++j) *reinterpret_cast<float4*>(o + j * plane) = make_float4(v[j][0], v[j][1], v[j][2], v[j][3]);
+    } else {
+        const size_t plane = (size_t)B * H * ldq;
+        float* o = Hc + ((size_t)b * H + (row - C)) * ldq + q4;
+#pragma unroll
+        for (int k = 0; k < 4; ++k) *reinterpret_cast<float4*>(o + k * plane) = make_float4(tap[k + 1][0], tap[k + 1][1], tap[k + 1][2], tap[k + 1][3]);
     }
 }
 
@@ -809,6 +901,33 @@
         hipLaunchKernelGGL(winograd_transform_kernel<0>, grid, dim3(256), 0, s, x, x_bstride, h2, h_bstride, V, Hc, C, H, d, L, Lp,
                            ld, pad, ldp, ncols);
     CTTS_CHECK_LAUNCH("winograd_transform");
+    return CTTS_OK;
+}
+
+int launch_winograd_g43(const float* in_w, float* dense, int rows, int C, hipStream_t s) {
+    const int n = rows * C;
+    hipLaunchKernelGGL(winograd_g43_kernel, dim3((n + 255) / 256), dim3(256), 0, s, in_w, dense, n);
+    CTTS_CHECK_LAUNCH("winograd_g43");
+    return CTTS_OK;
+}
+
+int launch_winograd_transform_quad(const float* x, long long x_bstride, const float* h2, long long h_bstride, float* V, float* Hc,
+                                   int batch, int C, int H, int d, int L, int Lq, int ld, int pad, int ldq, int ncols, bool cond_rows,
+                                   hipStream_t s) {
+    CTTS_CHECK_ARG(d >= 1 && Lq % d == 0 && (long long)Lq * 4 >= L && Lq <= ncols && ncols <= ldq && ncols % 4 == 0 && ldq % 4 == 0 &&
+                       ld % 4 == 0 && pad % 4 == 0 && pad + L <= ld && (!cond_rows || Hc != nullptr),
+                   "winograd_transform_quad: d=%d L=%d Lq=%d ncols=%d ldq=%d ld=%d pad=%d", d, L, Lq, ncols, ldq, ld, pad);
+    dim3 grid((ncols / 4 + 255) / 256, cond_rows ? C + H : C, batch);
+    if (d % 4 == 0 && L % 4 == 0)
+        hipLaunchKernelGGL(winograd_transform_quad_kernel<1>, grid, dim3(256), 0, s, x, x_bstride, h2, h_bstride, V, Hc, C, H, d, L, Lq,
+                           ld, pad, ldq, ncols);
+    else if (d == 2 && L % 4 == 0)
+        hipLaunchKernelGGL(winograd_transform_quad_kernel<2>, grid, dim3(256), 0, s, x, x_bstride, h2, h_bstride, V, Hc, C, H, d, L, Lq,
+                           ld, pad, ldq, ncols);
+    else
+        hipLaunchKernelGGL(winograd_transform_quad_kernel<0>, grid, dim3(256), 0, s, x, x_bstride, h2, h_bstride, V, Hc, C, H, d, L, Lq,
+                           ld, pad, ldq, ncols);
+    CTTS_CHECK_LAUNCH("winograd_transform_quad");
     return CTTS_OK;
 }
 
diff --git a/cookietts_amd/csrc/wn_winograd_layer.h b/cookietts_amd/csrc/wn_winograd_layer.h
--- a/cookietts_amd/csrc/wn_winograd_layer.h
+++ b/cookietts_amd/csrc/wn_winograd_layer.h
@@ -6,9 +6,11 @@
 namespace ctts {
 
 constexpr int WNWG_MAX_CHUNKS = 320;
+constexpr int WNWG_F23 = 0, WNWG_F43 = 1;
 
 struct WnWinogradLayerArgs {
     const float *A_T2, *A_T3, *A_e, *A_o, *bias;
+    const float *A_T4, *A_T5;
     const float* V; long long vplane;
     const float* Hc; long long hplane;
     const float* h2; long long h_bstride;
@@ -17,10 +19,12 @@
     int ldp, Lp, ntiles;
     int d, L, ld, pad;
     int in_place;
+    int form;
     int kt, kt_total, b0, col0;
 };
 
 bool wn_winograd_layer_supported(int C, int H);
+bool wn_winograd_layer_f43_supported(int C, int H);
 int launch_wn_winograd_layer(const WnWinogradLayerArgs& a, hipStream_t stream);
 
 }
diff --git a/cookietts_amd/csrc/wn_winograd_layer.hip b/cookietts_amd/csrc/wn_winograd_layer.hip
--- a/cookietts_amd/csrc/wn_winograd_layer.hip
+++ b/cookietts_amd/csrc/wn_winograd_layer.hip
@@ -16,8 +16,10 @@
 
 }
 
-template <int NT>
+template <int NT, int F43>
 __global__ __launch_bounds__(256, 2) void wn_winograd_layer_f32_kernel(const WnWinogradLayerArgs a) {
+    static_assert(!F43 || NT == 1, "the F(4,3) form runs on the 64-column shape");
+    constexpr int NI = F43 ? 4 : 2;
     constexpr int BN = 64 * NT;
     constexpr int A_ST = GEMM_KC * 128;
     constexpr int STG = A_ST + GEMM_KC * BN;
@@ -41,8 +43,13 @@
     const int b = a.b0 + gt / a.kt;
     const int n0 = a.col0 + (gt % a.kt) * BN;
 
-    const int n1 = a.C / GEMM_KC, n2 = (a.C + a.H) / GEMM_KC;
-    const int c_e = 2 * n1, c_o = 2 * n1 + n2, nch = 2 * n1 + 2 * n2;
+    const int n1 = a.C / GEMM_KC, n2 = (a.C + a.H) / GEMM_KC, nh = a.H / GEMM_KC;
+    const int c_e = NI * n1;
+    int ps[NI + 1];
+    ps[0] = c_e;
+#pragma unroll
+    for (int k = 0; k < NI; ++k) ps[k + 1] = ps[k] + (k == 0 || k == NI - 1 ? n2 : nh);
+    const int nch = ps[NI];
 
     const int mb_t = (64 * cb) >> 8, loc_t = (64 * cb) & 255;
     const int mb_s = (a.C + 64 * cb) >> 8, loc_s = (a.C + 64 * cb) & 255;
@@ -51,13 +58,17 @@
         for (int c = t; c < nch; c += 256) {
             const float *ap, *bp;
             if (c < c_e) {
-                const int ph = c >= n1, loc = c - ph * n1;
-                ap = (ph ? a.A_T3 : a.A_T2) + ((size_t)mb_t * n1 + loc) * (GEMM_KC * 256) + loc_t;
+                const int ph = F43 ? c / n1 : (int)(c >= n1), loc = c - ph * n1;
+                ap = (ph == 0 ? a.A_T2 : ph == 1 ? a.A_T3 : ph == 2 ? a.A_T4 : a.A_T5) + ((size_t)mb_t * n1 + loc) * (GEMM_KC * 256) + loc_t;
                 bp = a.V + (1 + ph) * a.vplane + ((size_t)b * a.C + (size_t)loc * GEMM_KC) * a.ldp + n0;
             } else {
-                const int ph = c >= c_o, loc = c - c_e - ph * n2;
-                ap = (ph ? a.A_o : a.A_e) + ((size_t)(cb >> 1) * n2 + loc) * (GEMM_KC * 256) + (cb & 1) * 128;
-                if (loc < n1) bp = a.V + (ph ? 3 : 0) * a.vplane + ((size_t)b * a.C + (size_t)loc * GEMM_KC) * a.ldp + n0;
+                int ph = 0;
+#pragma unroll
+                for (int k = 1; k < NI; ++k) ph += c >= ps[k];
+                const bool last = ph == NI - 1;
+                const int loc = c - ps[ph] + (ph == 0 || last ? 0 : n1);
+                ap = (last ? a.A_o : a.A_e) + ((size_t)(cb >> 1) * n2 + loc) * (GEMM_KC * 256) + (cb & 1) * 128;
+                if (loc < n1) bp = a.V + (last ? NI + 1 : 0) * a.vplane + ((size_t)b * a.C + (size_t)loc * GEMM_KC) * a.ldp + n0;
                 else if (a.in_place) bp = a.h2 + (size_t)b * a.h_bstride + (size_t)(loc - n1) * GEMM_KC * a.ld;
                 else bp = a.Hc + ph * a.hplane + ((size_t)b * a.H + (size_t)(loc - n1) * GEMM_KC) * a.ldp + n0;
             }
@@ -67,7 +78,7 @@
         if (t < 128) lds[BIAS + t] = a.bias[cb * 128 + t];
     }
 
-    unsigned offa_g[2], offa_s[2], offb[NT], offb_e[NT], offb_o[NT];
+    unsigned offa_g[2], offa_s[2], offb[NT], offb_m[NI][NT];
     {
         const int col = (lane & 31) * 4;
         const long long delta = ((long long)(mb_s - mb_t) * n1) * (GEMM_KC * 256) + (loc_s - loc_t);
@@ -82,26 +93,30 @@
         for (int j = 0; j < NT; ++j) {
             const int krow = (wave + 4 * j) * RPP + lane / UPR;
             offb[j] = (unsigned)(((size_t)krow * a.ldp + bcol) * 4);
-            offb_e[j] = offb_o[j] = 0;
+#pragma unroll
+            for (int k = 0; k < NI; ++k) offb_m[k][j] = 0;
             if (a.in_place) {
                 const int q = n0 + bcol;
-                const int te = (q / a.d) * (2 * a.d) + q % a.d;
+                const int te = (q / a.d) * (NI * a.d) + q % a.d;
                 const int lim = (a.ld - a.pad - 4) & ~3;
-                offb_e[j] = (unsigned)(((size_t)krow * a.ld + a.pad + min(te, lim)) * 4);
-                offb_o[j] = (unsigned)(((size_t)krow * a.ld + a.pad + min(te + a.d, lim)) * 4);
+#pragma unroll
+                for (int k = 0; k < NI; ++k) offb_m[k][j] = (unsigned)(((size_t)krow * a.ld + a.pad + min(te + k * a.d, lim)) * 4);
             }
         }
     }
-    const int m_e0 = a.in_place ? c_e + n1 : 0x7fffffff, m_e1 = c_o;
-    const int m_o0 = a.in_place ? c_o + n1 : 0x7fffffff;
-
-    wg_f32x16 S[2][NT], D[2][NT];
-#pragma unroll
-    for (int i = 0; i < 2; ++i)
-#pragma unroll
-        for (int j = 0; j < NT; ++j)
-#pragma unroll
-            for (int r = 0; r < 16; ++r) { S[i][j][r] = 0.0f; D[i][j][r] = 0.0f; }
+    int m_lo[NI];
+#pragma unroll
+    for (int k = 0; k < NI; ++k) m_lo[k] = a.in_place ? ps[k] + (k == 0 || k == NI - 1 ? n1 : 0) : 0x7fffffff;
+
+    wg_f32x16 X[NI][2][NT];
+#pragma unroll
+    for (int k = 0; k < NI; ++k)
+#pragma unroll
+        for (int i = 0; i < 2; ++i)
+#pragma unroll
+            for (int j = 0; j < NT; ++j)
+#pragma unroll
+                for (int r = 0; r < 16; ++r) X[k][i][j][r] = 0.0f;
     __syncthreads();
 
     typedef __attribute__((address_space(3))) float* lds_fptr;
@@ -112,7 +127,8 @@
     lds_fptr la_ = (lds_fptr)(lds + (buf) * STG + wave * 256);                                              \
     const uint4 e_ = ctab[c];                                                                               \
     const bool as_ = (c) < c_e;                                       \
-    const bool me_ = (c) >= m_e0 && (c) < m_e1, mo_ = (c) >= m_o0;
+    bool mk_[NI];                                                     \
+    _Pragma("unroll") for (int k = 0; k < NI; ++k) mk_[k] = (c) >= m_lo[k] && (c) < ps[k + 1];
 #define WNWG_BASES()                                                                                        \
     const gbyte_ptr ac_ = reinterpret_cast<gbyte_ptr>(                                                      \
         ((unsigned long long)(unsigned)__builtin_amdgcn_readfirstlane((int)e_.y) << 32) |                   \
@@ -127,7 +143,8 @@
             asm volatile("" : "+v"(o_));                                                                    \
             __builtin_amdgcn_global_load_lds((gfloat_ptr)(ac_ + o_), la_ + 1024 * (p), 16, 0, 0);           \
         } else if constexpr ((p) < 2 + NT) {                                                                \
-            unsigned o_ = me_ ? offb_e[(p) - 2] : mo_ ? offb_o[(p) - 2] : offb[(p) - 2];                     \
+            unsigned o_ = offb[(p) - 2];                                                                    \
+            _Pragma("unroll") for (int k = 0; k < NI; ++k) o_ = mk_[k] ? offb_m[k][(p) - 2] : o_;           \
             asm volatile("" : "+v"(o_));                                                                    \
             __builtin_amdgcn_global_load_lds((gfloat_ptr)(bp_ + o_), la_ + A_ST + 1024 * ((p) - 2), 16, 0, 0); \
         }                                                                                                   \
@@ -150,16 +167,16 @@
 #define WNWG_READ_FRAGS(ks)                                                                                 \
     _Pragma("unroll") for (int mt = 0; mt < 2; ++mt) av[ks][mt] = As[(2 * (ks) + lhi) * 128 + mt * 64];     \
     _Pragma("unroll") for (int nt = 0; nt < NT; ++nt) bv[ks][nt] = Bs[(2 * (ks) + lhi) * BN + nt * 32];
-#define WNWG_MFMA(X, ks)                                                                                    \
+#define WNWG_MFMA(Y, ks)                                                                                    \
     _Pragma("unroll") for (int mt = 0; mt < 2; ++mt)                                                        \
         _Pragma("unroll") for (int nt = 0; nt < NT; ++nt)                                                   \
-            X[mt][nt] = __builtin_amdgcn_mfma_f32_32x32x2f32(av[ks][mt], bv[ks][nt], X[mt][nt], 0, 0, 0);
-#define WNWG_REGION(X, ks, p)                                                                               \
+            Y[mt][nt] = __builtin_amdgcn_mfma_f32_32x32x2f32(av[ks][mt], bv[ks][nt], Y[mt][nt], 0, 0, 0);
+#define WNWG_REGION(Y, ks, p)                                                                               \
     __builtin_amdgcn_sched_barrier(0);                                                                      \
     if constexpr ((ks) + 1 < GEMM_KC / 2) { WNWG_READ_FRAGS((ks) + 1) }                                     \
-    WNWG_MFMA(X, ks)                                                                                        \
+    WNWG_MFMA(Y, ks)                                                                                        \
     WNWG_PIECE(p);
-#define WNWG_CHUNK(X)                                                                                       \
+#define WNWG_CHUNK(Y)                                                                                       \
     {                                                                                                       \
         const float* As = lds + cur * STG + wm * 32 + l31;                                                  \
         const float* Bs = lds + cur * STG + A_ST + wn * (32 * NT) + l31;                                    \
@@ -170,8 +187,8 @@
         WNWG_READ_FRAGS(0)                                                                                  \
         __builtin_amdgcn_sched_barrier(0);                                                                  \
         WNWG_BASES()                                                                                        \
-        WNWG_REGION(X, 0, 0) WNWG_REGION(X, 1, 1) WNWG_REGION(X, 2, 2) WNWG_REGION(X, 3, 3)                 \
-        WNWG_REGION(X, 4, 4) WNWG_REGION(X, 5, 4) WNWG_REGION(X, 6, 4) WNWG_REGION(X, 7, 4)                 \
+        WNWG_REGION(Y, 0, 0) WNWG_REGION(Y, 1, 1) WNWG_REGION(Y, 2, 2) WNWG_REGION(Y, 3, 3)                 \
+        WNWG_REGION(Y, 4, 4) WNWG_REGION(Y, 5, 4) WNWG_REGION(Y, 6, 4) WNWG_REGION(Y, 7, 4)                 \
         __builtin_amdgcn_sched_barrier(0);                                                                  \
         WNWG_WAIT();                                         \
         __builtin_amdgcn_s_barrier();                                                                       \
@@ -181,39 +198,77 @@
 
     float* dst = a.act + (size_t)b * a.act_bstride + (size_t)(cb * 64 + wm * 32) * a.ld + a.pad;
     const float* bias = lds + BIAS + wm * 32;
-#define WNWG_GATE(X, par)                                                                                   \
+#define WNWG_GATE(Y, par)                                                                                   \
     _Pragma("unroll") for (int nt = 0; nt < NT; ++nt) {                                                     \
         const int n = n0 + wn * (32 * NT) + nt * 32 + l31;                                                  \
-        const int ns = (n / a.d) * (2 * a.d) + n % a.d + (par) * a.d;                                       \
+        const int ns = (n / a.d) * (NI * a.d) + n % a.d + (par) * a.d;                                      \
         if (n < a.Lp && ns < a.L) {                                                                         \
             _Pragma("unroll") for (int r = 0; r < 16; ++r) {                                                \
                 const int row = (r & 3) + 8 * (r >> 2) + 4 * lhi;                                           \
-                const float u0 = X[0][nt][r] + bias[row];                                                   \
-                const float u1 = X[1][nt][r] + bias[64 + row];                                              \
+                const float u0 = Y[0][nt][r] + bias[row];                                                   \
+                const float u1 = Y[1][nt][r] + bias[64 + row];                                              \
                 dst[(size_t)row * a.ld + ns] = wg_tanh(u0) * wg_sigmoid(u1);                                \
             }                                                                                               \
         }                                                                                                   \
     }
 
+#define WNWG_RUN(k, end) for (; ch < (end); ++ch) WNWG_CHUNK(X[k])
+#define WNWG_DRAIN()                                                                                        \
+    asm volatile("s_waitcnt vmcnt(0)" ::: "memory");          \
+    __builtin_amdgcn_s_barrier();
     int ch = 0;
-    for (; ch < n1; ++ch) WNWG_CHUNK(S)
-    for (; ch < c_e; ++ch) WNWG_CHUNK(D)
-#pragma unroll
-    for (int i = 0; i < 2; ++i)
-#pragma unroll
-        for (int j = 0; j < NT; ++j)
-#pragma unroll
-            for (int r = 0; r < 16; ++r) {
-                const float s = S[i][j][r], dd = D[i][j][r];
-                S[i][j][r] = s + dd;
-                D[i][j][r] = s - dd;
-            }
-    for (; ch < c_o; ++ch) WNWG_CHUNK(S)
-    WNWG_GATE(S, 0)
-    for (; ch < nch; ++ch) WNWG_CHUNK(D)
-    asm volatile("s_waitcnt vmcnt(0)" ::: "memory");
-    __builtin_amdgcn_s_barrier();
-    WNWG_GATE(D, 1)
+    if constexpr (!F43) {
+        WNWG_RUN(0, n1)
+        WNWG_RUN(1, c_e)
+#pragma unroll
+        for (int i = 0; i < 2; ++i)
+#pragma unroll
+            for (int j = 0; j < NT; ++j)
+#pragma unroll
+                for (int r = 0; r < 16; ++r) {
+                    const float s = X[0][i][j][r], dd = X[1][i][j][r];
+                    X[0][i][j][r] = s + dd;
+                    X[1][i][j][r] = s - dd;
+                }
+        WNWG_RUN(0, ps[1])
+        WNWG_GATE(X[0], 0)
+        WNWG_RUN(1, nch)
+        WNWG_DRAIN()
+        WNWG_GATE(X[1], 1)
+    } else {
+        WNWG_RUN(0, n1)
+        WNWG_RUN(1, 2 * n1)
+        WNWG_RUN(2, 3 * n1)
+        WNWG_RUN(3, c_e)
+#pragma unroll
+        for (int i = 0; i < 2; ++i)
+#pragma unroll
+            for (int j = 0; j < NT; ++j)
+#pragma unroll
+                for (int r = 0; r < 16; ++r) {
+                    const float p1 = X[0][i][j][r], p2 = X[1][i][j][r], p3 = X[2][i][j][r], p4 = X[3][i][j][r];
+                    const float sa = p1 + p2, sb = p1 - p2, sc = p3 + p4, se = p3 - p4;
+                    X[0][i][j][r] = sa + sc;
+                    X[1][i][j][r] = sb + 2.0f * se;
+                    X[2][i][j][r] = sa + 4.0f * sc;
+                    X[3][i][j][r] = sb + 8.0f * se;
+                }
+#pragma unroll
+        for (int k = 0; k < NI; ++k)
+#pragma unroll
+            for (int i = 0; i < 2; ++i) asm volatile("" : "+v"(X[k][i][0]));
+        WNWG_RUN(0, ps[1])
+        WNWG_GATE(X[0], 0)
+        WNWG_RUN(1, ps[2])
+        WNWG_GATE(X[1], 1)
+        WNWG_RUN(2, ps[3])
+        WNWG_GATE(X[2], 2)
+        WNWG_RUN(3, nch)
+        WNWG_DRAIN()
+        WNWG_GATE(X[3], 3)
+    }
+#undef WNWG_DRAIN
+#undef WNWG_RUN
 #undef WNWG_GATE
 #undef WNWG_CHUNK
 #undef WNWG_REGION
@@ -229,14 +284,18 @@
     return C >= 128 && C % 128 == 0 && H > 0 && H % GEMM_KC == 0 && 2 * (C / GEMM_KC) + 2 * ((C + H) / GEMM_KC) <= WNWG_MAX_CHUNKS;
 }
 
+bool wn_winograd_layer_f43_supported(int C, int H) {
+    return wn_winograd_layer_supported(C, H) && 4 * (C / GEMM_KC) + 2 * ((C + H) / GEMM_KC) + 2 * (H / GEMM_KC) <= WNWG_MAX_CHUNKS;
+}
+
 namespace {
-template <int NT>
+template <int NT, int F43 = 0>
 int launch_wnwg_shape(WnWinogradLayerArgs a, int kt, long long kt_total, hipStream_t stream) {
     a.kt = kt;
     a.kt_total = (int)kt_total;
     const long long blocks = 8ll * (a.C / 64) * ((kt_total + 7) / 8);
     CTTS_CHECK_ARG(blocks > 0 && blocks < (1ll << 31) && kt_total < (1ll << 31), "wn_winograd_layer: grid %lld", blocks);
-    hipLaunchKernelGGL((wn_winograd_layer_f32_kernel<NT>), dim3((unsigned)blocks), dim3(256), 0, stream, a);
+    hipLaunchKernelGGL((wn_winograd_layer_f32_kernel<NT, F43>), dim3((unsigned)blocks), dim3(256), 0, stream, a);
     CTTS_CHECK_LAUNCH("wn_winograd_layer");
     return CTTS_OK;
 }
@@ -246,7 +305,10 @@
     WnWinogradLayerArgs a = a_in;
     CTTS_CHECK_ARG(wn_winograd_layer_supported(a.C, a.H), "wn_winograd_layer: C=%d H=%d", a.C, a.H);
     CTTS_CHECK_ARG(a.A_T2 && a.A_T3 && a.A_e && a.A_o && a.bias && a.V && a.act && a.batch >= 1, "wn_winograd_layer: operand not set");
-    CTTS_CHECK_ARG(a.d >= 1 && a.L >= 1 && a.Lp >= 1 && a.ntiles >= 1 && a.Lp <= a.ntiles * 128 && a.ntiles * 128 <= a.ldp && a.ldp % 4 == 0 &&
+    const bool f43 = a.form == WNWG_F43;
+    const int tw = f43 ? 64 : 128;
+    CTTS_CHECK_ARG(a.form == WNWG_F23 || (f43 && wn_winograd_layer_f43_supported(a.C, a.H) && a.A_T4 && a.A_T5), "wn_winograd_layer: form %d", a.form);
+    CTTS_CHECK_ARG(a.d >= 1 && a.L >= 1 && a.Lp >= 1 && a.ntiles >= 1 && a.Lp <= a.ntiles * tw && a.ntiles * tw <= a.ldp && a.ldp % 4 == 0 &&
                        a.ld % 4 == 0 && a.pad >= 0 && a.pad % 4 == 0 && a.L + a.pad <= a.ld,
                    "wn_winograd_layer: geometry d=%d L=%d Lp=%d ntiles=%d ldp=%d ld=%d pad=%d", a.d, a.L, a.Lp, a.ntiles, a.ldp, a.ld, a.pad);
     CTTS_CHECK_ARG(a.in_place ? (a.h2 && a.d % 4 == 0 && a.ld - a.pad >= 4 && a.h_bstride % 4 == 0 && reinterpret_cast<uintptr_t>(a.h2) % 16 == 0)
@@ -254,6 +316,7 @@
                    "wn_winograd_layer: cond rows (in_place=%d d=%d)", a.in_place, a.d);
     a.b0 = 0;
     a.col0 = 0;
+    if (f43) return launch_wnwg_shape<1, 1>(a, a.ntiles, (long long)a.ntiles * a.batch, stream);
     const Tuning tn = tuning();
     const int ncb = a.C / 64;
     const long long slots = 2ll * wf_row_cus();
```

New measurement: 3.824 million samples/s (median of 6 runs). 1.09x the previous value.
